# ShawnNew/Detectron2-CenterNet

Measured on AMD Instinct MI355X. Metric: images/sec at 512x512 (infer bs=64), higher is better.
Workload: dtype f16x3; 1 GPU; DLA-34 CenterNet eval forward+decode, 64x3x512x512 uint8 per GPU, 80 classes, K=100, random-init weights (BatchNorm statistics calibrated), DCN offsets ~N(0,1px), 100 detections per image post-processed; per_gpu_batch=64, global_batch=64, parallelism=replicas x1

## Files before the change

### detectron2-centernet_amd/_lib.py

```python
import ctypes as C
import os

_HERE = os.path.dirname(os.path.abspath(__file__))
LIB_PATH = os.path.join(_HERE, "lib", "libctdet_hip.so")

F16, F32, U8, F16X3 = 0, 1, 2, 3
ACT_NONE, ACT_RELU, ACT_SIGMOID_CLAMP = 0, 1, 2
DCN_MASK_LOGIT, DCN_MASK_PROB, DCN_MASK_NONE = 0, 1, 2
CLIP_NONE, CLIP_VALUE, CLIP_NORM = 0, 1, 2
NORM_L1, NORM_L2, NORM_INF = 1, 2, 3


class ConvDesc(C.Structure):
    _fields_ = [(n, C.c_int32) for n in (
        "B", "H", "W", "Cin", "in_stride", "Cout", "Ho", "Wo", "out_stride",
        "R", "S", "stride", "pad", "dil", "Kpad", "Cout_pad",
        "compute_dtype", "out_dtype", "act", "res_stride")] + [("clamp_lo", C.c_float), ("clamp_hi", C.c_float), ("korder", C.c_int32), ("in_dil", C.c_int32)]


_vp, _i32, _i64, _f32, _f64, _sz = C.c_void_p, C.c_int32, C.c_int64, C.c_float, C.c_double, C.c_size_t
SIGNATURES = {
    "ctdet_last_error": (C.c_char_p, []),
    "ctdet_abi_version": (_i32, []),
    "ctdet_conv_cout_tile": (_i32, [_i32]),
    "ctdet_set_label_mode": (_i32, [_i32]),
    "ctdet_last_kernel_label": (C.c_char_p, []),
    "ctdet_conv_pair_supported": (_i32, [C.POINTER(ConvDesc), _vp]),
    "ctdet_head_fused_supported": (_i32, [_i32, _i32, _i32, _i32, _i32, _vp]),
    "ctdet_conv2d_fwd": (_i32, [C.POINTER(ConvDesc), _vp, _vp, _vp, _vp, _vp, _vp, _vp]),
    "ctdet_conv1x1_cat_fwd": (_i32, [C.POINTER(ConvDesc), _vp, _vp, _vp, _i32, _vp, _vp, _vp, _vp, _vp, _vp]),
    "ctdet_dcnv2_fwd": (_i32, [C.POINTER(ConvDesc), _vp, _vp, _i32, _i32, _vp, _vp, _vp, _vp, _vp]),
    "ctdet_dcnv2_offset_supported": (_i32, [C.POINTER(ConvDesc)]),
    "ctdet_dcnv2_cols_supported": (_i32, [C.POINTER(ConvDesc), _vp, _vp]),
    "ctdet_dcnv2_fwd_cols": (_i32, [C.POINTER(ConvDesc), _vp, _vp, _i32, _i32, _vp, _vp, _vp, _vp, _vp, _vp]),
    "ctdet_dcnv2_offset_fwd": (_i32, [C.POINTER(ConvDesc), _vp, _vp, _vp, _vp, _i32, _vp, _vp, _vp, _vp, _vp]),
    "ctdet_preprocess": (_i32, [_vp, _i32, _vp, _i32, _i32, _i32, _i32, _i32, _i32, _i64, _vp, _vp, _i32, _i32, _vp]),
    "ctdet_preprocess_mirror": (_i32, [_vp, _i32, _vp, _i32, _i32, _i32, _i32, _i32, _i32, _i64, _vp, _vp, _i32, _i32, _i32, _vp]),
    "ctdet_head_fused_fwd": (_i32, [_vp, _vp, _vp, _vp, _vp]),
    "ctdet_head_fused_x3_fwd": (_i32, [_vp, _vp, _vp, _vp, _vp, _vp]),
    "ctdet_dla_base_fwd": (_i32, [_vp] * 14),
    "ctdet_dla_base_x3_fwd": (_i32, [_vp] * 14),
    "ctdet_dla_base_mirror_fwd": (_i32, [_vp, _i32] + [_vp] * 13),
    "ctdet_dla_base_x3_mirror_fwd": (_i32, [_vp, _i32] + [_vp] * 13),
    "ctdet_maxpool2x2": (_i32, [_vp, _vp, _i32, _i32, _i32, _i32, _i32, _i32, _i32, _vp]),
    "ctdet_maxpool3x3s2": (_i32, [_vp, _vp, _i32, _i32, _i32, _i32, _i32, _i32, _i32, _vp]),
    "ctdet_maxpool3x3s2_ceil": (_i32, [_vp, _vp, _i32, _i32, _i32, _i32, _i32, _i32, _i32, _vp]),
    "ctdet_global_avgpool": (_i32, [_vp, _i32, _i32, _i32, _i32, _i32, _vp, _vp]),
    "ctdet_ese_scale": (_i32, [_vp, _i32, _vp, _vp, _i32, _vp, _i32, _i32, _i32, _i32, _i32, _vp]),
    "ctdet_pack_weights": (_i32, [_vp, _vp, _i32, _i32, _i32, _i32, _i32, _i32, _i32, _i32, _i32, _vp]),
    "ctdet_pack_weights_batch": (_i32, [_vp, _i32, _i32, _vp]),
    "ctdet_split_weights": (_i32, [_vp, _vp, _i64, _vp]),
    "ctdet_pack_weights_x3": (_i32, [_vp, _vp, _vp] + [_i32] * 10 + [_vp]),
    "ctdet_pack_weights_x3_batch": (_i32, [_vp, _i32, _i32, _vp]),
    "ctdet_dwconvT_add": (_i32, [_vp, _vp, _vp, _vp, _i32, _i32, _i32, _i32, _i32, _i32, _i32, _i32, _i32, _vp]),
    "ctdet_dwconv3x3_fwd": (_i32, [_vp, _i32, _vp, _vp, _i32, _i32, _i32, _i32, _i32, _i32, _i32, _i32, _vp]),
    "ctdet_dwconv3x3_wgrad_workspace_bytes": (_sz, [_i32, _i32, _i32, _i32, _i32]),
    "ctdet_dwconv3x3_wgrad": (_i32, [_vp, _i32, _vp, _i32, _vp, _vp, _f32, _i32, _i32, _i32, _i32, _i32, _i32, _i32, _vp]),
    "ctdet_decode_workspace_bytes": (_sz, [_i32, _i32, _i32, _i32, _i32]),
    "ctdet_decode": (_i32, [_vp, _i32, _vp, _i32, _vp, _i32, _i32, _i32, _i32, _i32, _i32, _f32, _f32, _vp, _vp, _vp, _vp, _vp, _vp]),
    "ctdet_decode_flip": (_i32, [_vp, _i32, _vp, _i32, _vp, _i32, _i32, _i32, _i32, _i32, _i32, _f32, _f32, _vp, _vp, _vp, _vp, _vp, _vp]),
    "ctdet_postprocess": (_i32, [_vp, _vp, _vp, _i32, _i32, _i32, _f32, _vp, _vp, _vp, _vp, _vp, _vp]),
    "ctdet_decode_status": (_i32, [_vp, _i32, _i32, _i32, _i32, _i32, _vp]),
    "ctdet_gaussian_targets": (_i32, [_vp, _vp, _vp, _i32, _i32, _i32, _i32, _i32, _vp, _vp, _vp, _vp, _vp, _vp]),
    "ctdet_gaussian_radius": (_i32, [_vp, _i32, _vp, _vp, _vp]),
    "ctdet_focal_loss_workspace_bytes": (_sz, [_i64]),
    "ctdet_focal_loss": (_i32, [_vp, _vp, _vp, _i32, _i32, _i32, _i32, _f32, _vp, _vp, _vp, _vp, _vp]),
    "ctdet_reg_l1_loss": (_i32, [_vp, _i32, _vp, _vp, _vp, _i32, _i32, _i32, _f32, _vp, _vp, _i32, _vp]),
    "ctdet_chan_workspace_bytes": (_sz, [_i32]),
    "ctdet_bn_train_fwd": (_i32, [_vp, _i32, _vp, _i32, _vp, _i32, _i32, _i32, _vp, _vp, _f32, _f32, _vp, _vp, _vp, _vp,
                                   _vp, _vp, _vp, _i32, _i32, _vp]),
    "ctdet_bn_train_bwd": (_i32, [_vp, _i32, _vp, _i32, _vp, _i32, _vp, _vp, _vp, _i32, _i32, _i32, _vp, _i32, _vp, _i32,
                                   _vp, _vp, _f32, _vp, _i32, _vp]),
    "ctdet_bn_local_stats": (_i32, [_vp, _i32, _i32, _i32, _i32, _i32, _vp, _vp, _i32, _vp]),
    "ctdet_bn_sync_fwd": (_i32, [_vp, _i32, _vp, _i32, _vp, _i32, _i32, _i32, _vp, _i32, _vp, _vp, _f32, _f32, _vp, _vp, _vp,
                                  _vp, _vp, _vp, _i32, _i32, _vp]),
    "ctdet_bn_local_grad_sums": (_i32, [_vp, _i32, _vp, _i32, _vp, _i32, _vp, _vp, _i32, _i32, _i32, _i32, _i32, _vp, _vp, _vp,
                                         _f32, _vp, _i32, _vp]),
    "ctdet_bn_sync_bwd": (_i32, [_vp, _i32, _vp, _i32, _vp, _i32, _vp, _vp, _vp, _vp, _vp, _i32, _i32, _i32, _i32, _vp, _i32,
                                  _vp, _i32, _i32, _vp]),
    "ctdet_conv_wgrad": (_i32, [C.POINTER(ConvDesc), _vp, _vp, _vp, _f32, _vp]),
    "ctdet_conv_wgrad_oihw": (_i32, [C.POINTER(ConvDesc), _vp, _vp, _vp, _f32, _i32, _i32, _i32, _i32, _vp]),
    "ctdet_grad_scatter_oihw": (_i32, [_vp, _vp, _vp, _vp, _vp, _vp, _i32, _vp]),
    "ctdet_depth_to_space2": (_i32, [_vp, _i32, _vp, _i32, _i32, _i32, _i32, _i32, _i32, _i32, _i32, _vp]),
    "ctdet_maxpool3x3s2_bwd": (_i32, [_vp, _i32, _vp, _i32, _vp, _i32, _i32, _i32, _i32, _i32, _i32, _i32, _vp]),
    "ctdet_finite_flag": (_i32, [_vp, _i64, _i32, _i32, _vp, _vp]),
    "ctdet_ese_dot": (_i32, [_vp, _i32, _vp, _i32, _i32, _i32, _i32, _i32, _vp, _vp]),
    "ctdet_ese_bwd": (_i32, [_vp, _i32, _vp, _vp, _vp, _i32, _i32, _i32, _i32, _i32, _vp]),
    "ctdet_maxpool2x2_bwd": (_i32, [_vp, _i32, _vp, _i32, _vp, _i32, _i32, _i32, _i32, _i32, _i32, _vp]),
    "ctdet_dwconvT_bwd": (_i32, [_vp, _i32, _vp, _i32, _vp, _vp, _i32, _vp, _i32, _i32, _i32, _i32, _i32, _i32, _vp]),
    "ctdet_dcn_cols": (_i32, [_vp, _i32, _vp, _i32, _vp, _i32, _i32, _i32, _i32, _i32, _i32, _vp]),
    "ctdet_dcn_col2im_coord": (_i32, [_vp, _vp, _i32, _vp, _i32, _vp, _vp, _i32, _i32, _i32, _i32, _i32, _i32, _i32, _i32, _i32, _vp]),
    "ctdet_dcn_col2im_fused": (_i32, [_vp, _i32, _i32, _vp, _vp, _vp, _i32, _vp, _i32, _vp, _vp, _i32, _i32, _i32, _i32, _i32, _i32, _vp]),
    "ctdet_sgd_momentum": (_i32, [_vp, _vp, _vp, _i64, _vp, _f32, _f32, _i32, _vp]),
    "ctdet_sgd_momentum_runs": (_i32, [_vp, _vp, _vp, C.c_int64, _vp, _vp, _vp, _vp, _i32, _f32, _i32, _vp]),
    "ctdet_grad_chunk_norms": (_i32, [_vp, _i64, _vp, _vp, _i32, _i32, _vp, _vp]),
    "ctdet_grad_clip_coefs": (_i32, [_vp, _vp, _i32, _i32, _i32, _f32, _vp, _vp, _vp]),
    "ctdet_sgd_momentum_runs_clip": (_i32, [_vp, _vp, _vp, _i64, _vp, _vp, _vp, _vp, _i32, _f32, _i32, _i32, _i32, _f32, _vp,
                                             _vp]),
    "ctdet_adam_advance": (_i32, [_vp, _vp, _f64, _f64, _vp]),
    "ctdet_adam_runs": (_i32, [_vp, _vp, _vp, _vp, _vp, _i64, _vp, _vp, _vp, _vp, _i32, _vp, _f64, _f64, _f64, _i32, _i32, _i32,
                               _f32, _vp, _vp]),
    "ctdet_cocoeval_workspace_bytes": (_sz, [_i64, _i64, _i32, _i32, _i32, _i32]),
    "ctdet_cocoeval_iou": (_i32, [_vp, _i32, _vp, _vp, _i32, _vp, _vp]),
    "ctdet_cocoeval_match": (_i32, [_vp, _vp, _vp, _vp, _i64, _vp, _vp, _vp, _vp, _i64, _i32, _i32, _vp, _i32, _vp, _i32, _i32,
                                    _vp, _vp, _vp, _vp, _vp, _vp, _vp]),
    "ctdet_cocoeval_accumulate": (_i32, [_vp, _vp, _vp, _vp, _vp, _vp, _i64, _i32, _i32, _i32, _vp, _i32, _vp, _i32, _i32, _vp,
                                         _vp, _vp, _vp, _vp]),
    "ctdet_set_tuning_flags": (_i32, [C.c_uint32]),
    "ctdet_get_tuning_flags": (C.c_uint32, []),
    "ctdet_comm_unique_id": (_i32, [_vp]),
    "ctdet_comm_init": (_i32, [_vp, _i32, _i32, C.POINTER(C.c_void_p)]),
    "ctdet_allreduce_bucket": (_i32, [_vp, _vp, _i64, _vp]),
    "ctdet_bcast": (_i32, [_vp, _vp, _i64, _i32, _vp]),
    "ctdet_comm_destroy": (_i32, [_vp]),
}

_lib = None


def lib():
    global _lib
    if _lib is None:
        if not os.path.exists(LIB_PATH):
            raise RuntimeError(
                f"{LIB_PATH} is missing: build it with `python -c 'import __graft_entry__ as g; g.build()'` "
                "(or `make -C detectron2-centernet_amd/csrc`). There is no CPU fallback for the HIP path.")
        l = C.CDLL(LIB_PATH)
        for name, (res, args) in SIGNATURES.items():
            fn = getattr(l, name)
            fn.restype = res
            fn.argtypes = args
        _lib = l
        if os.environ.get("CTDET_TUNE_FLAGS"):
            l.ctdet_set_tuning_flags(int(os.environ["CTDET_TUNE_FLAGS"], 0))
    return _lib


def check(rc, what):
    if rc != 0:
        msg = lib().ctdet_last_error()
        raise RuntimeError(f"{what} failed (rc={rc}): {msg.decode() if msg else ''}")


class PackDesc(C.Structure):
    _fields_ = [("w", C.c_void_p), ("packed", C.c_void_p)] + [(n, C.c_int32) for n in (
        "O", "I", "R", "S", "chans_pad", "rows_pad", "Kpad", "korder", "transposed", "blk0")]


class Pack3Desc(C.Structure):
    _fields_ = [("w", C.c_void_p), ("packed", C.c_void_p), ("scale_out", C.c_void_p)] + [(n, C.c_int32) for n in (
        "O", "I", "R", "S", "chans_pad", "rows_pad", "Kpad", "layout", "transposed", "scale_n", "blk0", "pad_")]


class DlaBaseDesc(C.Structure):
    _fields_ = [("B", C.c_int32), ("H", C.c_int32), ("W", C.c_int32), ("Hp", C.c_int32), ("Wp", C.c_int32),
                ("img_dtype", C.c_int32), ("img_batch_stride", C.c_int64), ("mean", C.c_float * 3), ("std", C.c_float * 3),
                ("out_stride", C.c_int32), ("pool_stride", C.c_int32)]


class HeadDesc(C.Structure):
    _fields_ = [("nheads", C.c_int32), ("B", C.c_int32), ("H", C.c_int32), ("W", C.c_int32), ("Cin", C.c_int32),
                ("in_stride", C.c_int32), ("w2", C.c_void_p * 4), ("b2", C.c_void_p * 4), ("y", C.c_void_p * 4),
                ("y_stride", C.c_int32 * 4), ("cout", C.c_int32 * 4), ("act", C.c_int32 * 4),
                ("clamp_lo", C.c_float), ("clamp_hi", C.c_float)]


TUNE_NO_HALO, TUNE_NO_WIN, TUNE_DCN_MIXED, TUNE_NO_WGRAD_WINDOW, TUNE_NO_COL2IM_WINDOW, TUNE_NO_F32_DCN_WINDOW, TUNE_DCN_WINDOW_V1, TUNE_NO_SMALL_GRID_TILES = 1, 2, 4, 8, 16, 32, 64, 128
TUNE_DCN_SPLIT_4W = 256
TUNE_NO_HALO_TAP2 = 512
TUNE_PAIR2_128, TUNE_DCN_SPLIT_8W64, TUNE_TARGETS_MEMSET = 1024, 2048, 4096


class tuning:

    def __init__(self, flags):
        self.flags = flags

    def __enter__(self):
        self.prev = lib().ctdet_get_tuning_flags()
        lib().ctdet_set_tuning_flags(self.prev | self.flags)
        return self

    def __exit__(self, *exc):
        lib().ctdet_set_tuning_flags(self.prev)
        return False
```

### detectron2-centernet_amd/csrc/api.hip

```cpp
#include "conv_common.h"
#include "../../include/ctdet_hip.h"
#include <stdarg.h>
#include <stdio.h>
#include <string.h>
#include <stdlib.h>
#include <atomic>

static thread_local char g_err[512] = "";
void ctdet_set_error(const char* fmt, ...) {
  va_list ap;
  va_start(ap, fmt);
  vsnprintf(g_err, sizeof(g_err), fmt, ap);
  va_end(ap);
}

thread_local int g_label_mode = 0;
static thread_local char g_label[128] = "";
bool ctdet_set_label(const char* fmt, ...) {
  va_list ap;
  va_start(ap, fmt);
  vsnprintf(g_label, sizeof(g_label), fmt, ap);
  va_end(ap);
  return g_label_mode == 2;
}
// ... 193 lines not shown
    if (j < nsrc) {
      CTDET_CHECK(xs[j] && cins[j] > 0 && cins[j] % align == 0 && strides[j] >= cins[j] && strides[j] % align == 0,
                  "conv1x1_cat: bad source %d (cin=%d stride=%d)", j, cins[j], strides[j]);
      cum += cins[j];
      a.xs[j] = xs[j]; a.xs_stride[j] = strides[j];
    } else {
      a.xs[j] = xs[nsrc - 1]; a.xs_stride[j] = strides[nsrc - 1];
    }
    a.xs_cend[j] = cum;
  }
  CTDET_CHECK(cum == d->Cin, "conv1x1_cat: sources sum to %d channels, descriptor says %d", cum, d->Cin);
  a.nsrc = nsrc < 2 ? 2 : nsrc;
  if (nsrc == 1) { a.nsrc = 1; a.in_stride = strides[0]; }
  a.x = xs[0]; a.w = w_packed; a.scale = scale; a.bias = bias; a.res = residual; a.y = y;
  if (d->compute_dtype == CTDET_DT_F16) return launch_conv_f16(a, d->out_dtype, false, (hipStream_t)stream);
  if (d->compute_dtype == CTDET_DT_F32 || d->compute_dtype == CTDET_DT_F16X3) {
    CTDET_CHECK(d->out_dtype == CTDET_DT_F32, "conv1x1_cat(f32 / f16x3): output must be f32");
    return launch_conv_f32(a, false, d->compute_dtype == CTDET_DT_F16X3, (hipStream_t)stream);
  }
  CTDET_CHECK(false, "conv1x1_cat: bad compute dtype %d", d->compute_dtype);
}

int32_t ctdet_dcnv2_fwd(const ctdet_conv_desc* d, const void* x, const float* offset_mask, int32_t om_stride,
                        int32_t mask_is_prob, const void* w_packed, const float* scale, const float* bias, void* y, void* stream) {
  ConvArgs a;
  int rc = fill_args(d, a);
  if (rc) return rc;
  if (a.M == 0) return 0;
  CTDET_CHECK(x && w_packed && y && offset_mask, "dcnv2: null pointer");
  CTDET_CHECK(mask_is_prob >= CTDET_DCN_MASK_LOGIT && mask_is_prob <= CTDET_DCN_MASK_NONE, "dcnv2: mask mode %d", mask_is_prob);
  CTDET_CHECK(om_stride >= (mask_is_prob == CTDET_DCN_MASK_NONE ? 2 : 3) * d->R * d->S, "dcnv2: om_stride=%d < %d*R*S", om_stride,
              mask_is_prob == CTDET_DCN_MASK_NONE ? 2 : 3);
  a.x = x; a.w = w_packed; a.scale = scale; a.bias = bias; a.res = nullptr; a.y = y;
  a.om = offset_mask; a.om_stride = om_stride; a.mask_is_prob = mask_is_prob;
  if (d->compute_dtype == CTDET_DT_F16) return launch_conv_f16(a, d->out_dtype, true, (hipStream_t)stream);
  if (d->compute_dtype == CTDET_DT_F32 || d->compute_dtype == CTDET_DT_F16X3) {
    CTDET_CHECK(d->out_dtype == CTDET_DT_F32, "dcnv2(f32 / f16x3): output must be f32");
    return launch_conv_f32(a, true, d->compute_dtype == CTDET_DT_F16X3, (hipStream_t)stream);
  }
  CTDET_CHECK(false, "dcnv2: bad compute dtype %d", d->compute_dtype);
}

int32_t ctdet_dcnv2_cols_supported(const ctdet_conv_desc* d, const void* x, const void* y) {
  ConvArgs a;
  if (fill_args(d, a) || d->compute_dtype != CTDET_DT_F16X3 || d->out_dtype != CTDET_DT_F32) return 0;
  a.x = x; a.y = const_cast<void*>(y);
  return dcn_split_window_ok(a) ? 1 : 0;
}

int32_t ctdet_dcnv2_fwd_cols(const ctdet_conv_desc* d, const void* x, const float* offset_mask, int32_t om_stride,
                             int32_t mask_is_prob, const void* w_packed, const float* scale, const float* bias, void* y,
                             float* cols_out, void* stream) {
  ConvArgs a;
  int rc = fill_args(d, a);
  if (rc) return rc;
  if (a.M == 0) return 0;
  CTDET_CHECK(x && w_packed && y && offset_mask && cols_out, "dcnv2_fwd_cols: null pointer");
  CTDET_CHECK(mask_is_prob >= CTDET_DCN_MASK_LOGIT && mask_is_prob <= CTDET_DCN_MASK_NONE, "dcnv2: mask mode %d", mask_is_prob);
  CTDET_CHECK(om_stride >= (mask_is_prob == CTDET_DCN_MASK_NONE ? 2 : 3) * d->R * d->S, "dcnv2: om_stride=%d < %d*R*S", om_stride,
              mask_is_prob == CTDET_DCN_MASK_NONE ? 2 : 3);
  CTDET_CHECK(d->compute_dtype == CTDET_DT_F16X3 && d->out_dtype == CTDET_DT_F32 && (((size_t)cols_out) & 15) == 0,
              "dcnv2_fwd_cols: the f16x3 mode's entry point (f32 tensors), 16-byte aligned columns");
  a.x = x; a.w = w_packed; a.scale = scale; a.bias = bias; a.res = nullptr; a.y = y;
  a.om = offset_mask; a.om_stride = om_stride; a.mask_is_prob = mask_is_prob;
  CTDET_CHECK(dcn_split_window_ok(a), "dcnv2_fwd_cols: shape not served by the LDS-window kernel (ask ctdet_dcnv2_cols_supported first)");
  a.cols_out = cols_out;
  return launch_conv_f32(a, true, true, (hipStream_t)stream);
}

int32_t ctdet_dcnv2_offset_supported(const ctdet_conv_desc* d) {
  ConvArgs a;
  if (fill_args(d, a)) return 0;
  a.y = nullptr;
  if (d->compute_dtype == CTDET_DT_F16X3) return (d->out_dtype == CTDET_DT_F32 && dcn_offset_fused_x3_ok(a)) ? 1 : 0;
  if (d->compute_dtype != CTDET_DT_F16) return 0;
  return dcn_offset_fused_ok(a) ? 1 : 0;
}

int32_t ctdet_dcnv2_offset_fwd(const ctdet_conv_desc* d, const void* x, const void* w_off_packed, const float* b_off,
                               float* om_out, int32_t om_out_stride, const void* w_packed, const float* scale,
                               const float* bias, void* y, void* stream) {
  ConvArgs a;
  int rc = fill_args(d, a);
  if (rc) return rc;
  if (a.M == 0) return 0;
  CTDET_CHECK(x && w_off_packed && b_off && w_packed && y, "dcnv2_offset: null pointer");
  if (d->compute_dtype == CTDET_DT_F16X3) {
    CTDET_CHECK(d->out_dtype == CTDET_DT_F32 && !om_out, "dcnv2_offset(f16x3): f32 output, no om_out (inference form)");
    a.x = x; a.w = w_packed; a.scale = scale; a.bias = bias; a.res = nullptr; a.y = y;
    a.w_off = w_off_packed; a.b_off = b_off; a.mask_is_prob = DCN_MASK_LOGIT;
    return launch_dcn_offset_x3(a, (hipStream_t)stream);
  }
  CTDET_CHECK(d->compute_dtype == CTDET_DT_F16, "dcnv2_offset: f16 or f16x3");
  CTDET_CHECK(!om_out || (om_out_stride >= 28 && om_out_stride % 4 == 0 && ((size_t)om_out & 15) == 0),
              "dcnv2_offset: om_out needs a 16-byte aligned row of >= 28 floats (stride %d)", om_out_stride);
  a.x = x; a.w = w_packed; a.scale = scale; a.bias = bias; a.res = nullptr; a.y = y;
  a.w_off = w_off_packed; a.b_off = b_off; a.om_out = om_out; a.om_out_stride = om_out_stride;
  return launch_conv_f16(a, d->out_dtype, true, (hipStream_t)stream);
}

int32_t ctdet_preprocess(const void* img, int32_t img_dtype, void* out, int32_t out_dtype, int32_t B, int32_t H,
                         int32_t W, int32_t Hp, int32_t Wp, int64_t img_batch_stride, const float* mean3,
                         const float* std3, int32_t out_stride, int32_t border, void* stream) {
  CTDET_CHECK(img && out && mean3 && std3, "preprocess: null pointer");
  return launch_preprocess(img, img_dtype, out, out_dtype, B, H, W, Hp, Wp, (long)img_batch_stride, mean3, std3,
                           out_stride, border, -1, (hipStream_t)stream);
}

int32_t ctdet_preprocess_mirror(const void* img, int32_t img_dtype, void* out, int32_t out_dtype, int32_t B, int32_t H,
                                int32_t W, int32_t Hp, int32_t Wp, int64_t img_batch_stride, const float* mean3,
                                const float* std3, int32_t out_stride, int32_t border, int32_t mirror_from, void* stream) {
  CTDET_CHECK(img && out && mean3 && std3, "preprocess: null pointer");
  CTDET_CHECK(mirror_from >= 0 && mirror_from <= B, "preprocess: mirror_from=%d outside [0, B=%d]", mirror_from, B);
  return launch_preprocess(img, img_dtype, out, out_dtype, B, H, W, Hp, Wp, (long)img_batch_stride, mean3, std3,
                           out_stride, border, mirror_from, (hipStream_t)stream);
}

static int head_args(const ctdet_head_desc* d, HeadArgs& a) {
  a.nheads = d->nheads; a.B = d->B; a.H = d->H; a.W = d->W; a.Cin = d->Cin; a.in_stride = d->in_stride;
  a.clamp_lo = d->clamp_lo; a.clamp_hi = d->clamp_hi;
  CTDET_CHECK(d->nheads >= 1 && d->nheads <= 4, "head_fused: nheads=%d out of range", d->nheads);
  for (int h = 0; h < d->nheads; ++h) {
    CTDET_CHECK(d->w2[h] && d->b2[h] && d->y[h], "head_fused: head %d: null pointer", h);
    a.w2[h] = d->w2[h]; a.b2[h] = (const float*)d->b2[h]; a.y[h] = (float*)d->y[h];
    a.y_stride[h] = d->y_stride[h]; a.cout[h] = d->cout[h]; a.act[h] = d->act[h];
  }
  return 0;
}

int32_t ctdet_head_fused_supported(int32_t compute_dtype, int32_t H, int32_t W, int32_t Cin, int32_t in_stride, const void* x) {
  HeadArgs a = {};
  a.x = x; a.H = H; a.W = W; a.Cin = Cin; a.in_stride = in_stride;
  if (compute_dtype != CTDET_DT_F16 && compute_dtype != CTDET_DT_F16X3) return 0;
  return head_fused_x_ok(a, compute_dtype == CTDET_DT_F16X3) ? 1 : 0;
}

int32_t ctdet_head_fused_fwd(const ctdet_head_desc* d, const void* x, const void* w1, const float* b1, void* stream) {
  CTDET_CHECK(d && x && w1 && b1, "head_fused: null pointer");
  HeadArgs a = {};
  a.x = x; a.w1 = w1; a.b1 = b1;
  if (int rc = head_args(d, a)) return rc;
  return launch_head_fused(a, (hipStream_t)stream);
}

int32_t ctdet_head_fused_x3_fwd(const ctdet_head_desc* d, const void* x, const void* w1, const float* s1, const float* b1,
                                void* stream) {
  CTDET_CHECK(d && x && w1 && s1 && b1, "head_fused_x3: null pointer");
  HeadArgs a = {};
  a.x = x; a.w1 = w1; a.s1 = s1; a.b1 = b1;
  if (int rc = head_args(d, a)) return rc;
  return launch_head_fused_x3(a, (hipStream_t)stream);
}

static int32_t dla_base_entry(const ctdet_dla_base_desc* d, int mirror_from, const void* images, const void* w_stem,
                              const float* scale_stem, const float* bias_stem, const void* w_l0, const float* scale_l0,
                              const float* bias_l0, const void* w_l1, const float* scale_l1, const float* bias_l1,
                              void* out, void* pooled, void* stream) {
  CTDET_CHECK(d && images && w_stem && scale_stem && bias_stem && w_l0 && scale_l0 && bias_l0 && w_l1 && scale_l1 && bias_l1 &&
              out, "dla_base: null pointer");
  BaseArgs a = {};
  a.img = images; a.img_dtype = d->img_dtype; a.img_batch_stride = (long)d->img_batch_stride;
  a.B = d->B; a.H = d->H; a.W = d->W; a.Hp = d->Hp; a.Wp = d->Wp;
  for (int i = 0; i < 3; ++i) { a.mean[i] = d->mean[i]; a.stdv[i] = d->std[i]; }
  a.w0 = w_stem; a.s0 = scale_stem; a.b0 = bias_stem;
  a.w1 = w_l0; a.s1 = scale_l0; a.b1 = bias_l0;
  a.w2 = w_l1; a.s2 = scale_l1; a.b2 = bias_l1;
  a.y = out; a.out_stride = d->out_stride;
  a.pool = pooled; a.pool_stride = d->pool_stride;
  a.mirror_from = mirror_from;
  return launch_dla_base(a, (hipStream_t)stream);
}

int32_t ctdet_dla_base_fwd(const ctdet_dla_base_desc* d, const void* images, const void* w_stem, const float* scale_stem,
                           const float* bias_stem, const void* w_l0, const float* scale_l0, const float* bias_l0,
                           const void* w_l1, const float* scale_l1, const float* bias_l1, void* out, void* pooled,
                           void* stream) {
  return dla_base_entry(d, -1, images, w_stem, scale_stem, bias_stem, w_l0, scale_l0, bias_l0, w_l1, scale_l1, bias_l1, out,
                        pooled, stream);
}

int32_t ctdet_dla_base_mirror_fwd(const ctdet_dla_base_desc* d, int32_t mirror_from, const void* images, const void* w_stem,
                                  const float* scale_stem, const float* bias_stem, const void* w_l0, const float* scale_l0,
                                  const float* bias_l0, const void* w_l1, const float* scale_l1, const float* bias_l1,
                                  void* out, void* pooled, void* stream) {
  CTDET_CHECK(d && mirror_from >= 0 && mirror_from <= d->B, "dla_base: mirror_from=%d outside [0, B=%d]", mirror_from,
              d ? d->B : 0);
  return dla_base_entry(d, mirror_from, images, w_stem, scale_stem, bias_stem, w_l0, scale_l0, bias_l0, w_l1, scale_l1,
                        bias_l1, out, pooled, stream);
}

static int32_t dla_base_x3_entry(const ctdet_dla_base_desc* d, int mirror_from, const void* images, const void* w_stem,
                                 const float* scale_stem, const float* bias_stem, const void* w_l0, const float* scale_l0,
                                 const float* bias_l0, const void* w_l1, const float* scale_l1, const float* bias_l1,
                                 float* out, float* pooled, void* stream) {
  CTDET_CHECK(d && images && w_stem && scale_stem && bias_stem && w_l0 && scale_l0 && bias_l0 && w_l1 && scale_l1 && bias_l1 &&
              out, "dla_base(f16x3): null pointer");
  BaseArgs a = {};
  a.img = images; a.img_dtype = d->img_dtype; a.img_batch_stride = (long)d->img_batch_stride;
  a.B = d->B; a.H = d->H; a.W = d->W; a.Hp = d->Hp; a.Wp = d->Wp;
  for (int i = 0; i < 3; ++i) { a.mean[i] = d->mean[i]; a.stdv[i] = d->std[i]; }
  a.w0 = w_stem; a.s0 = scale_stem; a.b0 = bias_stem;
  a.w1 = w_l0; a.s1 = scale_l0; a.b1 = bias_l0;
  a.w2 = w_l1; a.s2 = scale_l1; a.b2 = bias_l1;
  a.y = out; a.out_stride = d->out_stride;
  a.pool = pooled; a.pool_stride = d->pool_stride;
  a.mirror_from = mirror_from;
  return launch_dla_base_x3(a, (hipStream_t)stream);
}

int32_t ctdet_dla_base_x3_fwd(const ctdet_dla_base_desc* d, const void* images, const void* w_stem, const float* scale_stem,
                              const float* bias_stem, const void* w_l0, const float* scale_l0, const float* bias_l0,
                              const void* w_l1, const float* scale_l1, const float* bias_l1, float* out, float* pooled,
                              void* stream) {
  return dla_base_x3_entry(d, -1, images, w_stem, scale_stem, bias_stem, w_l0, scale_l0, bias_l0, w_l1, scale_l1, bias_l1,
                           out, pooled, stream);
}

int32_t ctdet_dla_base_x3_mirror_fwd(const ctdet_dla_base_desc* d, int32_t mirror_from, const void* images,
                                     const void* w_stem, const float* scale_stem, const float* bias_stem, const void* w_l0,
                                     const float* scale_l0, const float* bias_l0, const void* w_l1, const float* scale_l1,
                                     const float* bias_l1, float* out, float* pooled, void* stream) {
  CTDET_CHECK(d && mirror_from >= 0 && mirror_from <= d->B, "dla_base(f16x3): mirror_from=%d outside [0, B=%d]", mirror_from,
              d ? d->B : 0);
  return dla_base_x3_entry(d, mirror_from, images, w_stem, scale_stem, bias_stem, w_l0, scale_l0, bias_l0, w_l1, scale_l1,
                           bias_l1, out, pooled, stream);
}

int32_t ctdet_maxpool2x2(const void* x, void* y, int32_t dtype, int32_t B, int32_t H, int32_t W, int32_t C,
                         int32_t in_stride, int32_t out_stride, void* stream) {
  CTDET_CHECK(x && y, "maxpool2x2: null pointer");
  return launch_maxpool2x2(x, y, dtype, B, H, W, C, in_stride, out_stride, (hipStream_t)stream);
}

int32_t ctdet_maxpool3x3s2(const void* x, void* y, int32_t dtype, int32_t B, int32_t H, int32_t W, int32_t C,
                           int32_t in_stride, int32_t out_stride, void* stream) {
  CTDET_CHECK(x && y, "maxpool3x3s2: null pointer");
  return launch_maxpool3x3s2(x, y, dtype, B, H, W, C, in_stride, out_stride, 0, (hipStream_t)stream);
}

int32_t ctdet_maxpool3x3s2_ceil(const void* x, void* y, int32_t dtype, int32_t B, int32_t H, int32_t W, int32_t C,
                                int32_t in_stride, int32_t out_stride, void* stream) {
  CTDET_CHECK(x && y, "maxpool3x3s2_ceil: null pointer");
  return launch_maxpool3x3s2(x, y, dtype, B, H, W, C, in_stride, out_stride, 1, (hipStream_t)stream);
}

int32_t ctdet_global_avgpool(const void* x, int32_t dtype, int32_t B, int32_t HW, int32_t C, int32_t stride, float* out,
                             void* stream) {
  CTDET_CHECK(x && out, "global_avgpool: null pointer");
  return launch_global_avgpool(x, dtype, B, HW, C, stride, out, (hipStream_t)stream);
}

int32_t ctdet_finite_flag(const float* x, int64_t M, int32_t C, int32_t stride, int32_t* flag, void* stream) {
  CTDET_CHECK(x && flag, "finite_flag: null pointer");
  return launch_finite_flag(x, (long)M, C, stride, (int*)flag, (hipStream_t)stream);
}

int32_t ctdet_ese_scale(const void* x, int32_t x_stride, const float* s, const void* identity, int32_t identity_stride,
                        void* y, int32_t y_stride, int32_t dtype, int32_t B, int32_t HW, int32_t C, void* stream) {
  CTDET_CHECK(x && s && y, "ese_scale: null pointer");
  return launch_ese_scale(x, x_stride, s, identity, identity_stride, y, y_stride, dtype, B, HW, C, (hipStream_t)stream);
}

int32_t ctdet_pack_weights(const float* w, void* packed, int32_t O, int32_t I, int32_t R, int32_t S, int32_t chans_pad,
                           int32_t rows_pad, int32_t Kpad, int32_t korder, int32_t transposed, void* stream) {
  CTDET_CHECK(w && packed, "pack_weights: null pointer");
  return launch_pack_weights(w, packed, O, I, R, S, chans_pad, rows_pad, Kpad, korder, transposed, (hipStream_t)stream);
}

int32_t ctdet_split_weights(const float* w_packed_f32, void* w_split, int64_t n, void* stream) {
  CTDET_CHECK(w_packed_f32 && w_split && n >= 0, "split_weights: bad arguments");
  return launch_split_weights(w_packed_f32, w_split, (long)n, (hipStream_t)stream);
}

int32_t ctdet_pack_weights_batch(const ctdet_pack_desc* table_dev, int32_t n, int32_t total_blocks, void* stream) {
  CTDET_CHECK(n >= 0 && total_blocks >= 0 && (n == 0 || table_dev), "pack_weights_batch: bad arguments");
  static_assert(sizeof(ctdet_pack_desc) == 56, "ctdet_pack_desc layout");
  return launch_pack_weights_batch(table_dev, n, total_blocks, (hipStream_t)stream);
}

int32_t ctdet_pack_weights_x3(const float* w, void* packed, float* scale_out, int32_t O, int32_t I, int32_t R, int32_t S,
                              int32_t chans_pad, int32_t rows_pad, int32_t Kpad, int32_t layout, int32_t transposed,
                              int32_t scale_n, void* stream) {
  return launch_pack_weights_x3(w, packed, scale_out, O, I, R, S, chans_pad, rows_pad, Kpad, layout, transposed, scale_n,
                                (hipStream_t)stream);
}

int32_t ctdet_pack_weights_x3_batch(const ctdet_pack3_desc* table_dev, int32_t n, int32_t total_blocks, void* stream) {
  CTDET_CHECK(n >= 0 && total_blocks >= 0 && (n == 0 || table_dev), "pack_weights_x3_batch: bad arguments");
  static_assert(sizeof(ctdet_pack3_desc) == 72, "ctdet_pack3_desc layout");
  return launch_pack_weights_x3_batch(table_dev, n, total_blocks, (hipStream_t)stream);
}

int32_t ctdet_dwconvT_add(const void* x, const float* w, const void* skip, void* y, int32_t dtype, int32_t B,
                          int32_t H, int32_t W, int32_t C, int32_t f, int32_t in_stride, int32_t skip_stride,
                          int32_t out_stride, void* stream) {
  CTDET_CHECK(x && w && y, "dwconvT: null pointer");
  return launch_dwconvT_add(x, w, skip, y, dtype, B, H, W, C, f, in_stride, skip_stride, out_stride,
                            (hipStream_t)stream);
}

int32_t ctdet_dwconv3x3_fwd(const void* x, int32_t x_stride, const float* w, void* y, int32_t y_stride, int32_t B, int32_t H,
                            int32_t W, int32_t C, int32_t stride, int32_t rot180, int32_t dtype, void* stream) {
  CTDET_CHECK(x && w && y, "dwconv3x3: null pointer");
  CTDET_CHECK(rot180 == 0 || rot180 == 1, "dwconv3x3: rot180 %d", rot180);
  const int strides[2] = {x_stride, y_stride};
  const int rc = dwconv3x3_check(dtype, B, H, W, C, stride, strides, 2);
  if (rc) return rc;
  return launch_dwconv3x3(x, x_stride, w, y, y_stride, B, H, W, C, stride, rot180, dtype, (hipStream_t)stream);
}

size_t ctdet_dwconv3x3_wgrad_workspace_bytes(int32_t B, int32_t H, int32_t W, int32_t C, int32_t dtype) {
  return dwconv3x3_wgrad_workspace_bytes(B, H, W, C, dtype);
}

int32_t ctdet_dwconv3x3_wgrad(const void* x, int32_t x_stride, const void* dy, int32_t dy_stride, float* workspace, float* dw,
                              float scale, int32_t accumulate, int32_t B, int32_t H, int32_t W, int32_t C, int32_t stride,
                              int32_t dtype, void* stream) {
  CTDET_CHECK(x && dy && dw, "dwconv3x3_wgrad: null pointer");
  CTDET_CHECK(accumulate == 0 || accumulate == 1, "dwconv3x3_wgrad: accumulate %d", accumulate);
  const int strides[2] = {x_stride, dy_stride};
  const int rc = dwconv3x3_check(dtype, B, H, W, C, stride, strides, 2);
  if (rc) return rc;
  CTDET_CHECK(stride == 1, "dwconv3x3_wgrad: stride %d: only the stride-1 backward is built", stride);
  CTDET_CHECK(workspace || dwconv3x3_wgrad_workspace_bytes(B, H, W, C, dtype) == 0, "dwconv3x3_wgrad: null workspace");
  CTDET_CHECK(((uintptr_t)dw & 3) == 0 && ((uintptr_t)workspace & 3) == 0, "dwconv3x3_wgrad: misaligned dw / workspace");
  return launch_dwconv3x3_wgrad(x, x_stride, dy, dy_stride, workspace, dw, scale, accumulate, B, H, W, C, dtype,
                                (hipStream_t)stream);
}

size_t ctdet_decode_workspace_bytes(int32_t B, int32_t H, int32_t W, int32_t C, int32_t K) {
  return decode_workspace_bytes(B, H, W, C, K);
}

static int32_t decode_entry(bool flip, const float* heat, int32_t heat_stride, const float* wh, int32_t wh_stride,
                            const float* reg, int32_t reg_stride, int32_t B, int32_t H, int32_t W, int32_t C, int32_t K,
                            float down_ratio, float heat_floor, void* workspace, float* boxes, float* scores,
                            int32_t* classes, int32_t* inds, void* stream) {
  CTDET_CHECK(heat && wh && workspace && boxes && scores && classes, "decode: null pointer");
  CTDET_CHECK(B >= 0 && H > 0 && W > 0, "decode: bad shape B=%d H=%d W=%d", B, H, W);
  CTDET_CHECK(heat_floor >= 0.f && heat_floor < 1.f, "decode: heat_floor %g outside [0, 1)", (double)heat_floor);
  DecArgs a;
  a.heat = heat; a.wh = wh; a.reg = reg; a.heat_stride = heat_stride; a.wh_stride = wh_stride; a.reg_stride = reg_stride;
  a.B = B; a.H = H; a.W = W; a.C = C; a.K = K; a.down_ratio = down_ratio;
  memcpy(&a.floor_bits, &heat_floor, 4);
  a.ws = (uint32_t*)workspace; a.boxes = boxes; a.scores = scores; a.classes = classes; a.inds = inds;
  return launch_decode(a, flip, (hipStream_t)stream);
}

int32_t ctdet_decode(const float* heat, int32_t heat_stride, const float* wh, int32_t wh_stride, const float* reg,
                     int32_t reg_stride, int32_t B, int32_t H, int32_t W, int32_t C, int32_t K, float down_ratio,
                     float heat_floor, void* workspace, float* boxes, float* scores, int32_t* classes, int32_t* inds,
                     void* stream) {
  return decode_entry(false, heat, heat_stride, wh, wh_stride, reg, reg_stride, B, H, W, C, K, down_ratio, heat_floor,
                      workspace, boxes, scores, classes, inds, stream);
}

int32_t ctdet_decode_flip(const float* heat, int32_t heat_stride, const float* wh, int32_t wh_stride, const float* reg,
                          int32_t reg_stride, int32_t B, int32_t H, int32_t W, int32_t C, int32_t K, float down_ratio,
                          float heat_floor, void* workspace, float* boxes, float* scores, int32_t* classes, int32_t* inds,
                          void* stream) {
  return decode_entry(true, heat, heat_stride, wh, wh_stride, reg, reg_stride, B, H, W, C, K, down_ratio, heat_floor,
                      workspace, boxes, scores, classes, inds, stream);
}

int32_t ctdet_postprocess(const float* boxes, const float* scores, const int32_t* classes, int32_t B, int32_t K,
                          int32_t max_det, float score_thresh, const float* img_params, float* out_boxes,
                          float* out_scores, int32_t* out_classes, int32_t* counts, void* stream) {
  CTDET_CHECK(boxes && scores && classes && img_params && out_boxes && out_scores && out_classes && counts,
              "postprocess: null pointer");
  return launch_postprocess(boxes, scores, classes, B, K, max_det, score_thresh, img_params, out_boxes, out_scores,
                            out_classes, counts, (hipStream_t)stream);
}

int32_t ctdet_decode_status(const void* workspace, int32_t B, int32_t H, int32_t W, int32_t C, int32_t K, void* stream) {
  long words = 0;
  int below = 0;
  const int flag = decode_status_words(H, W, C, K, &words, &below);
  for (int b = 0; b < B; ++b) {
    uint32_t st[16];
    hipError_t e = hipMemcpyAsync(st, (const char*)workspace + (size_t)words * 4 * b, sizeof(st), hipMemcpyDeviceToHost,
                                  (hipStream_t)stream);
    if (e == hipSuccess) e = hipStreamSynchronize((hipStream_t)stream);
    CTDET_CHECK(e == hipSuccess, "decode_status: copy failed: %s", hipGetErrorString(e));
    if (st[flag]) {
      ctdet_set_error("decode: image %d overflowed the candidate buffer", b);
      return -75;
    }
    if (st[below]) {
      ctdet_set_error("decode: image %d holds positive heat values below the promised heat_floor", b);
      return -22;
    }
  }
  return 0;
}

int32_t ctdet_gaussian_targets(const float* boxes, const int64_t* classes, const int32_t* counts, int32_t B,
                               int32_t Nmax, int32_t H, int32_t W, int32_t C, float* hm, float* wh, float* reg,
                               int64_t* ind, uint8_t* reg_mask, void* stream) {
  CTDET_CHECK(boxes && classes && counts && hm && wh && reg && ind && reg_mask, "gaussian_targets: null pointer");
  CTDET_CHECK(Nmax >= 1, "gaussian_targets: Nmax must be >= 1");
  return launch_gaussian_targets(boxes, classes, counts, B, Nmax, H, W, C, hm, wh, reg, ind, reg_mask,
                                 (hipStream_t)stream);
}

int32_t ctdet_gaussian_radius(const int32_t* hw_pairs, int32_t n, double* out_radius, int32_t* out_int, void* stream) {
  CTDET_CHECK(hw_pairs, "gaussian_radius: null pointer");
  return launch_gaussian_radius(hw_pairs, n, out_radius, out_int, (hipStream_t)stream);
}

size_t ctdet_focal_loss_workspace_bytes(int64_t numel) { return focal_workspace_bytes((long)numel); }

int32_t ctdet_focal_loss(const float* logits, const float* gt, const float* alpha, int32_t B, int32_t H, int32_t W,
                         int32_t C, float grad_scale, void* workspace, float* loss, float* stats, float* grad,
                         void* stream) {
  CTDET_CHECK(logits && gt && alpha && workspace && loss && stats, "focal_loss: null pointer");
  return launch_focal_loss(logits, gt, alpha, B, H, W, C, grad_scale, workspace, loss, stats, grad, (hipStream_t)stream);
}

int32_t ctdet_reg_l1_loss(const float* pred, int32_t pred_stride, const uint8_t* mask, const int64_t* ind,
                          const float* target, int32_t B, int32_t N, int32_t HW, float grad_scale, float* loss,
                          float* grad, int32_t grad_stride, void* stream) {
  CTDET_CHECK(pred && mask && ind && target && loss, "reg_l1_loss: null pointer");
  return launch_reg_l1(pred, pred_stride, mask, ind, target, B, N, HW, grad_scale, loss, grad, grad_stride,
                       (hipStream_t)stream);
}

size_t ctdet_chan_workspace_bytes(int32_t C) { return chan_reduce_workspace_bytes(C); }

int32_t ctdet_bn_train_fwd(const void* y, int32_t y_stride, const void* res, int32_t res_stride, void* z,
                           int32_t z_stride, int32_t M, int32_t C, const float* gamma, const float* beta, float eps,
                           float momentum, float* running_mean, float* running_var, float* save_mean,
                           float* save_invstd, float* scale, float* shift, void* workspace, int32_t relu, int32_t dtype,
                           void* stream) {
  CTDET_CHECK(y && z && gamma && beta && save_mean && save_invstd && scale && shift && workspace, "bn_train_fwd: null pointer");
  CTDET_CHECK(M > 0, "bn_train_fwd: empty batch");
  if (dtype == CTDET_DT_F32)
    return launch_bn_train_fwd_f32((const float*)y, y_stride, (const float*)res, res_stride, (float*)z, z_stride, M, C, gamma,
                                   beta, eps, momentum, running_mean, running_var, save_mean, save_invstd, scale, shift,
                                   workspace, relu, (hipStream_t)stream);
  return launch_bn_train_fwd((const f16*)y, y_stride, (const f16*)res, res_stride, (f16*)z, z_stride, M, C, gamma, beta,
                             eps, momentum, running_mean, running_var, save_mean, save_invstd, scale, shift, workspace,
                             relu, (hipStream_t)stream);
}

int32_t ctdet_bn_train_bwd(const void* dz, int32_t dz_stride, const void* z, int32_t z_stride, const void* y,
                           int32_t y_stride, const float* mean, const float* invstd, const float* scale, int32_t M,
                           int32_t C, int32_t relu, void* dy, int32_t dy_stride, void* dres, int32_t dres_stride,
                           float* dgamma, float* dbeta, float grad_mult, void* workspace, int32_t dtype, void* stream) {
  CTDET_CHECK(dz && dy && dgamma && dbeta && workspace, "bn_train_bwd: null pointer");
  CTDET_CHECK(!relu || z, "bn_train_bwd: relu backward needs z");
  CTDET_CHECK(!y || (mean && invstd && scale), "bn_train_bwd: statistics missing");
  if (dtype == CTDET_DT_F32)
    return launch_bn_train_bwd_f32((const float*)dz, dz_stride, (const float*)z, z_stride, (const float*)y, y_stride, mean,
                                   invstd, scale, M, C, relu, (float*)dy, dy_stride, (float*)dres, dres_stride, dgamma,
                                   dbeta, grad_mult, workspace, (hipStream_t)stream);
  return launch_bn_train_bwd((const f16*)dz, dz_stride, (const f16*)z, z_stride, (const f16*)y, y_stride, mean, invstd,
                             scale, M, C, relu, (f16*)dy, dy_stride, (f16*)dres, dres_stride, dgamma, dbeta, grad_mult,
                             workspace, (hipStream_t)stream);
}

static const int SYNC_BN_MAX_WORLD = 4096;

int32_t ctdet_bn_local_stats(const void* y, int32_t y_stride, int32_t M, int32_t C, int32_t rank, int32_t world,
                             double* stats, void* workspace, int32_t dtype, void* stream) {
  CTDET_CHECK(M > 0, "bn_local_stats: empty batch on rank %d (SyncBatchNorm needs at least one row on every rank)", rank);
  CTDET_CHECK(y && stats && workspace, "bn_local_stats: null pointer");
  CTDET_CHECK(world >= 1 && world <= SYNC_BN_MAX_WORLD && rank >= 0 && rank < world, "bn_local_stats: rank %d of world %d",
              rank, world);
  return launch_bn_local_stats(y, y_stride, M, C, rank, world, stats, workspace, dtype == CTDET_DT_F32, (hipStream_t)stream);
}

int32_t ctdet_bn_sync_fwd(const void* y, int32_t y_stride, const void* res, int32_t res_stride, void* z, int32_t z_stride,
                          int32_t M, int32_t C, const double* stats, int32_t world, const float* gamma, const float* beta,
                          float eps, float momentum, float* running_mean, float* running_var, float* save_mean,
                          float* save_invstd, float* scale, float* shift, int32_t relu, int32_t dtype, void* stream) {
  CTDET_CHECK(y && z && stats && gamma && beta && save_mean && save_invstd && scale && shift, "bn_sync_fwd: null pointer");
  CTDET_CHECK(!running_mean == !running_var, "bn_sync_fwd: running_mean and running_var go together");
  CTDET_CHECK(M > 0, "bn_sync_fwd: empty batch");
  CTDET_CHECK(world >= 1 && world <= SYNC_BN_MAX_WORLD, "bn_sync_fwd: world %d", world);
  return launch_bn_sync_fwd(y, y_stride, res, res_stride, z, z_stride, M, C, stats, world, gamma, beta, eps, momentum,
                            running_mean, running_var, save_mean, save_invstd, scale, shift, relu, dtype == CTDET_DT_F32,
                            (hipStream_t)stream);
}

int32_t ctdet_bn_local_grad_sums(const void* dz, int32_t dz_stride, const void* z, int32_t z_stride, const void* y,
                                 int32_t y_stride, const float* mean, const float* invstd, int32_t M, int32_t C, int32_t relu,
                                 int32_t rank, int32_t world, double* sums, float* dgamma, float* dbeta, float grad_mult,
                                 void* workspace, int32_t dtype, void* stream) {
  CTDET_CHECK(dz && sums && dgamma && dbeta && workspace, "bn_local_grad_sums: null pointer");
  CTDET_CHECK(!relu || z, "bn_local_grad_sums: relu backward needs z");
  CTDET_CHECK(!y || (mean && invstd), "bn_local_grad_sums: statistics missing");
// ... 220 lines not shown
```

### detectron2-centernet_amd/csrc/common.h

```cpp
#pragma once
#include <hip/hip_runtime.h>
#include <stdint.h>

typedef _Float16 f16;
typedef f16 f16x4 __attribute__((ext_vector_type(4)));
typedef f16 f16x8 __attribute__((ext_vector_type(8)));
typedef f16 f16x16 __attribute__((ext_vector_type(16)));
typedef float f32x4 __attribute__((ext_vector_type(4)));

void ctdet_set_error(const char* fmt, ...);
#define CTDET_CHECK(cond, ...)            \
  do {                                    \
    if (!(cond)) {                        \
      ctdet_set_error(__VA_ARGS__);       \
      return -22;            \
    }                                     \
  } while (0)
#define CTDET_LAUNCH_CHECK()                                          \
  do {                                                                \
    hipError_t e_ = hipGetLastError();                                \
    if (e_ != hipSuccess) {                                           \
      ctdet_set_error("kernel launch failed: %s (%s:%d)",            \
                      hipGetErrorString(e_), __FILE__, __LINE__);     \
      return -5;                                            \
    }                                                                 \
  } while (0)

extern thread_local int g_label_mode;
bool ctdet_set_label(const char* fmt, ...);
#define CTDET_KERNEL(...)                                             \
  do {                                                                \
    if (g_label_mode && ctdet_set_label(__VA_ARGS__)) return 0;       \
  } while (0)
template <typename TOut> inline const char* out_name() { return sizeof(TOut) == 2 ? "f16" : "f32"; }

enum { CTDET_F16 = 0, CTDET_F32 = 1, CTDET_U8 = 2, CTDET_F16X3 = 3 };
enum { CTDET_ACT_NONE = 0, CTDET_ACT_RELU = 1, CTDET_ACT_SIGMOID_CLAMP = 2 };
enum { DCN_MASK_LOGIT = 0, DCN_MASK_PROB = 1, DCN_MASK_NONE = 2 };
enum { SGD_CLIP_NONE = 0, SGD_CLIP_VALUE = 1, SGD_CLIP_NORM = 2 };
enum { GRAD_NORM_L1 = 1, GRAD_NORM_L2 = 2, GRAD_NORM_INF = 3 };
__host__ __device__ inline int dcn_om_channels(int mask_mode) { return mask_mode == DCN_MASK_NONE ? 18 : 27; }

struct ConvArgs {
  const void* x;
  const void* w;
  const float* scale;
  const float* bias;
  const void* res;
  void* y;
  const void* xs[4];
  int xs_stride[4];
  int xs_cend[4];
  int nsrc;
  const float* om;
  int om_stride;
  int mask_is_prob;
  int B, H, W, Cin, in_stride;
  int Cout, Ho, Wo, out_stride, res_stride;
  int R, S, stride, pad, dil;
  int K, Kpad, Cout_pad;
  int M;
  int act;
  float clamp_lo, clamp_hi;
  int korder;
  int in_dil;
  const void* w_off; const float* b_off; float* om_out; int om_out_stride;
  float* cols_out;
};

struct HeadArgs {
  const void* x;
  const void* w1;
  const float* b1;
  const void* w2[4];
  const float* b2[4];
  float* y[4];
  int y_stride[4], cout[4], act[4];
  int nheads, B, H, W, Cin, in_stride;
  float clamp_lo, clamp_hi;
  const float* s1;
};

struct BaseArgs {
  const void* img;
  int img_dtype;
  long img_batch_stride;
  int B, H, W;
  int Hp, Wp;
  float mean[3], stdv[3];
  const void* w0;
  const void* w1;
  const void* w2;
  const float *s0, *b0, *s1, *b1, *s2, *b2;
  void* y;
  int out_stride;
  void* pool;
  int pool_stride;
  int mirror_from;
};
int launch_dla_base(const BaseArgs& a, hipStream_t s);
int launch_dla_base_x3(const BaseArgs& a, hipStream_t s);

struct DecArgs {
  const float* heat; const float* wh; const float* reg;
  int heat_stride, wh_stride, reg_stride;
  int B, H, W, C, K;
  float down_ratio;
  uint32_t floor_bits;
  uint32_t* ws;
  float* boxes; float* scores; int* classes; int* inds;
};

__device__ __forceinline__ float ctdet_sigmoid(float v) { return 1.0f / (1.0f + __expf(-v)); }
__device__ __forceinline__ float ctdet_sigmoid_exact(float v) { return 1.0f / (1.0f + expf(-v)); }

enum {
  CTDET_TUNE_NO_HALO = 1,
  CTDET_TUNE_NO_WIN = 2,
  CTDET_TUNE_DCN_MIXED = 4,
  CTDET_TUNE_NO_WGRAD_WINDOW = 8,
  CTDET_TUNE_NO_COL2IM_WINDOW = 16,
  CTDET_TUNE_NO_F32_DCN_WINDOW = 32,
  CTDET_TUNE_NO_SMALL_GRID_TILES = 128,
  CTDET_TUNE_NO_HALO_TAP2 = 512,
  CTDET_TUNE_DCN_SPLIT_4W = 256,
  CTDET_TUNE_PAIR2_128 = 1024,
  CTDET_TUNE_DCN_SPLIT_8W64 = 2048,
  CTDET_TUNE_TARGETS_MEMSET = 4096,
  CTDET_TUNE_DCN_WINDOW_V1 = 64,
};
unsigned ctdet_tuning_flags();
int ctdet_device_cu_count();

int launch_conv_f16(const ConvArgs& a, int out_dtype, bool deform, hipStream_t s);
int launch_head_fused(const HeadArgs& a, hipStream_t s);
int launch_head_fused_x3(const HeadArgs& a, hipStream_t s);
int launch_conv_f32(const ConvArgs& a, bool deform, bool split, hipStream_t s);
```

### detectron2-centernet_amd/csrc/conv_igemm.hip

```cpp
#include "common.h"
#include <type_traits>
#include <stdlib.h>

#include "conv_common.h"

template <int BP, int BC, int WP, int WC_, typename TOut>
__global__ void __launch_bounds__(256) conv_igemm_dma_kernel(const ConvArgs a) {
  constexpr int TP = BP / WP / 16;
  constexpr int TC = BC / WC_ / 16;
  constexpr int A_LD = BP / 64;
  constexpr int BCL = BC < 64 ? 64 : BC;
  constexpr int B_LD = BCL / 64;
  constexpr int NLOAD = A_LD + B_LD;
  constexpr int STAGE = (BP + BCL) * 64;
  constexpr int NST = 3;
  static_assert(WP * WC_ == 4, "4 waves per workgroup");
  __shared__ __attribute__((aligned(16))) char smem[NST * STAGE];

  const int tid = threadIdx.x, lane = tid & 63;
  const int wave = __builtin_amdgcn_readfirstlane(tid >> 6);
  const int wp = wave / WC_, wc = wave % WC_;
  int m_tile, n_tile;
  if (!tile_of_block((a.M + BP - 1) / BP, a.Cout_pad / BC, m_tile, n_tile)) return;
  const int m0 = m_tile * BP, n0 = n_tile * BC;
// ... 1390 lines not shown
#pragma unroll
    for (int hb = 0; hb < TC / 2; ++hb) {
      const f16x8 wa = *(const f16x8*)(wrow + hb * 32);
#pragma unroll
      for (int p = 0; p < TP; ++p) o[p] = __builtin_amdgcn_mfma_f32_16x16x32_f16(wa, frag[p][hb], o[p], 0, 0, 0);
    }
    const int c0 = ot * 16 + 4 * kg;
    if (c0 < ((cout + 3) & ~3)) {
      const f32x4 bv = *(const f32x4*)(b2 + c0);
#pragma unroll
      for (int p = 0; p < TP; ++p) {
        f32x4 v = o[p] + bv;
        if (act == CTDET_ACT_RELU) {
#pragma unroll
          for (int j = 0; j < 4; ++j) v[j] = fmaxf(v[j], 0.f);
        } else if (act == CTDET_ACT_SIGMOID_CLAMP) {
#pragma unroll
          for (int j = 0; j < 4; ++j) v[j] = fminf(fmaxf(ctdet_sigmoid_exact(v[j]), a.clamp_lo), a.clamp_hi);
        }
        const long m = (long)(b * a.H + ty0 + row0 + p) * a.W + tx0 + l15;
        *(f32x4*)(yh + m * ystride + c0) = v;
      }
    }
  }
}

bool head_fused_x_ok(const HeadArgs& a, bool x3) {
  if (!x3) return a.Cin % 32 == 0 && a.H % 8 == 0 && a.W % 16 == 0 && a.in_stride % 8 == 0;
  return a.Cin % 32 == 0 && ((a.H % 8 == 0 && a.W % 32 == 0) || (a.H % 16 == 0 && a.W % 16 == 0)) && a.in_stride % 4 == 0 &&
         (((size_t)a.x) & 15) == 0;
}

int launch_head_fused(const HeadArgs& a, hipStream_t s) {
  CTDET_CHECK(a.nheads >= 1 && a.nheads <= 4, "head_fused: 1..4 heads");
  CTDET_CHECK(head_fused_x_ok(a, false),
              "head_fused: needs Cin %% 32 == 0 and a map divisible by 8x16 (Cin=%d, %dx%d)", a.Cin, a.H, a.W);
  for (int h = 0; h < a.nheads; ++h)
    CTDET_CHECK(a.cout[h] >= 1 && a.cout[h] <= 256 && a.y_stride[h] % 4 == 0 && a.y_stride[h] >= ((a.cout[h] + 3) & ~3) &&
                    (((size_t)a.y[h]) & 15) == 0,
                "head_fused: head %d: bad output (cout %d, stride %d)", h, a.cout[h], a.y_stride[h]);
  const int nbx = a.B * (a.H / 8) * (a.W / 16);
  dim3 grid(8 * ((nbx + 7) / 8) * a.nheads);
  CTDET_KERNEL("head_fused_kernel<128x256,f16>");
  hipLaunchKernelGGL(head_fused_kernel, grid, dim3(256), 0, s, a);
  CTDET_LAUNCH_CHECK();
  return 0;
}

template <int TW>
__global__ void __launch_bounds__(256, 2) head_fused_x3_kernel(const HeadArgs a) {
  constexpr int HID = 256, BC = 64, WP = 4, NSL = HID / BC;
  constexpr int TH = 256 / TW, EN = TW / 16, TP = 256 / WP / 16, TC = BC / 16, ROWS_W = TH / WP;
  static_assert(TP == 4 && TC == 4, "four 16-pixel tiles x four 16-channel tiles per wave");
  __shared__ __attribute__((aligned(16))) char smem[pair2_smem_bytes<BC>()];
  const int tiles_x = a.W / TW, tiles_y = a.H / TH;
  int m_tile, head;
  if (!tile_of_block(a.B * tiles_y * tiles_x, a.nheads, m_tile, head)) return;
  const int tx0 = (m_tile % tiles_x) * TW;
  const int ty0 = ((m_tile / tiles_x) % tiles_y) * TH;
  const int b = m_tile / (tiles_x * tiles_y);
  ConvArgs c = {};
  c.x = a.x; c.w = a.w1; c.H = a.H; c.W = a.W; c.in_stride = a.in_stride; c.Cin = a.Cin; c.Kpad = a.Cin / 32 * 288;

  const int lane = threadIdx.x & 63, wave = __builtin_amdgcn_readfirstlane(threadIdx.x >> 6);
  const int row0 = wave * ROWS_W, l15 = lane & 15, q = lane >> 4;
  const f16* w2 = (const f16*)a.w2[head];
  const float* b2 = a.b2[head];
  float* yh = a.y[head];
  const int ystride = a.y_stride[head], cout = a.cout[head], act = a.act[head];
  const int rows2 = (cout + 15) & ~15, ntile2 = rows2 >> 4, cw = (cout + 3) & ~3;
  long mpix[TP];
#pragma unroll
  for (int p = 0; p < TP; ++p) mpix[p] = (long)(b * a.H + ty0 + row0 + p / EN) * a.W + tx0 + 16 * (p % EN) + l15;

  for (int sl = 0; sl < NSL; ++sl) {
    if (sl > 0) __syncthreads();
    const int n0 = head * HID + sl * BC;
    f32x4 acc[TP][TC];
    pair2_kloop<BC, WP, 1, TW>(c, smem, b, ty0, tx0, n0, acc);

    f16x8 hf[TP][TC / 2], lf[TP][TC / 2];
#pragma unroll
    for (int hb = 0; hb < TC / 2; ++hb) {
      const int c0 = n0 + hb * 32 + q * 8;
      const f32x4 sa = *(const f32x4*)(a.s1 + c0), sb = *(const f32x4*)(a.s1 + c0 + 4);
      const f32x4 ba = *(const f32x4*)(a.b1 + c0), bb = *(const f32x4*)(a.b1 + c0 + 4);
#pragma unroll
      for (int p = 0; p < TP; ++p) {
        const f32x4 v0 = acc[p][2 * hb] * sa + ba, v1 = acc[p][2 * hb + 1] * sb + bb;
        f16x8 hi, lo;
#pragma unroll
        for (int j = 0; j < 8; ++j) {
          const float h = fmaxf(j < 4 ? v0[j] : v1[j - 4], 0.f);
          hi[j] = (f16)h;
          lo[j] = (f16)(h - (float)hi[j]);
        }
        hf[p][hb] = hi;
        lf[p][hb] = lo;
      }
    }
    for (int ot = 0; ot < ntile2; ++ot) {
      f32x4 o[TP];
#pragma unroll
      for (int p = 0; p < TP; ++p) o[p] = (f32x4){0.f, 0.f, 0.f, 0.f};
      const f16* wrow = w2 + (long)(ot * 16 + l15) * (2 * HID) + sl * BC + q * 8;
#pragma unroll
      for (int hb = 0; hb < TC / 2; ++hb) {
        const f16x8 X = *(const f16x8*)(wrow + hb * 32), Y = *(const f16x8*)(wrow + HID + hb * 32);
#pragma unroll
        for (int p = 0; p < TP; ++p) o[p] = __builtin_amdgcn_mfma_f32_16x16x32_f16(X, hf[p][hb], o[p], 0, 0, 0);
#pragma unroll
        for (int p = 0; p < TP; ++p) o[p] = __builtin_amdgcn_mfma_f32_16x16x32_f16(Y, hf[p][hb], o[p], 0, 0, 0);
#pragma unroll
        for (int p = 0; p < TP; ++p) o[p] = __builtin_amdgcn_mfma_f32_16x16x32_f16(X, lf[p][hb], o[p], 0, 0, 0);
      }
      const int c0 = ot * 16 + 4 * q;
      if (c0 < cw) {
#pragma unroll
        for (int p = 0; p < TP; ++p) {
          float* yp = yh + mpix[p] * ystride + c0;
          f32x4 v = o[p];
          if (sl > 0) v = *(const f32x4*)yp + v;
          if (sl == NSL - 1) {
            v = v * *(const f32x4*)(b2 + rows2 + c0) + *(const f32x4*)(b2 + c0);
            if (act == CTDET_ACT_RELU) {
#pragma unroll
              for (int j = 0; j < 4; ++j) v[j] = fmaxf(v[j], 0.f);
            } else if (act == CTDET_ACT_SIGMOID_CLAMP) {
#pragma unroll
              for (int j = 0; j < 4; ++j) v[j] = fminf(fmaxf(ctdet_sigmoid_exact(v[j]), a.clamp_lo), a.clamp_hi);
            }
          }
          *(f32x4*)yp = v;
        }
      }
    }
  }
}

int launch_head_fused_x3(const HeadArgs& a, hipStream_t s) {
  CTDET_CHECK(a.nheads >= 1 && a.nheads <= 4, "head_fused_x3: 1..4 heads");
  CTDET_CHECK(head_fused_x_ok(a, true) && (((size_t)a.w1 | (size_t)a.s1 | (size_t)a.b1) & 15) == 0,
              "head_fused_x3: needs Cin %% 32 == 0 and a map divisible by 8x32 or 16x16 (Cin=%d, %dx%d)", a.Cin, a.H, a.W);
  for (int h = 0; h < a.nheads; ++h)
    CTDET_CHECK(a.cout[h] >= 1 && a.cout[h] <= 256 && a.y_stride[h] % 4 == 0 && a.y_stride[h] >= ((a.cout[h] + 3) & ~3) &&
                    ((((size_t)a.y[h]) | (size_t)a.w2[h] | (size_t)a.b2[h]) & 15) == 0,
                "head_fused_x3: head %d: bad output (cout %d, stride %d)", h, a.cout[h], a.y_stride[h]);
  const int TW = a.W % 32 == 0 ? 32 : 16;
  const int nbx = a.B * (a.H / (256 / TW)) * (a.W / TW);
  dim3 grid(8 * ((nbx + 7) / 8) * a.nheads);
  CTDET_KERNEL(TW == 32 ? "head_fused_x3_kernel<256x256,f16x3>" : "head_fused_x3_kernel<16x16x256,f16x3>");
  if (TW == 32) hipLaunchKernelGGL(head_fused_x3_kernel<32>, grid, dim3(256), 0, s, a);
  else hipLaunchKernelGGL(head_fused_x3_kernel<16>, grid, dim3(256), 0, s, a);
  CTDET_LAUNCH_CHECK();
  return 0;
}

static bool halo16_ok(const ConvArgs& a) {
  return a.R == 3 && a.S == 3 && a.stride == 1 && a.pad == 1 && a.dil == 1 && a.in_dil == 1 && a.nsrc <= 1 &&
         a.korder == 1 && a.Cin % 32 == 0 && a.Kpad == a.K && a.H % 16 == 0 && a.W % 16 == 0 && a.W % 32 != 0 && a.Ho == a.H &&
         a.Wo == a.W && !(ctdet_tuning_flags() & CTDET_TUNE_NO_HALO);
}

static bool halo_ok(const ConvArgs& a) {
  return a.R == 3 && a.S == 3 && a.stride == 1 && a.pad == 1 && a.dil == 1 && a.in_dil == 1 && a.nsrc <= 1 &&
         a.korder == 1 && a.Cin % 32 == 0 && a.Kpad == a.K && a.H % 8 == 0 && a.W % 32 == 0 && a.Ho == a.H &&
         a.Wo == a.W && !(ctdet_tuning_flags() & CTDET_TUNE_NO_HALO);
}

__device__ __forceinline__ unsigned pk_mul_wlo(unsigned v, unsigned w) {
  unsigned r;
  asm("v_pk_mul_f16 %0, %1, %2 op_sel_hi:[1,0]" : "=v"(r) : "v"(v), "v"(w));
  return r;
}
__device__ __forceinline__ unsigned pk_fma_wlo(unsigned v, unsigned w, unsigned c) {
  unsigned r;
  asm("v_pk_fma_f16 %0, %1, %2, %3 op_sel_hi:[1,0,1]" : "=v"(r) : "v"(v), "v"(w), "v"(c));
  return r;
}
__device__ __forceinline__ unsigned pk_fma_whi(unsigned v, unsigned w, unsigned c) {
  unsigned r;
  asm("v_pk_fma_f16 %0, %1, %2, %3 op_sel:[0,1,0] op_sel_hi:[1,1,1]" : "=v"(r) : "v"(v), "v"(w), "v"(c));
  return r;
}
typedef unsigned u32x4 __attribute__((ext_vector_type(4)));
__device__ __forceinline__ u32x4 dcn_blend(const u32x4& v0, const u32x4& v1, const u32x4& v2, const u32x4& v3,
                                           unsigned w01, unsigned w23) {
  unsigned r0, r1, r2, r3;
  asm("v_pk_mul_f16 %0, %4, %20 op_sel_hi:[1,0]\n\t"
      "v_pk_mul_f16 %1, %5, %20 op_sel_hi:[1,0]\n\t"
      "v_pk_mul_f16 %2, %6, %20 op_sel_hi:[1,0]\n\t"
      "v_pk_mul_f16 %3, %7, %20 op_sel_hi:[1,0]\n\t"
      "v_pk_fma_f16 %0, %8, %20, %0 op_sel:[0,1,0] op_sel_hi:[1,1,1]\n\t"
      "v_pk_fma_f16 %1, %9, %20, %1 op_sel:[0,1,0] op_sel_hi:[1,1,1]\n\t"
      "v_pk_fma_f16 %2, %10, %20, %2 op_sel:[0,1,0] op_sel_hi:[1,1,1]\n\t"
      "v_pk_fma_f16 %3, %11, %20, %3 op_sel:[0,1,0] op_sel_hi:[1,1,1]\n\t"
      "v_pk_fma_f16 %0, %12, %21, %0 op_sel_hi:[1,0,1]\n\t"
      "v_pk_fma_f16 %1, %13, %21, %1 op_sel_hi:[1,0,1]\n\t"
      "v_pk_fma_f16 %2, %14, %21, %2 op_sel_hi:[1,0,1]\n\t"
      "v_pk_fma_f16 %3, %15, %21, %3 op_sel_hi:[1,0,1]\n\t"
      "v_pk_fma_f16 %0, %16, %21, %0 op_sel:[0,1,0] op_sel_hi:[1,1,1]\n\t"
      "v_pk_fma_f16 %1, %17, %21, %1 op_sel:[0,1,0] op_sel_hi:[1,1,1]\n\t"
      "v_pk_fma_f16 %2, %18, %21, %2 op_sel:[0,1,0] op_sel_hi:[1,1,1]\n\t"
      "v_pk_fma_f16 %3, %19, %21, %3 op_sel:[0,1,0] op_sel_hi:[1,1,1]"
      : "=&v"(r0), "=&v"(r1), "=&v"(r2), "=&v"(r3)
      : "v"(v0.x), "v"(v0.y), "v"(v0.z), "v"(v0.w), "v"(v1.x), "v"(v1.y), "v"(v1.z), "v"(v1.w), "v"(v2.x), "v"(v2.y),
        "v"(v2.z), "v"(v2.w), "v"(v3.x), "v"(v3.y), "v"(v3.z), "v"(v3.w), "v"(w01), "v"(w23));
  u32x4 r;
  r.x = r0; r.y = r1; r.z = r2; r.w = r3;
  return r;
}

template <int BC, int NST, bool PARTIAL, typename TOut, bool MIXED = false, bool NM = false>
__global__ void __launch_bounds__(256, 2) dcn_window_kernel(const ConvArgs a) {
  constexpr int TH = 8, TW = 16, BP = 128, MG = 4;
  constexpr int WR = TH + 2 + 2 * MG, WCOLS = TW + 2 + 2 * MG;
  constexpr int NPIECE = WR * WCOLS * 4;
  constexpr int W_LD = (NPIECE + 255) / 256;
  constexpr int WINB = ((NPIECE + 63) / 64) * 1024;
  constexpr int GEOW = 9 * BP * 8, GEOO = 9 * BP * 4;
  constexpr int TP = 2, TC = BC / 16;
  constexpr int B_LD = BC / 64, WST = BC * 64;
  constexpr int PF = NST - 1;
  static_assert(BC % 64 == 0, "BC");
  constexpr int SBB = 2 * BC * 4;
  constexpr bool WPRE = BC == 64;
  static_assert(WINB + GEOW + GEOO + NST * WST + SBB <= 81920, "two workgroups per CU");
  __shared__ __attribute__((aligned(16))) char smem[WINB + GEOW + GEOO + NST * WST + SBB];
  char* const win = smem;
  char* const geow = smem + WINB;
  char* const geoo = smem + WINB + GEOW;
  char* const ring = smem + WINB + GEOW + GEOO;
  float* const sbuf = (float*)(smem + WINB + GEOW + GEOO + NST * WST);

  const int tid = threadIdx.x, lane = tid & 63;
  const int wave = __builtin_amdgcn_readfirstlane(tid >> 6);
  const int tiles_x = (a.W + TW - 1) / TW, tiles_y = (a.H + TH - 1) / TH;
  int m_tile, n_tile;
  if (!tile_of_block(a.B * tiles_y * tiles_x, a.Cout_pad / BC, m_tile, n_tile)) return;
  const int tx0 = (m_tile % tiles_x) * TW;
  const int ty0 = ((m_tile / tiles_x) % tiles_y) * TH;
  const int b = m_tile / (tiles_x * tiles_y);
  const int n0 = n_tile * BC;
  const f16* zero = (const f16*)g_zero_page;
  asm volatile("" : "+v"(zero));
  const f16* ximg = (const f16*)a.x + (long)b * a.H * a.W * a.in_stride;
  const int wy0 = ty0 - 1 - MG, wx0 = tx0 - 1 - MG;
  const int nch = a.Cin / 32, nk = nch * 9;

  const int lrow = tid >> 2, slotw = tid & 3;
  const int gwk = slotw ^ swz(lrow);
  const f16* wptr[B_LD];
#pragma unroll
  for (int j = 0; j < B_LD; ++j) {
    const int L = lrow + 64 * j;
    const int tt = L >> 4, r = L & 15;
    const int cl = cout_of<TC>(tt, r >> 2, r & 3);
    wptr[j] = (const f16*)a.w + (long)(n0 + cl) * a.Kpad + gwk * 8;
  }
  auto issue_w = [&](int kt) {
    const int st = kt % NST;
#pragma unroll
    for (int j = 0; j < B_LD; ++j) dma16(wptr[j] + (long)kt * 32, ring + st * WST + wave * 1024 + j * 4096);
  };
  int wofs[W_LD];
#pragma unroll
  for (int i = 0; i < W_LD; ++i) {
    const int pid = tid + 256 * i;
    const int pw = pid >> 2, sl = pid & 3;
    const int wr = pw / WCOLS, wcn = pw - wr * WCOLS;
    const int y = wy0 + wr, x = wx0 + wcn;
    const bool ok = pid < NPIECE && y >= 0 && y < a.H && x >= 0 && x < a.W;
    wofs[i] = ok ? (y * a.W + x) * a.in_stride + (sl ^ (2 * (wr & 1))) * 8 : -1;
  }
  auto issue_window = [&](int chunk) {
#pragma unroll
    for (int i = 0; i < W_LD; ++i) {
      if (i < W_LD - 1 || (wave * 64 + 256 * i) * 16 < WINB)
        dma16(wofs[i] >= 0 ? ximg + wofs[i] + chunk * 32 : zero, win + (wave * 64 + 256 * i) * 16);
    }
  };
  issue_window(0);
#pragma unroll
  for (int i = 0; i < PF; ++i)
    if (i < nk) issue_w(i);

  if (tid < BC) {
    const int c = n0 + tid;
    sbuf[tid] = (a.scale && c < a.Cout) ? a.scale[c] : 1.f;
    sbuf[BC + tid] = (a.bias && c < a.Cout) ? a.bias[c] : 0.f;
  }
  {
    const int gp = tid & 127, gh = tid >> 7;
    const int py = ty0 + (gp >> 4), pxx = tx0 + (gp & 15);
    const bool pin = !PARTIAL || (py < a.H && pxx < a.W);
    const float* omrow = a.om + ((long)(b * a.H + (pin ? py : 0)) * a.W + (pin ? pxx : 0)) * a.om_stride;
    float oh[5], ow[5], om_[5];
#pragma unroll
    for (int i = 0; i < 5; ++i) {
      const int t = 2 * i + gh;
      const bool on = t < 9 && pin;
      oh[i] = on ? omrow[2 * t] : 0.f; ow[i] = on ? omrow[2 * t + 1] : 0.f; om_[i] = (on && !NM) ? omrow[18 + t] : 0.f;
    }
#pragma unroll
    for (int i = 0; i < 5; ++i) {
      const int t = 2 * i + gh;
// ... 941 lines not shown
```

### detectron2-centernet_amd/csrc/decode.hip

```cpp
#include "common.h"

#define DEC_CAP 2048
#define DEC_NCAND 4096
#define DEC_HIST 4096
#define DEC_LEVELS 6
#define DEC_TILE_SLACK 128
#define DEC_TW 16
#define DEC_LDS_TILE (60 * 1024)
#define DEC_ST_WORDS 16
enum { ST_NCAND = 0, ST_OVERFLOW = 1, ST_BELOW_FLOOR = 2 };

__device__ __forceinline__ int dec_d0(uint32_t bits) {
  const int d = ((int)bits - 0x38000000) >> 15;
  return d < 0 ? 0 : (d > 4095 ? 4095 : d);
}
__device__ __forceinline__ uint64_t dec_key(uint32_t bits, uint32_t canon) {
  return ((uint64_t)bits << 24) | (uint64_t)(0xFFFFFFu - canon);
}

struct DecSel { uint32_t p0; uint64_t care, want; uint32_t above, inbin; bool takeall; };

template <int NT, typename V>
__device__ __forceinline__ DecSel dec_select(V visit, uint32_t* lh, uint32_t need, uint32_t slack) {
  constexpr int NW = NT / 64;
// ... 238 lines not shown
  const uint32_t npk = sh_npk;
  auto visit = [&](auto f) {
    for (uint32_t i = t; i < npk; i += DEC_TNT) {
      const uint32_t lp = ppos[i];
      const uint32_t pos = (uint32_t)((y0 + (int)((lp >> 4) & 7u)) * a.W + x0 + (int)(lp & 15u));
      f(pbits[i], (uint32_t)(c0 + (int)(lp >> 7)) * (uint32_t)HW + pos);
    }
  };
  const DecSel sel = dec_select<DEC_TNT>(visit, lh, (uint32_t)a.K, DEC_TILE_SLACK);
  uint32_t* ws = a.ws + (long)b * ws_words;
  if (t == 0) {
    const uint32_t n = sel.above + sel.inbin;
    sh_slot = 0;
    sh_base = n ? atomicAdd(&ws[ST_NCAND], n) : 0u;
  }
  __syncthreads();
  uint64_t* cand = (uint64_t*)(ws + DEC_ST_WORDS);
  const uint32_t base = sh_base;
  visit([&](uint32_t bits, uint32_t canon) {
    if (!dec_selected(sel, bits, canon)) return;
    const uint32_t slot = base + atomicAdd(&sh_slot, 1u);
    if (slot < (uint32_t)cap) cand[slot] = ((uint64_t)bits << 32) | (uint64_t)(0xFFFFFFFFu - canon);
    else ws[ST_OVERFLOW] = 1;
  });
}

template <bool FLIP>
__global__ void __launch_bounds__(1024) dec_final_kernel(DecArgs a, long ws_words, int cap) {
  __shared__ uint64_t keys[DEC_NCAND];
  __shared__ uint32_t lh[DEC_HIST];
  __shared__ uint32_t sh_n;
  const int b = blockIdx.x;
  uint32_t* ws = a.ws + (long)b * ws_words;
  const uint64_t* cand = (const uint64_t*)(ws + DEC_ST_WORDS);
  uint32_t ncand = ws[ST_NCAND];
  if (ncand > (uint32_t)cap) ncand = (uint32_t)cap;
  const int t = threadIdx.x;
  auto visit = [&](auto f) {
    for (uint32_t i = t; i < ncand; i += 1024) {
      const uint64_t k = cand[i];
      f((uint32_t)(k >> 32), 0xFFFFFFFFu - (uint32_t)k);
    }
  };
  const DecSel sel = dec_select<1024>(visit, lh, (uint32_t)a.K, DEC_CAP);
  if (t == 0) sh_n = 0;
  __syncthreads();
  visit([&](uint32_t bits, uint32_t canon) {
    if (!dec_selected(sel, bits, canon)) return;
    const uint32_t slot = atomicAdd(&sh_n, 1u);
    if (slot < DEC_NCAND) keys[slot] = ((uint64_t)bits << 32) | (uint64_t)(0xFFFFFFFFu - canon);
    else ws[ST_OVERFLOW] = 1;
  });
  __syncthreads();
  uint32_t n = sh_n;
  if (n > DEC_NCAND) n = DEC_NCAND;
  int NS = 256;
  while ((uint32_t)NS < n) NS <<= 1;
  for (int i = t; i < NS; i += 1024) if ((uint32_t)i >= n) keys[i] = 0ull;
  __syncthreads();
  for (int k = 2; k <= NS; k <<= 1) {
    for (int j = k >> 1; j > 0; j >>= 1) {
      for (int i = t; i < NS; i += 1024) {
        const int ixj = i ^ j;
        if (ixj > i) {
          const uint64_t x = keys[i], y = keys[ixj];
          const bool desc = (i & k) == 0;
          if (desc ? (x < y) : (x > y)) { keys[i] = y; keys[ixj] = x; }
        }
      }
      __syncthreads();
    }
  }
  const int HW = a.H * a.W;
  uint32_t* fill = lh;
  uint32_t nfloor = 0;
  if (n < (uint32_t)a.K) {
    __shared__ uint32_t sh_got, wcnt[16];
    const float* hb = a.heat + (long)b * HW * a.heat_stride;
    const float* hb2 = FLIP ? a.heat + (long)(b + a.B) * HW * a.heat_stride : nullptr;
    const uint32_t total = (uint32_t)a.C * (uint32_t)HW, need = (uint32_t)a.K - n;
    const int lane = t & 63, wv = t >> 6;
    auto probe = [&](uint32_t c, float& v) -> bool {
      const int cls = (int)(c / (uint32_t)HW), pix = (int)(c % (uint32_t)HW);
      const int x = pix % a.W, y = pix / a.W;
      if constexpr (FLIP) v = dec_heat_flip(hb, hb2, a.W, a.heat_stride, pix, cls);
      else v = hb[(long)pix * a.heat_stride + cls];
      if (!(v > 0.f)) return false;
      bool peak = true;
      for (int dy = -1; dy <= 1; ++dy)
        for (int dx = -1; dx <= 1; ++dx) {
          const int yy = y + dy, xx = x + dx;
          if (yy < 0 || yy >= a.H || xx < 0 || xx >= a.W) continue;
          if constexpr (FLIP) peak &= dec_heat_flip(hb, hb2, a.W, a.heat_stride, yy * a.W + xx, cls) <= v;
          else peak &= hb[(long)(yy * a.W + xx) * a.heat_stride + cls] <= v;
        }
      return peak;
    };
    if (t == 0) sh_got = 0;
    __syncthreads();
    if (a.floor_bits) {
      for (uint32_t base = 0; base < total; base += 1024) {
        const uint32_t c = base + (uint32_t)t;
        bool on = false;
        if (c < total) {
          const int cls = (int)(c / (uint32_t)HW), pix = (int)(c % (uint32_t)HW);
          float v = hb[(long)pix * a.heat_stride + cls];
          if constexpr (FLIP) v = dec_heat_flip(hb, hb2, a.W, a.heat_stride, pix, cls);
          if (__float_as_uint(v) == a.floor_bits) on = probe(c, v);
        }
        const unsigned long long m = __ballot(on);
        if (lane == 0) wcnt[wv] = (uint32_t)__popcll(m);
        __syncthreads();
        uint32_t before = sh_got, all = 0;
        for (int w = 0; w < 16; ++w) { const uint32_t q = wcnt[w]; all += q; if (w < wv) before += q; }
        if (on) {
          const uint32_t pos = before + (uint32_t)__popcll(m & ((1ull << lane) - 1ull));
          if (pos < need) fill[2048 + pos] = c;
        }
        __syncthreads();
        if (t == 0) sh_got += all;
        __syncthreads();
        if (sh_got >= need) break;
      }
    }
    const uint32_t got_f = sh_got < need ? sh_got : need;
    nfloor = got_f;
    if (got_f < need) {
      const uint32_t span = 2u * (uint32_t)a.K < total ? 2u * (uint32_t)a.K : total;
      for (uint32_t c = t; c < span; c += 1024) { float v; fill[c] = probe(c, v) ? 1u : 0u; }
      __syncthreads();
      if (t == 0) {
        uint32_t got = got_f;
        for (uint32_t c = 0; c < span && got < need; ++c)
          if (!fill[c]) fill[2048 + got++] = c;
        for (; got < need; ++got) fill[2048 + got] = 0;
      }
      __syncthreads();
    }
  }
  for (int k = t; k < a.K; k += 1024) {
    const uint64_t key = k < NS ? keys[k] : 0ull;
    float score = 0.f; int cls = 0, ind = 0;
    if ((uint32_t)k < n) {
      score = __uint_as_float((uint32_t)(key >> 32));
      const uint32_t canon = 0xFFFFFFFFu - (uint32_t)key;
      cls = (int)(canon / HW);
      ind = (int)(canon % HW);
    } else {
      const uint32_t canon = fill[2048 + k - n];
      cls = (int)(canon / HW);
      ind = (int)(canon % HW);
      if ((uint32_t)k - n < nfloor) score = __uint_as_float(a.floor_bits);
    }
    const int x = ind % a.W, y = ind / a.W;
    const long pix = (long)b * HW + ind;
    float xs = (float)x, ys = (float)y;
    if (a.reg) { xs = xs + a.reg[pix * a.reg_stride]; ys = ys + a.reg[pix * a.reg_stride + 1]; }
    else { xs += 0.5f; ys += 0.5f; }
    const float w0 = a.wh[pix * a.wh_stride], h0 = a.wh[pix * a.wh_stride + 1];
    float wm = w0, hm = h0;
    if constexpr (FLIP) {
      const long mpix = (long)(b + a.B) * HW + (ind - x) + (a.W - 1 - x);
      wm = (w0 + a.wh[mpix * a.wh_stride]) * 0.5f;
      hm = (h0 + a.wh[mpix * a.wh_stride + 1]) * 0.5f;
    }
    const float w = wm, h = hm;
    const long o = (long)b * a.K + k;
    a.boxes[o * 4 + 0] = (xs - w / 2) * a.down_ratio;
    a.boxes[o * 4 + 1] = (ys - h / 2) * a.down_ratio;
    a.boxes[o * 4 + 2] = (xs + w / 2) * a.down_ratio;
    a.boxes[o * 4 + 3] = (ys + h / 2) * a.down_ratio;
    a.scores[o] = score;
    a.classes[o] = cls;
    if (a.inds) a.inds[o] = ind;
  }
}

__global__ void __launch_bounds__(64) dec_postprocess_kernel(const float* __restrict__ boxes,
                                                            const float* __restrict__ scores,
                                                            const int* __restrict__ classes, int K, int max_det,
                                                            float thresh, const float* __restrict__ img_params,
                                                            float* __restrict__ out_boxes, float* __restrict__ out_scores,
                                                            int* __restrict__ out_classes, int* __restrict__ counts) {
  const int b = blockIdx.x, lane = threadIdx.x;
  const float sx = img_params[b * 4 + 0], sy = img_params[b * 4 + 1];
  const float ow = img_params[b * 4 + 2], oh = img_params[b * 4 + 3];
  int base = 0;
  for (int k0 = 0; k0 < K; k0 += 64) {
    const int k = k0 + lane;
    bool keep = false;
    float x1 = 0, y1 = 0, x2 = 0, y2 = 0, sc = 0;
    int cl = 0;
    if (k < K && k < max_det) {
      const long o = (long)b * K + k;
      sc = scores[o];
      cl = classes[o];
      x1 = fminf(fmaxf(boxes[o * 4 + 0] * sx, 0.f), ow);
      y1 = fminf(fmaxf(boxes[o * 4 + 1] * sy, 0.f), oh);
      x2 = fminf(fmaxf(boxes[o * 4 + 2] * sx, 0.f), ow);
      y2 = fminf(fmaxf(boxes[o * 4 + 3] * sy, 0.f), oh);
      keep = sc > thresh && (x2 - x1) > 0.f && (y2 - y1) > 0.f;
    }
    const unsigned long long m = __ballot(keep);
    if (keep) {
      const int pos = base + __popcll(m & ((1ull << lane) - 1ull));
      const long o = (long)b * K + pos;
      out_boxes[o * 4 + 0] = x1; out_boxes[o * 4 + 1] = y1; out_boxes[o * 4 + 2] = x2; out_boxes[o * 4 + 3] = y2;
      out_scores[o] = sc;
      out_classes[o] = cl;
    }
    base += __popcll(m);
  }
  if (lane == 0) counts[b] = base;
}

int launch_postprocess(const float* boxes, const float* scores, const int* classes, int B, int K, int max_det,
                       float thresh, const float* img_params, float* out_boxes, float* out_scores, int* out_classes,
                       int* counts, hipStream_t s) {
  if (B == 0) return 0;
  hipLaunchKernelGGL(dec_postprocess_kernel, dim3(B), dim3(64), 0, s, boxes, scores, classes, K, max_det, thresh,
                     img_params, out_boxes, out_scores, out_classes, counts);
  CTDET_LAUNCH_CHECK();
  return 0;
}

static long dec_cap(int H, int W, int C, int K) {
  const DecGeom g = dec_geom(H, W, C);
  return (long)g.tiles_x * g.tiles_y * g.cchunks * (K - 1 + DEC_TILE_SLACK);
}
static long dec_ws_words(int H, int W, int C, int K) { return DEC_ST_WORDS + 2 * dec_cap(H, W, C, K); }

size_t decode_workspace_bytes(int B, int H, int W, int C, int K) {
  return (size_t)B * dec_ws_words(H, W, C, K) * sizeof(uint32_t);
}
int decode_status_words(int H, int W, int C, int K, long* ws_words, int* below_word) {
  *ws_words = dec_ws_words(H, W, C, K);
  *below_word = ST_BELOW_FLOOR;
  return ST_OVERFLOW;
}

int launch_decode(const DecArgs& a, bool flip, hipStream_t s) {
  CTDET_CHECK(a.C >= 1 && a.heat_stride >= a.C, "decode: C=%d / heat_stride=%d invalid", a.C, a.heat_stride);
  CTDET_CHECK(a.K >= 1 && a.K <= 1024 && a.K - 1 + DEC_CAP <= DEC_NCAND, "decode: K=%d out of range", a.K);
  CTDET_CHECK((long)a.C * a.H * a.W < (1L << 24), "decode: C*H*W too large for the 24-bit index field");
  CTDET_CHECK(((uintptr_t)a.heat & 15) == 0, "decode: heat must be 16-byte aligned");
  if (a.B == 0) return 0;
  const DecGeom g = dec_geom(a.H, a.W, a.C);
  const long words = dec_ws_words(a.H, a.W, a.C, a.K);
  const long cap = dec_cap(a.H, a.W, a.C, a.K);
  CTDET_CHECK(cap < (1L << 31), "decode: candidate list too large");
  const size_t tile_b = (size_t)(g.TH + 2) * (DEC_TW + 2) * g.CW * 4, list_b = (size_t)g.TH * DEC_TW * g.CW * 6;
  const size_t lds = DEC_HIST * 4 + (tile_b > list_b ? tile_b : list_b);
  CTDET_CHECK((DEC_TW + 2) * (g.CW / 4) <= DEC_TNT && g.CW <= 112, "decode: tile geometry");
  hipLaunchKernelGGL(dec_init_kernel, dim3(a.B), dim3(256), 0, s, a, words);
  const dim3 grid(g.tiles_x * g.tiles_y * g.cchunks, a.B);
#define DEC_TILE(TH_, FLIP_)                                                                                          \
  hipLaunchKernelGGL((dec_tile_kernel<TH_, FLIP_>), grid, dim3(DEC_TNT), lds, s, a, g.CW, g.tiles_x, g.tiles_y, words, \
                     (int)cap)
#define DEC_RUN(FLIP_)                                                                                       \
  do {                                                                                                       \
    switch (g.TH) {                                                                                          \
      case 8: DEC_TILE(8, FLIP_); break;                                                                     \
      case 4: DEC_TILE(4, FLIP_); break;                                                                     \
      case 2: DEC_TILE(2, FLIP_); break;                                                                     \
      default: DEC_TILE(1, FLIP_); break;                                                                    \
    }                                                                                                        \
    hipLaunchKernelGGL((dec_final_kernel<FLIP_>), dim3(a.B), dim3(1024), 0, s, a, words, (int)cap);          \
  } while (0)
  if (flip) DEC_RUN(true);
  else DEC_RUN(false);
#undef DEC_RUN
#undef DEC_TILE
  CTDET_LAUNCH_CHECK();
  return 0;
}
```

### detectron2-centernet_amd/modeling/meta_arch/centernet.py

```python
import numpy as np
import torch
from torch import nn

from ... import ops
from ...data.catalog import DatasetCatalog, MetadataCatalog
from ...layers import hipnn
from ...ops import ACT_NONE, ACT_RELU, ACT_SIGMOID_CLAMP, F16, F16X3, F32
from ...structures import Boxes, ImageList, Instances
from ..backbone import build_backbone
from .build import META_ARCH_REGISTRY

__all__ = ["CenterNet", "ctdet_decode"]


def fill_fc_weights(layers):
    for m in layers.modules():
        if isinstance(m, nn.Conv2d) and m.bias is not None:
            nn.init.constant_(m.bias, 0)


def ctdet_decode(heat, wh, reg=None, down_ratio=1, cat_spec_wh=False, K=100):
    if cat_spec_wh:
        raise NotImplementedError("cat_spec_wh is not used by any CenterNet config of the reference")
    if not heat.is_cuda:
        raise NotImplementedError("ctdet_decode runs on the HIP device only")
    h = heat.permute(0, 2, 3, 1).float().contiguous()
    w = wh.permute(0, 2, 3, 1).float().contiguous()
    r = reg.permute(0, 2, 3, 1).float().contiguous() if reg is not None else None
    boxes, scores, classes, _ = ops.decode(h, w, r, K, down_ratio)
    if heat.shape[0] == 1:
        return boxes[0], scores[0], classes[0]
    return boxes, scores, classes


MAX_ENGINES = 16
SIGMOID_CLAMP = (ops.SIGMOID_CLAMP_FLOOR, 1.0 - ops.SIGMOID_CLAMP_FLOOR)


def _engine_key(fused_base, B, H, W, Hp, Wp, img_dtype, flip=False):
    key = (B, Hp, Wp, img_dtype) if fused_base else (B, H, W, Hp, Wp, img_dtype)
    return key + ("flip",) if flip else key


class _EvalEngine:

    def __init__(self, model, B, H, W, Hp, Wp, img_dtype, use_graph=True, flip=False):
        import weakref
        self._model = weakref.ref(model)
        dev = model.device
        self.B, self.img_dtype, self.flip = B, img_dtype, bool(flip)
        NB = 2 * B if flip else B
        self._mirror = "both" if flip else False
        self.img_params = torch.zeros(B, 4, dtype=torch.float32, device=dev)
        self.fused_base = model.backbone_type == "dla34" and model.backbone.images_fusable(model._ctx, Hp, Wp)
        self.key = _engine_key(self.fused_base, B, H, W, Hp, Wp, img_dtype, flip)
        self.images = torch.zeros(B, 3, H, W, dtype=img_dtype, device=dev)
        self.border = int(getattr(model.backbone, "stem_border", 3))
        xch = 4 if (model._ctx.dtype == torch.float32 and model.backbone_type == "dla34") else 8
        self.xpad = None if self.fused_base else torch.zeros(NB, Hp + 2 * self.border, Wp + 2 * self.border, xch,
                                                             dtype=model._ctx.dtype, device=dev)
        self.l1 = torch.empty(NB, Hp // 2, Wp // 2, 32, dtype=model._ctx.dtype, device=dev) if self.fused_base else None
        self.l1p = torch.empty(NB, Hp // 4, Wp // 4, 32, dtype=model._ctx.dtype, device=dev) if self.fused_base else None
        self.graph = None
        self.Hp, self.Wp = Hp, Wp
        if self.fused_base:
            self._base(self.images)
        self._run()
        torch.cuda.synchronize()
        if use_graph:
            import gc
            gc.collect()
            gc_was_on = gc.isenabled()
            gc.disable()
            try:
                g = torch.cuda.CUDAGraph(keep_graph=True)
                with torch.cuda.graph(g):
                    self._run()
                from ...engine import graph_nodes
                self.graph_nodes = graph_nodes.inspect(g, "eval step") or {}
                g.instantiate()
            finally:
                if gc_was_on:
                    gc.enable()
            self.graph = g

    @property
    def model(self):
        m = self._model()
        if m is None:
            raise RuntimeError("the model of this eval engine no longer exists")
        return m

    def staging(self, H, W):
        if tuple(self.images.shape[2:]) != (H, W):
            assert self.fused_base, "this engine's graph reads a fixed-size image buffer"
            self.images = torch.zeros(self.B, 3, H, W, dtype=self.img_dtype, device=self.images.device)
        return self.images

    def _base(self, images):
        m = self.model
        m.backbone.base.base_level1(images, m._mean_host, m._std_host, self.Hp, self.Wp, out=self.l1, pooled=self.l1p,
                                    x3=m._ctx.compute == ops.F16X3, mirror=self._mirror)

    def _run(self):
        m = self.model
        if self.fused_base:
            self.out = m._network_outputs(None, apply_sigmoid=True, level1=(self.l1, self.l1p))
        else:
            x = ops.preprocess(self.images, m._mean_host, m._std_host, self.Hp, self.Wp, out=self.xpad, border=self.border,
                               mirror=self._mirror)
            self.out = m._network_outputs(x, apply_sigmoid=True, prepadded=self.border > 0)
        hm, wh, reg = self.out
        self.dec = ops.decode(hm, wh, reg, m.topk_candidates, m.backbone.down_ratio, heat_floor=ops.SIGMOID_CLAMP_FLOOR,
                              flip=self.flip)
        self.finite = ops.finite_flag(wh, reg).bool()

    def _post(self):
        m = self.model
        boxes, scores, classes, _ = self.dec
        max_det = min(m.max_detections_per_image, m.topk_candidates)
        boxes, scores, classes, counts = ops.postprocess(boxes, scores, classes, max_det, m.score_threshold, self.img_params)
        return boxes, scores, classes, torch.where(self.finite, counts, torch.full_like(counts, -1))

    def __call__(self, images=None):
        if self.fused_base:
            self._base(self.images if images is None else images)
        elif images is not None:
            self.images.copy_(images, non_blocking=True)
        if self.graph is not None:
            self.graph.replay()
        else:
            self._run()
        return self._post()


@META_ARCH_REGISTRY.register()
class CenterNet(nn.Module):
    def __init__(self, cfg):
        super().__init__()
        head_conv                     = cfg.MODEL.CENTERNET.HEAD_CONV
        final_kernel                  = cfg.MODEL.CENTERNET.FINAL_KERNEL
        backbone_type                 = cfg.MODEL.BACKBONE.NAME
        self.heads                    = dict(cfg.MODEL.CENTERNET.TASK)
        self.hm_weight                = cfg.MODEL.CENTERNET.HM_WEIGHT
        self.wh_weight                = cfg.MODEL.CENTERNET.WH_WEIGHT
        self.off_weight               = cfg.MODEL.CENTERNET.OFF_WEIGHT
        self.focal_loss_alpha         = list(cfg.MODEL.CENTERNET.FOCAL_LOSS_ALPHA)
        self.score_threshold          = cfg.MODEL.CENTERNET.SCORE_THRESH_TEST
        self.topk_candidates          = cfg.MODEL.CENTERNET.TOPK_CANDIDATES_TEST
        self.max_detections_per_image = cfg.TEST.DETECTIONS_PER_IMAGE
        precision                     = cfg.MODEL.CENTERNET.get("HIP_PRECISION", "f16")
        assert precision in ("f16", "f32", "f16x3"), precision
        self._ctx = hipnn.Ctx({"f16": F16, "f32": F32, "f16x3": F16X3}[precision])

        given_dataset = cfg.DATASETS.TRAIN[0]
        DatasetCatalog.get(given_dataset)
        self.meta = MetadataCatalog.get(given_dataset)
        self.num_classes = len(self.meta.thing_classes)
        self.heads["HM"] = self.num_classes
        self.register_buffer("pixel_mean", torch.Tensor(cfg.MODEL.PIXEL_MEAN).view(-1, 1, 1))
        self.register_buffer("pixel_std", torch.Tensor(cfg.MODEL.PIXEL_STD).view(-1, 1, 1))
        self._mean_host = [float(v) for v in cfg.MODEL.PIXEL_MEAN]
        self._std_host = [float(v) for v in cfg.MODEL.PIXEL_STD]

        self.backbone_type = backbone_type.split("_")[1]
        self.backbone = build_backbone(cfg)
        if self.backbone_type in ("resnet", "vovnet"):
            self.backbone.down_ratio = 4
            self.size_divisibility = 16
            self.deconv_feature = "res4" if self.backbone_type == "resnet" else "stage4"
            self.deconv_layers = self._make_deconv_layer(self.backbone._out_feature_channels[self.deconv_feature], 2,
                                                         [256, 256], [4, 4])
            cin, final_kernel = 256, 1
        elif self.backbone_type == "dla34":
            self.size_divisibility = self.backbone.size_divisibility
            cin = self.backbone.channels[self.backbone.first_level]
        else:
            raise NotImplementedError(f"backbone '{backbone_type}': DLA-34, ResNet and VoVNet are built (SURVEY.md 8(a), 8(f))")
        self.head_conv = head_conv
        for head in self.heads:
            classes = self.heads[head]
            if head_conv > 0:
                fc = nn.Sequential(
                    nn.Conv2d(cin, head_conv, kernel_size=3, padding=1, bias=True),
                    nn.ReLU(inplace=True),
                    nn.Conv2d(head_conv, classes, kernel_size=final_kernel, stride=1, padding=final_kernel // 2,
                              bias=True))
                if "hm" in head.lower():
                    fc[-1].bias.data.fill_(-2.19)
                else:
                    fill_fc_weights(fc)
            else:
                fc = nn.Conv2d(cin, classes, kernel_size=final_kernel, stride=1, padding=final_kernel // 2, bias=True)
                if "hm" in head.lower():
                    fc.bias.data.fill_(-2.19)
                else:
                    fill_fc_weights(fc)
            self.__setattr__(head.lower(), fc)
        if self.backbone_type == "resnet":
            self.init_weights()
        self._engines = {}
        self.use_hip_graph = True

    @staticmethod
    def _make_deconv_layer(inplanes, num_layers, num_filters, num_kernels):
        assert num_layers == len(num_filters) == len(num_kernels)
        layers = []
        for i in range(num_layers):
            planes = num_filters[i]
            layers.append(nn.ConvTranspose2d(inplanes, planes, kernel_size=num_kernels[i], stride=2, padding=1,
                                             output_padding=0, bias=False))
            layers.append(nn.BatchNorm2d(planes, momentum=0.1))
            layers.append(nn.ReLU(inplace=True))
            inplanes = planes
        return nn.Sequential(*layers)

    def init_weights(self):
        for m in self.deconv_layers.modules():
            if isinstance(m, nn.ConvTranspose2d):
                nn.init.normal_(m.weight, std=0.001)
            elif isinstance(m, nn.BatchNorm2d):
                nn.init.constant_(m.weight, 1)
                nn.init.constant_(m.bias, 0)
        for head in self.heads:
            for m in getattr(self, head.lower()).modules():
                if isinstance(m, nn.Conv2d) and m.weight.shape[0] == self.heads[head]:
                    if "hm" in head.lower():
                        nn.init.constant_(m.bias, -2.19)
                    else:
                        nn.init.normal_(m.weight, std=0.001)
                        nn.init.constant_(m.bias, 0)

    @property
    def device(self):
        return self.pixel_mean.device

    def load_state_dict(self, *args, **kwargs):
        self._engines = {}
        return super().load_state_dict(*args, **kwargs)

    def train(self, mode=True):
        if mode != self.training:
            self._engines = {}
        return super().train(mode)

    def _engine(self, B, H, W, Hp, Wp, img_dtype, flip=False):
        fused = self.backbone_type == "dla34" and self.backbone.images_fusable(self._ctx, Hp, Wp)
        key = _engine_key(fused, B, H, W, Hp, Wp, img_dtype, flip)
        eng = self._engines.get(key)
        if eng is not None:
            self._engines[key] = self._engines.pop(key)
            return eng
        while len(self._engines) >= MAX_ENGINES:
            old = self._engines.pop(next(iter(self._engines)))
            del old
        eng = self._engines[key] = _EvalEngine(self, B, H, W, Hp, Wp, img_dtype, self.use_hip_graph and not ops.RANGE_CHECK,
                                               flip=flip)
        return eng

    def _head_outputs(self, y, apply_sigmoid):
        ctx = self._ctx
        names = [h.lower() for h in self.heads]
        out = {}
        fused = (self.head_conv == ops.PackedHeads.HID and ctx.compute in (F16, F16X3) and ops.HEADS_FUSED
                 and ops.heads_fused_ok(y, ctx.compute) and len(names) <= 4
                 and all(getattr(self, n)[2].kernel_size == (1, 1) for n in names))
        if fused:
            fcs = [getattr(self, n) for n in names]
            acts = [ACT_SIGMOID_CLAMP if (apply_sigmoid and n == "hm") else ACT_NONE for n in names]
            cache = self.__dict__.setdefault("_ctdet_packed", {})
            ver = tuple((t.data_ptr(), t._version) for fc in fcs for t in (fc[0].weight, fc[0].bias, fc[2].weight, fc[2].bias))
            key = ("heads_fused", ctx.compute, tuple(acts))
            hit = cache.get(key)
            if hit is None or hit[0] != ver:
                ph = ops.PackedHeads([fc[0].weight for fc in fcs], [fc[0].bias for fc in fcs],
                                     [fc[2].weight for fc in fcs], [fc[2].bias for fc in fcs], acts, compute=ctx.compute)
                hit = cache[key] = (ver, ph)
            outs = ops.heads_fused(y, hit[1], clamp=SIGMOID_CLAMP)
            return dict(zip(names, outs))
        if self.head_conv > 0:
            convs = [getattr(self, n)[0] for n in names]
            w = torch.cat([c.weight for c in convs], 0)
            b = torch.cat([c.bias for c in convs], 0)
            p = self._packed_cat("heads3x3", w, b, convs, 1)
            hid = ops.conv2d(y, p, act=ACT_RELU)
            c0 = 0
            for n in names:
                fc = getattr(self, n)
                hs = hid[..., c0:c0 + self.head_conv]
                c0 += self.head_conv
                act = ACT_SIGMOID_CLAMP if (apply_sigmoid and n == "hm") else ACT_NONE
                out[n] = hipnn.conv_module(hs, fc[2], None, act, ctx=ctx, out_dtype=torch.float32,
                                           clamp=SIGMOID_CLAMP)
        else:
            for n in names:
                act = ACT_SIGMOID_CLAMP if (apply_sigmoid and n == "hm") else ACT_NONE
                out[n] = hipnn.conv_module(y, getattr(self, n), None, act, ctx=ctx, out_dtype=torch.float32,
                                           clamp=SIGMOID_CLAMP)
        return out

    def _packed_cat(self, key, w, b, convs, pad):
        cache = self.__dict__.setdefault("_ctdet_packed", {})
        ver = tuple((c.weight.data_ptr(), c.weight._version, c.bias._version) for c in convs)
        hit = cache.get((key, self._ctx.compute))
        if hit is not None and hit[0] == ver:
            return hit[1]
        p = ops.PackedConv(w, None, b, stride=1, pad=pad, compute=self._ctx.compute)
        cache[(key, self._ctx.compute)] = (ver, p)
        return p

    def _deconv_forward(self, y):
        mods = list(self.deconv_layers)
        for i in range(0, len(mods), 3):
            up, bn = mods[i], mods[i + 1]
            cache = up.__dict__.setdefault("_ctdet_packed", {})
            ver = hipnn._versions(up.weight, bn.weight, bn.bias, bn.running_mean, bn.running_var)
            slot = cache.get(self._ctx.compute)
            if slot is None or slot[0] != ver:
                slot = cache[self._ctx.compute] = (ver, {})
            scale, bias = hipnn.fold_bn(bn)
            y = ops.conv_transpose2d(y, up.weight, scale, bias, up.stride[0], up.padding[0], self._ctx.compute,
                                     act=ACT_RELU, cache=slot[1])
            if y.shape[3] != up.out_channels:
                y = y[..., :up.out_channels]
        return y

    def _network_outputs(self, x_nhwc, apply_sigmoid, prepadded=False, level1=None):
        if self.backbone_type in ("resnet", "vovnet"):
            y = self._deconv_forward(self.backbone.hip_forward(x_nhwc, self._ctx, prepadded)[self.deconv_feature])
        else:
            y = self.backbone.hip_forward(x_nhwc, self._ctx, prepadded, level1=level1)[-1]
        z = self._head_outputs(y, apply_sigmoid)
        hm = z["hm"]
        assert hm.shape[3] == self.num_classes or hm.shape[3] == ops.round_up(self.num_classes, 4)
        return hm[..., :self.num_classes] if hm.shape[3] != self.num_classes else hm, z["wh"][..., :2], z["reg"][..., :2]

    def forward(self, batched_inputs):
        if self.training:
            return self._forward_train(batched_inputs)
        return self._forward_eval(batched_inputs)

    def _forward_eval(self, batched_inputs, flip=False):
        dev = self.device
        if dev.type != "cuda":
            raise NotImplementedError("the CenterNet HIP path has no CPU implementation (MODEL.DEVICE must be cuda)")
        imgs = [x["image"] for x in batched_inputs]
        sizes = [tuple(im.shape[-2:]) for im in imgs]
        B = len(imgs)
        same = all(s == sizes[0] for s in sizes) and all(im.dtype == imgs[0].dtype for im in imgs)
        Hp, Wp = ImageList.padded_size(sizes, self.size_divisibility)
        if not same:
            return self._forward_eval_ragged(batched_inputs, imgs, sizes, Hp, Wp, flip)
        H, W = sizes[0]
        img_dtype = torch.uint8 if imgs[0].dtype == torch.uint8 else torch.float32
        eng = self._engine(B, H, W, Hp, Wp, img_dtype, flip)
        stage = eng.staging(H, W)
        for b, im in enumerate(imgs):
            stage[b].copy_(im if im.dtype == img_dtype else im.to(img_dtype), non_blocking=True)
        return self._finish_eval(eng, batched_inputs, sizes)

    def forward_async(self, batched_inputs, flip=False):
        assert not self.training
        imgs = [x["image"] for x in batched_inputs]
        sizes = [tuple(im.shape[-2:]) for im in imgs]
        if not (all(s == sizes[0] for s in sizes) and all(im.dtype == imgs[0].dtype for im in imgs)):
            return _Done(self._forward_eval(batched_inputs, flip))
        Hp, Wp = ImageList.padded_size(sizes, self.size_divisibility)
        H, W = sizes[0]
        img_dtype = torch.uint8 if imgs[0].dtype == torch.uint8 else torch.float32
        eng = self._engine(len(imgs), H, W, Hp, Wp, img_dtype, flip)
        stage = eng.staging(H, W)
        for b, im in enumerate(imgs):
            stage[b].copy_(im if im.dtype == img_dtype else im.to(img_dtype), non_blocking=True)
        return self._launch_eval(eng, batched_inputs, sizes)

    def infer_batch_tensor(self, images, out_sizes=None, flip=False):
        return self.infer_batch_tensor_async(images, out_sizes, flip).result()

    def infer_batch_tensor_async(self, images, out_sizes=None, flip=False):
        B, _, H, W = images.shape
        Hp, Wp = ImageList.padded_size([(H, W)], self.size_divisibility)
        img_dtype = torch.uint8 if images.dtype == torch.uint8 else torch.float32
        eng = self._engine(B, H, W, Hp, Wp, img_dtype, flip)
        if images.dtype != img_dtype or not images.is_contiguous():
            images = images.to(img_dtype).contiguous()
        inputs = [{} if out_sizes is None else {"height": out_sizes[b][0], "width": out_sizes[b][1]} for b in range(B)]
        return self._launch_eval(eng, inputs, [(H, W)] * B, images=images)

    def _finish_eval(self, eng, batched_inputs, sizes):
        return self._launch_eval(eng, batched_inputs, sizes).result()

    def _launch_eval(self, eng, batched_inputs, sizes, images=None):
        out_sizes = tuple((inp.get("height", size[0]), inp.get("width", size[1])) for inp, size in zip(batched_inputs, sizes))
        pkey = (out_sizes, tuple(sizes))
        if getattr(eng, "_params_key", None) != pkey:
            params = torch.tensor([[ow / size[1], oh / size[0], ow, oh] for (oh, ow), size in zip(out_sizes, sizes)],
                                  dtype=torch.float32)
            eng.img_params.copy_(params, non_blocking=False)
            eng._params_key = pkey
        boxes, scores, classes, counts = eng(images)
        return _EvalHandle(boxes, scores, classes, counts, out_sizes)

    def _forward_eval_ragged(self, batched_inputs, imgs, sizes, Hp, Wp, flip=False):
        dev, B = self.device, len(imgs)
        x = torch.zeros(2 * B if flip else B, Hp, Wp, 8, dtype=self._ctx.dtype, device=dev)
        for b, im in enumerate(imgs):
            im = im.to(dev)
            im = (im if im.dtype == torch.uint8 else im.float()).unsqueeze(0).contiguous()
            ops.preprocess(im, self._mean_host, self._std_host, Hp, Wp, out=x[b:b + 1], partial=True)
            if flip:
                ops.preprocess(im, self._mean_host, self._std_host, Hp, Wp, out=x[B + b:B + b + 1], partial=True, mirror=True)
        hm, wh, reg = self._network_outputs(x, apply_sigmoid=True)
        boxes, scores, classes, _ = ops.decode(hm, wh, reg, self.topk_candidates, self.backbone.down_ratio,
                                               heat_floor=ops.SIGMOID_CLAMP_FLOOR, flip=flip)
        params = torch.empty(B, 4, dtype=torch.float32)
        out_sizes = []
        for b, (inp, size) in enumerate(zip(batched_inputs, sizes)):
            oh, ow = inp.get("height", size[0]), inp.get("width", size[1])
            out_sizes.append((oh, ow))
            params[b, 0], params[b, 1], params[b, 2], params[b, 3] = ow / size[1], oh / size[0], ow, oh
        max_det = min(self.max_detections_per_image, self.topk_candidates)
        boxes, scores, classes, counts = ops.postprocess(boxes, scores, classes, max_det, self.score_threshold,
                                                         params.to(dev))
        counts = counts.tolist()
        results = []
        for b in range(B):
            r = Instances(out_sizes[b])
            r.pred_boxes = Boxes(boxes[b, :counts[b]])
            r.scores = scores[b, :counts[b]]
            r.pred_classes = classes[b, :counts[b]]
            results.append({"instances": r})
        return results

    def preprocess_image(self, batched_inputs, flip=False):
        dev = self.device
        imgs = [x["image"].to(dev) for x in batched_inputs]
        sizes = [tuple(im.shape[-2:]) for im in imgs]
        B = len(imgs)
        assert not (flip and self.training), "the flip test is an inference-time augmentation"
        Hp, Wp = ImageList.padded_size(sizes, self.size_divisibility)
        x = torch.zeros(2 * B if flip else B, Hp, Wp, 8, dtype=self._ctx.dtype, device=dev)
        for b, im in enumerate(imgs):
            im = (im if im.dtype == torch.uint8 else im.float()).unsqueeze(0).contiguous()
            ops.preprocess(im, self._mean_host, self._std_host, Hp, Wp, out=x[b:b + 1], partial=True)
            if flip:
                ops.preprocess(im, self._mean_host, self._std_host, Hp, Wp, out=x[B + b:B + b + 1], partial=True, mirror=True)
        images = ImageList(x[..., :3].permute(0, 3, 1, 2), sizes)
        images.nhwc = x
        if not self.training:
            return images, []
        targets = self.generate_targets([x["instances"] for x in batched_inputs], Hp // self.backbone.down_ratio,
                                        Wp // self.backbone.down_ratio)
        return images, targets

    def generate_targets(self, instances, out_h, out_w):
        dev = self.device
        B = len(instances)
        nmax = max(1, max(len(i) for i in instances))
        boxes = torch.zeros(B, nmax, 4, dtype=torch.float32)
        classes = torch.zeros(B, nmax, dtype=torch.int64)
        counts = torch.zeros(B, dtype=torch.int32)
        for b, inst in enumerate(instances):
            n = len(inst)
            counts[b] = n
            if n:
                boxes[b, :n] = inst.gt_boxes.tensor.detach().float().cpu()
                classes[b, :n] = inst.gt_classes.detach().cpu()
        return ops.gaussian_targets(boxes.to(dev), classes.to(dev), counts.to(dev), out_h, out_w, self.num_classes)

    def _alpha_tensor(self):
        a = list(self.focal_loss_alpha)
        C = self.num_classes
        if len(a) == 1:
            a = a * C
        elif len(a) != C:
            a = a + [1] * (C - len(a))
        key = (tuple(a), str(self.device))
        hit = self.__dict__.get("_alpha_cache")
        if hit is None or hit[0] != key:
            hit = self.__dict__["_alpha_cache"] = (key, torch.tensor(a, dtype=torch.float32, device=self.device))
        return hit[1]

    def losses(self, outputs, targets):
        hm, wh, reg = outputs
        hm_loss, _, _ = ops.focal_loss(hm.contiguous(), targets["hm"], self._alpha_tensor(), want_grad=False)
        wh_loss, _ = ops.reg_l1_loss(wh, targets["reg_mask"], targets["ind"], targets["wh"], want_grad=False)
        off_loss, _ = ops.reg_l1_loss(reg, targets["reg_mask"], targets["ind"], targets["reg"], want_grad=False)
        return {"hm_loss": hm_loss[0] * self.hm_weight, "wh_loss": wh_loss[0] * self.wh_weight,
# ... 73 lines not shown
```

### detectron2-centernet_amd/ops.py

```python
import ctypes as C
import os
import math

import torch

from . import _lib
from ._lib import (ACT_NONE, ACT_RELU, ACT_SIGMOID_CLAMP, DCN_MASK_LOGIT, DCN_MASK_NONE, DCN_MASK_PROB, F16, F16X3, F32, U8,
                   ConvDesc, HeadDesc)

_TORCH_DT = {F16: torch.float16, F32: torch.float32}

PROFILE_ON = False
PROFILE = []
PROFILE_REP = 5


class _Prof:
    def __init__(self, p, M, deform, out_dt, nsrc=1, flops=None):
        self.on = PROFILE_ON
        if self.on:
            _lib.lib().ctdet_set_label_mode(1)
            self.flops = flops if flops is not None else 2.0 * M * p.Cout * p.R * p.S * p.Cin_real
            osz = 2 if out_dt == F16 else 4
            if p is not None:
# ... 629 lines not shown
    return out


class PackedDlaBase:

    def __init__(self, w_stem, sb_stem, w_l0, sb_l0, w_l1, sb_l1):
        assert tuple(w_stem.shape) == (16, 3, 7, 7) and tuple(w_l0.shape) == (16, 16, 3, 3) and tuple(w_l1.shape) == (32, 16, 3, 3)
        dev = w_stem.device
        w4 = torch.zeros(16, 7, 8, 4, dtype=torch.float32, device=dev)
        w4[:, :, :7, :3] = w_stem.detach().float().permute(0, 2, 3, 1)
        self.w0 = w4.reshape(16, 224).to(torch.float16).contiguous()
        self.p1 = PackedConv(w_l0, sb_l0[0], sb_l0[1], stride=1, pad=1, compute=F16)
        self.p2 = PackedConv(w_l1, sb_l1[0], sb_l1[1], stride=2, pad=1, compute=F16)
        assert self.p1.korder == 0 and self.p1.Kpad == 160 and self.p2.korder == 0 and self.p2.Kpad == 160
        self.s0 = sb_stem[0].detach().float().contiguous()
        self.b0 = sb_stem[1].detach().float().contiguous()


class PackedDlaBaseX3:
    x3 = True

    def __init__(self, w_stem, sb_stem, w_l0, sb_l0, w_l1, sb_l1):
        assert tuple(w_stem.shape) == (16, 3, 7, 7) and tuple(w_l0.shape) == (16, 16, 3, 3) and tuple(w_l1.shape) == (32, 16, 3, 3)
        w4 = torch.zeros(16, 7, 8, 4, dtype=torch.float32, device=w_stem.device)
        w4[:, :, :7, :3] = w_stem.detach().float().permute(0, 2, 3, 1)
        self.p0 = PackedConv(w4.reshape(16, 224, 1, 1), sb_stem[0], sb_stem[1], compute=F16X3)
        self.p1 = PackedConv(w_l0.detach().float().contiguous(), sb_l0[0], sb_l0[1], stride=1, pad=1, compute=F16X3)
        self.p2 = PackedConv(w_l1.detach().float().contiguous(), sb_l1[0], sb_l1[1], stride=2, pad=1, compute=F16X3)
        for p, kpad, rows in ((self.p0, 224, 16), (self.p1, 144, 16), (self.p2, 144, 32)):
            assert p.korder == 0 and p.Kpad == kpad and p.w.shape[0] >= rows and p.w.shape[1] == kpad, (p.korder, p.Kpad, p.w.shape)
            assert p.scale.numel() >= rows and p.bias.numel() >= rows


BASE_FUSED = os.environ.get("CTDET_NO_FUSED_BASE", "0") != "1"


def dla_base_fused_ok(Hp, Wp):
    return BASE_FUSED and Hp % 16 == 0 and Wp % 32 == 0


def dla_base_fused(images, mean, std, Hp, Wp, p, out=None, pooled=None, mirror=False):
    _require_cuda(images, out, pooled)
    B, Cc, H, W = images.shape
    assert Cc == 3 and images.stride(3) == 1 and images.stride(2) == W and images.stride(1) == H * W
    B, mfrom = _mirror_from(mirror, B)
    x3 = getattr(p, "x3", False)
    odt = torch.float32 if x3 else torch.float16
    if out is None:
        out = torch.empty(B, Hp // 2, Wp // 2, 32, dtype=odt, device=images.device)
    assert out.dtype == odt and tuple(out.shape[:3]) == (B, Hp // 2, Wp // 2) and out.shape[3] >= 32
    d = _lib.DlaBaseDesc()
    d.B, d.H, d.W, d.Hp, d.Wp, d.img_dtype = B, H, W, Hp, Wp, dt_of(images)
    d.img_batch_stride = images.stride(0)
    for i in range(3):
        d.mean[i], d.std[i] = float(mean[i]), float(std[i])
    d.out_stride = _nhwc_stride(out)
    if pooled is not None:
        assert pooled.dtype == odt and tuple(pooled.shape[:3]) == (B, Hp // 4, Wp // 4) and pooled.shape[3] >= 32
        d.pool_stride = _nhwc_stride(pooled)
    px = B * Hp * Wp
    prof = _Prof(None, px, False, F16X3 if x3 else F16,
                 flops=2.0 * (px * 16 * 147 + px * 16 * 144 + (px // 4) * 32 * 144))
    L = _lib.lib()
    if x3:
        operands = (_ptr(images), _ptr(p.p0.w), _ptr(p.p0.scale), _ptr(p.p0.bias), _ptr(p.p1.w), _ptr(p.p1.scale),
                    _ptr(p.p1.bias), _ptr(p.p2.w), _ptr(p.p2.scale), _ptr(p.p2.bias), _ptr(out), _ptr(pooled), _stream())
        fn = L.ctdet_dla_base_x3_fwd if mfrom is None else L.ctdet_dla_base_x3_mirror_fwd
    else:
        operands = (_ptr(images), _ptr(p.w0), _ptr(p.s0), _ptr(p.b0), _ptr(p.p1.w), _ptr(p.p1.scale), _ptr(p.p1.bias),
                    _ptr(p.p2.w), _ptr(p.p2.scale), _ptr(p.p2.bias), _ptr(out), _ptr(pooled), _stream())
        fn = L.ctdet_dla_base_fwd if mfrom is None else L.ctdet_dla_base_mirror_fwd
    for _ in range(prof.reps()):
        rc = fn(C.byref(d), *operands) if mfrom is None else fn(C.byref(d), mfrom, *operands)
    _lib.check(rc, "ctdet_dla_base_fwd")
    if prof.on:
        prof.bytes = images.numel() * images.element_size() + (px // 4) * 32 * out.element_size() * (1.25 if pooled is not None else 1.0)
        prof.info = f"M={px} 3->16->16->32 fused"
    prof.done()
    return out


class PackedHeads:

    HID = 256

    def __init__(self, first_weights, first_biases, final_weights, final_biases, acts, compute=F16):
        n = len(first_weights)
        assert 1 <= n <= 4 and all(w.shape[0] == self.HID and tuple(w.shape[2:]) == (3, 3) for w in first_weights)
        assert all(tuple(w.shape[1:]) == (self.HID, 1, 1) for w in final_weights)
        assert compute in (F16, F16X3)
        dev = first_weights[0].device
        self.n, self.Cin, self.acts, self.compute = n, first_weights[0].shape[1], list(acts), compute
        w1 = torch.cat([w.detach().float() for w in first_weights], 0).contiguous()
        b1 = torch.cat([b.detach().float() for b in first_biases]).contiguous()
        self.couts = [w.shape[0] for w in final_weights]
        self.w2, self.b2 = [], []
        if compute == F16X3:
            assert self.Cin % 32 == 0, "f16x3 fused heads: Cin % 32 == 0"
            self.p1 = PackedConv(w1, None, b1, stride=1, pad=1, compute=F16X3)
            self.w1, self.s1 = self.p1._x3_operand(3)
            self.b1 = self.p1.bias
            for w, b in zip(final_weights, final_biases):
                c = w.shape[0]
                rows = round_up(c, 16)
                wp = torch.zeros(rows, self.HID, dtype=torch.float32, device=dev)
                wp[:c] = w.detach().reshape(c, self.HID).float()
                amax = wp.abs().amax(dim=1)
                e = torch.floor(torch.log2(amax.clamp_min(1e-30)))
                pw = torch.where(amax > 0, torch.exp2(10.0 - e), torch.ones_like(amax))
                ws = wp * pw[:, None]
                hi = ws.to(torch.float16)
                lo = (ws - hi.float()).to(torch.float16)
                self.w2.append(torch.stack([hi, lo], 1).contiguous())
                bp = torch.zeros(2, rows, dtype=torch.float32, device=dev)
                bp[0, :c] = b.detach().float()
                bp[1] = 1.0 / pw
                self.b2.append(bp)
            return
        self.p1 = PackedConv(w1, None, None, stride=1, pad=1, compute=F16)
        assert self.p1.korder == 1 and self.p1.Kpad == 9 * self.Cin
        self.b1 = b1
        for w, b in zip(final_weights, final_biases):
            c = w.shape[0]
            wp = torch.zeros(round_up(c, 16), self.HID, dtype=torch.float16, device=dev)
            wp[:c] = w.detach().reshape(c, self.HID).half()
            bp = torch.zeros(round_up(c, 16), dtype=torch.float32, device=dev)
            bp[:c] = b.detach().float()
            self.w2.append(wp)
            self.b2.append(bp)


def heads_fused_ok(x, compute):
    if compute not in (F16, F16X3) or x.dtype != _TORCH_DT[F16 if compute == F16 else F32] or (compute == F16X3 and RANGE_CHECK):
        return False
    _, H, W, Cin = x.shape
    return bool(_lib.lib().ctdet_head_fused_supported(compute, H, W, Cin, _nhwc_stride(x), _ptr(x)))


def heads_fused(x, ph, clamp=(0.0, 1.0), outs=None):
    _require_cuda(x)
    x3 = ph.compute == F16X3
    assert x.dtype == (torch.float32 if x3 else torch.float16) and x.shape[3] == ph.Cin
    B, H, W, _ = x.shape
    if outs is None:
        outs = [torch.empty(B, H, W, round_up(c, 4), dtype=torch.float32, device=x.device) for c in ph.couts]
    d = HeadDesc()
    d.nheads, d.B, d.H, d.W, d.Cin, d.in_stride = ph.n, B, H, W, ph.Cin, _nhwc_stride(x)
    for h in range(ph.n):
        d.w2[h], d.b2[h], d.y[h] = ph.w2[h].data_ptr(), ph.b2[h].data_ptr(), outs[h].data_ptr()
        d.y_stride[h], d.cout[h], d.act[h] = _nhwc_stride(outs[h]), ph.couts[h], ph.acts[h]
    d.clamp_lo, d.clamp_hi = clamp
    M = B * H * W
    prof = _Prof(None, M, False, F32, flops=sum(2.0 * M * PackedHeads.HID * (9 * ph.Cin + c) for c in ph.couts))
    for _ in range(prof.reps()):
        if x3:
            rc = _lib.lib().ctdet_head_fused_x3_fwd(C.byref(d), _ptr(x), _ptr(ph.w1), _ptr(ph.s1), _ptr(ph.b1), _stream())
        else:
            rc = _lib.lib().ctdet_head_fused_fwd(C.byref(d), _ptr(x), _ptr(ph.p1.w), _ptr(ph.b1), _stream())
    _lib.check(rc, "ctdet_head_fused_x3_fwd" if x3 else "ctdet_head_fused_fwd")
    prof.done()
    return outs


def maxpool3x3s2(x, out=None):
    _require_cuda(x, out)
    B, H, W, Cc = x.shape
    if out is None:
        out = torch.empty(B, (H - 1) // 2 + 1, (W - 1) // 2 + 1, Cc, dtype=x.dtype, device=x.device)
    rc = _lib.lib().ctdet_maxpool3x3s2(_ptr(x), _ptr(out), dt_of(x), B, H, W, Cc, _nhwc_stride(x), _nhwc_stride(out),
                                       _stream())
    _lib.check(rc, "ctdet_maxpool3x3s2")
    return out


def maxpool3x3s2_ceil(x, out=None):
    _require_cuda(x, out)
    B, H, W, Cc = x.shape
    Ho, Wo = -(-(H - 3) // 2) + 1, -(-(W - 3) // 2) + 1
    if (Ho - 1) * 2 >= H:
        Ho -= 1
    if (Wo - 1) * 2 >= W:
        Wo -= 1
    if out is None:
        out = torch.empty(B, Ho, Wo, Cc, dtype=x.dtype, device=x.device)
    assert tuple(out.shape[:3]) == (B, Ho, Wo)
    rc = _lib.lib().ctdet_maxpool3x3s2_ceil(_ptr(x), _ptr(out), dt_of(x), B, H, W, Cc, _nhwc_stride(x), _nhwc_stride(out),
                                            _stream())
    _lib.check(rc, "ctdet_maxpool3x3s2_ceil")
    return out


def finite_flag(*tensors):
    _require_cuda(*tensors)
    flag = torch.ones(1, dtype=torch.int32, device=tensors[0].device)
    for t in tensors:
        assert t.dtype == torch.float32 and t.dim() == 4 and t.stride(3) == 1
        B, H, W, Cc = t.shape
        _lib.check(_lib.lib().ctdet_finite_flag(_ptr(t), B * H * W, Cc, _nhwc_stride(t), _ptr(flag), _stream()), "ctdet_finite_flag")
    return flag


def global_avgpool(x):
    _require_cuda(x)
    B, H, W, Cc = x.shape
    out = torch.empty(B, Cc, dtype=torch.float32, device=x.device)
    rc = _lib.lib().ctdet_global_avgpool(_ptr(x), dt_of(x), B, H * W, Cc, _nhwc_stride(x), _ptr(out), _stream())
    _lib.check(rc, "ctdet_global_avgpool")
    return out


def ese_scale(x, s, identity=None, out=None):
    _require_cuda(x, s, identity, out)
    B, H, W, Cc = x.shape
    s = s.contiguous()
    assert s.dtype == torch.float32 and tuple(s.shape) == (B, Cc)
    if out is None:
        out = torch.empty(B, H, W, Cc, dtype=x.dtype, device=x.device)
    if identity is not None:
        assert identity.dtype == x.dtype and tuple(identity.shape) == tuple(x.shape)
    rc = _lib.lib().ctdet_ese_scale(_ptr(x), _nhwc_stride(x), _ptr(s), _ptr(identity),
                                    _nhwc_stride(identity) if identity is not None else 0, _ptr(out), _nhwc_stride(out),
                                    dt_of(x), B, H * W, Cc, _stream())
    _lib.check(rc, "ctdet_ese_scale")
    return out


def conv_transpose2d(x, weight, scale, bias, stride, padding, compute, act=ACT_NONE, cache=None):
    _require_cuda(x, weight)
    Cin, Cout, k, k2 = weight.shape
    assert k == k2 and x.shape[3] == Cin
    p = cache.get("p") if cache is not None else None
    if p is None:
        wc = weight.detach().flip(2, 3).permute(1, 0, 2, 3).contiguous()
        p = PackedConv(wc, scale, bias, stride=1, pad=k - 1 - padding, compute=compute, tap_major=True)
        if cache is not None:
            cache["p"] = p
    B, H, W, _ = x.shape
    Ho, Wo = (H - 1) * stride - 2 * padding + k, (W - 1) * stride - 2 * padding + k
    out = torch.empty(B, Ho, Wo, p.Cout_eff, dtype=x.dtype, device=x.device)
    p.in_dil = stride
    return conv2d(x, p, out=out, act=act)


def maxpool2x2(x, out=None):
    _require_cuda(x, out)
    B, H, W, Cc = x.shape
    if out is None:
        out = torch.empty(B, H // 2, W // 2, Cc, dtype=x.dtype, device=x.device)
    rc = _lib.lib().ctdet_maxpool2x2(_ptr(x), _ptr(out), dt_of(x), B, H, W, Cc, _nhwc_stride(x), _nhwc_stride(out),
                                     _stream())
    _lib.check(rc, "ctdet_maxpool2x2")
    return out


def _dw_weight(weight, Cc, f, fresh=False):
    if fresh:
        return weight.detach().reshape(Cc, 2 * f, 2 * f).to(torch.float32).permute(1, 2, 0).contiguous()
    hit = getattr(weight, "_ctdet_dw", None)
    if hit is None or hit[0] != (weight.data_ptr(), weight._version):
        packed = weight.detach().reshape(Cc, 2 * f, 2 * f).to(torch.float32).permute(1, 2, 0).contiguous()
        hit = ((weight.data_ptr(), weight._version), packed)
        try:
            weight._ctdet_dw = hit
        except AttributeError:
            pass
    return hit[1]


def dwconvT_add(x, weight, f, skip=None, out=None, fresh_weight=False, prepared=None):
    _require_cuda(x, weight, skip, out)
    B, H, W, Cc = x.shape
    w = prepared if prepared is not None else _dw_weight(weight, Cc, f, fresh_weight)
    if out is None:
        out = torch.empty(B, H * f, W * f, Cc, dtype=x.dtype, device=x.device)
    rc = _lib.lib().ctdet_dwconvT_add(_ptr(x), _ptr(w), _ptr(skip), _ptr(out), dt_of(x), B, H, W, Cc, f,
                                      _nhwc_stride(x), _nhwc_stride(skip) if skip is not None else 0,
                                      _nhwc_stride(out), _stream())
    _lib.check(rc, "ctdet_dwconvT_add")
    return out


def dw3_weight(weight, fresh=False):
    Cc = weight.shape[0]
    assert tuple(weight.shape) == (Cc, 1, 3, 3), f"depthwise 3x3 weight expected, got {tuple(weight.shape)}"
    if fresh:
        return weight.detach().reshape(Cc, 9).to(torch.float32).t().contiguous()
    hit = getattr(weight, "_ctdet_dw3", None)
    if hit is None or hit[0] != (weight.data_ptr(), weight._version):
        hit = ((weight.data_ptr(), weight._version), weight.detach().reshape(Cc, 9).to(torch.float32).t().contiguous())
        try:
            weight._ctdet_dw3 = hit
        except AttributeError:
            pass
    return hit[1]


def dwconv3x3(x, weight, stride, out=None, rot180=False, prepared=None):
    _require_cuda(x, weight, out)
    B, H, W, Cc = x.shape
    w = prepared if prepared is not None else dw3_weight(weight)
    assert w.shape == (9, Cc) and w.dtype == torch.float32 and w.is_contiguous()
    Ho, Wo = (H - 1) // stride + 1, (W - 1) // stride + 1
    if out is None:
        out = torch.empty(B, Ho, Wo, Cc, dtype=x.dtype, device=x.device)
    assert tuple(out.shape) == (B, Ho, Wo, Cc) and out.dtype == x.dtype
    with prof_region(f"dwconv3x3<s{stride}>", flops=2.0 * 9 * B * Ho * Wo * Cc,
                     nbytes=float(x.element_size() * (B * H * W + B * Ho * Wo) * Cc), info=f"{H}x{W} C={Cc}"):
        rc = _lib.lib().ctdet_dwconv3x3_fwd(_ptr(x), _nhwc_stride(x), _ptr(w), _ptr(out), _nhwc_stride(out), B, H, W, Cc,
                                            stride, int(rot180), dt_of(x), _stream())
    _lib.check(rc, "ctdet_dwconv3x3_fwd")
    return out


class DecodeWorkspace:

    def __init__(self, B, H, W, Cc, K, device):
        n = _lib.lib().ctdet_decode_workspace_bytes(B, H, W, Cc, K)
        self.key = (B, H, W, Cc, K)
        self.buf = torch.empty(n // 4, dtype=torch.int32, device=device)


SIGMOID_CLAMP_FLOOR = 1e-4


def decode(heat, wh, reg, K, down_ratio, workspace=None, check_status=False, heat_floor=0.0, flip=False):
    _require_cuda(heat, wh, reg)
    assert heat.dtype == torch.float32
    B, H, W, Cc = heat.shape
    if flip:
        assert B % 2 == 0 and wh.shape[0] == B and (reg is None or reg.shape[0] == B), "flip decode: 2B images, plain half first"
        assert heat.stride(0) == H * W * heat.stride(2) and wh.stride(0) == H * W * wh.stride(2), "flip decode: dense batches"
        B //= 2
    if workspace is None or workspace.key != (B, H, W, Cc, K):
        workspace = DecodeWorkspace(B, H, W, Cc, K, heat.device)
    dev = heat.device
    boxes = torch.empty(B, K, 4, dtype=torch.float32, device=dev)
    scores = torch.empty(B, K, dtype=torch.float32, device=dev)
    classes = torch.empty(B, K, dtype=torch.int32, device=dev)
    inds = torch.empty(B, K, dtype=torch.int32, device=dev)
    with prof_region("decode", nbytes=float(B * H * W * Cc * 4), info=f"{B}x{H}x{W}x{Cc} K={K}"):
        fn = _lib.lib().ctdet_decode_flip if flip else _lib.lib().ctdet_decode
        rc = fn(_ptr(heat), _nhwc_stride(heat), _ptr(wh), _nhwc_stride(wh), _ptr(reg),
                _nhwc_stride(reg) if reg is not None else 0, B, H, W, Cc, K, float(down_ratio),
                float(heat_floor), _ptr(workspace.buf), _ptr(boxes), _ptr(scores), _ptr(classes), _ptr(inds), _stream())
    _lib.check(rc, "ctdet_decode")
    if check_status:
        _lib.check(_lib.lib().ctdet_decode_status(_ptr(workspace.buf), B, H, W, Cc, K, _stream()), "ctdet_decode_status")
    return boxes, scores, classes, inds


def postprocess(boxes, scores, classes, max_det, score_thresh, img_params):
    _require_cuda(boxes, scores, classes, img_params)
    B, K = scores.shape
    ob, os_, oc = torch.empty_like(boxes), torch.empty_like(scores), torch.empty_like(classes)
    counts = torch.empty(B, dtype=torch.int32, device=boxes.device)
    rc = _lib.lib().ctdet_postprocess(_ptr(boxes), _ptr(scores), _ptr(classes), B, K, int(max_det), float(score_thresh),
                                      _ptr(img_params), _ptr(ob), _ptr(os_), _ptr(oc), _ptr(counts), _stream())
    _lib.check(rc, "ctdet_postprocess")
    return ob, os_, oc, counts


def gaussian_targets(boxes, classes, counts, H, W, num_classes, hm=None):
    _require_cuda(boxes, classes, counts)
    B, Nmax, _ = boxes.shape
    dev = boxes.device
    assert boxes.dtype == torch.float32 and classes.dtype == torch.int64 and counts.dtype == torch.int32
    boxes, classes = boxes.contiguous(), classes.contiguous()
    if hm is None:
        hm = torch.empty(B, H, W, num_classes, dtype=torch.float32, device=dev)
    wh = torch.empty(B, 128, 2, dtype=torch.float32, device=dev)
    reg = torch.empty(B, 128, 2, dtype=torch.float32, device=dev)
    ind = torch.empty(B, 128, dtype=torch.int64, device=dev)
    reg_mask = torch.empty(B, 128, dtype=torch.uint8, device=dev)
    rc = _lib.lib().ctdet_gaussian_targets(_ptr(boxes), _ptr(classes), _ptr(counts), B, Nmax, H, W, num_classes,
                                           _ptr(hm), _ptr(wh), _ptr(reg), _ptr(ind), _ptr(reg_mask), _stream())
    _lib.check(rc, "ctdet_gaussian_targets")
    return {"hm": hm, "wh": wh, "reg": reg, "ind": ind, "reg_mask": reg_mask}


def gaussian_radius(hw_pairs):
    _require_cuda(hw_pairs)
    n = hw_pairs.shape[0]
    r = torch.empty(n, dtype=torch.float64, device=hw_pairs.device)
    ri = torch.empty(n, dtype=torch.int32, device=hw_pairs.device)
    rc = _lib.lib().ctdet_gaussian_radius(_ptr(hw_pairs.contiguous()), n, _ptr(r), _ptr(ri), _stream())
    _lib.check(rc, "ctdet_gaussian_radius")
    return r, ri


def focal_loss(logits, gt, alpha, want_grad=True, grad_scale=1.0):
    _require_cuda(logits, gt, alpha)
    assert logits.is_contiguous() and gt.is_contiguous() and logits.shape == gt.shape
    B, H, W, Cc = logits.shape
    dev = logits.device
    ws = torch.empty(_lib.lib().ctdet_focal_loss_workspace_bytes(logits.numel()) // 4, dtype=torch.float32, device=dev)
    loss = torch.empty(1, dtype=torch.float32, device=dev)
    stats = torch.empty(4, dtype=torch.float32, device=dev)
    grad = torch.empty_like(logits) if want_grad else None
    rc = _lib.lib().ctdet_focal_loss(_ptr(logits), _ptr(gt), _ptr(alpha), B, H, W, Cc, float(grad_scale), _ptr(ws),
                                     _ptr(loss), _ptr(stats), _ptr(grad), _stream())
    _lib.check(rc, "ctdet_focal_loss")
    return loss, stats, grad


def reg_l1_loss(pred, mask, ind, target, want_grad=True, grad_scale=1.0, grad=None):
    _require_cuda(pred, mask, ind, target)
    B, H, W, _ = pred.shape
    N = mask.shape[1]
    dev = pred.device
    loss = torch.empty(1, dtype=torch.float32, device=dev)
    if want_grad and grad is None:
        grad = torch.zeros(B, H, W, 2, dtype=torch.float32, device=dev)
    rc = _lib.lib().ctdet_reg_l1_loss(_ptr(pred), _nhwc_stride(pred), _ptr(mask.contiguous()), _ptr(ind.contiguous()),
                                      _ptr(target.contiguous()), B, N, H * W, float(grad_scale), _ptr(loss),
                                      _ptr(grad) if want_grad else C.c_void_p(0),
                                      _nhwc_stride(grad) if want_grad else 0, _stream())
    _lib.check(rc, "ctdet_reg_l1_loss")
    return loss, grad


def sgd_momentum_(param, grad, buf, lr_dev, momentum, weight_decay, first_step):
    _require_cuda(param, grad, buf, lr_dev)
    assert param.is_contiguous() and grad.is_contiguous() and buf.is_contiguous()
    rc = _lib.lib().ctdet_sgd_momentum(_ptr(param), _ptr(grad), _ptr(buf), param.numel(), _ptr(lr_dev),
                                       float(momentum), float(weight_decay), int(bool(first_step)), _stream())
    _lib.check(rc, "ctdet_sgd_momentum")


def sgd_momentum_runs_(param, grad, buf, run_end, run_lr_index, run_wd, lr_table, momentum, first_step):
    _require_cuda(param, grad, buf, run_end, run_lr_index, run_wd, lr_table)
    assert param.is_contiguous() and grad.is_contiguous() and buf.is_contiguous()
    assert run_end.dtype == torch.int64 and run_lr_index.dtype == torch.int32
    rc = _lib.lib().ctdet_sgd_momentum_runs(_ptr(param), _ptr(grad), _ptr(buf), param.numel(), _ptr(run_end),
                                            _ptr(run_lr_index), _ptr(run_wd), _ptr(lr_table), run_end.numel(),
                                            float(momentum), int(bool(first_step)), _stream())
    _lib.check(rc, "ctdet_sgd_momentum_runs")


def grad_chunk_norms_(grad, chunk_start, chunk_len, norm_type, partials):
    _require_cuda(grad, chunk_start, chunk_len, partials)
    assert grad.is_contiguous() and grad.dtype == torch.float32 and partials.dtype == torch.float32
    assert chunk_start.dtype == torch.int64 and chunk_len.dtype == torch.int32
    assert chunk_start.numel() == chunk_len.numel() == partials.numel()
    rc = _lib.lib().ctdet_grad_chunk_norms(_ptr(grad), grad.numel(), _ptr(chunk_start), _ptr(chunk_len), chunk_start.numel(),
                                           int(norm_type), _ptr(partials), _stream())
    _lib.check(rc, "ctdet_grad_chunk_norms")


def grad_clip_coefs_(partials, param_chunk_end, norm_type, clip_value, norms, coefs):
    _require_cuda(partials, param_chunk_end, norms, coefs)
    assert param_chunk_end.dtype == torch.int32 and norms.dtype == coefs.dtype == torch.float32
    assert param_chunk_end.numel() == norms.numel() == coefs.numel()
    rc = _lib.lib().ctdet_grad_clip_coefs(_ptr(partials), _ptr(param_chunk_end), param_chunk_end.numel(), partials.numel(),
                                          int(norm_type), float(clip_value), _ptr(norms), _ptr(coefs), _stream())
    _lib.check(rc, "ctdet_grad_clip_coefs")


def sgd_momentum_runs_clip_(param, grad, buf, run_end, run_lr_index, run_wd, lr_table, momentum, first_step, nesterov=False,
                            clip_type=_lib.CLIP_NONE, clip_value=0.0, coefs=None):
    _require_cuda(param, grad, buf, run_end, run_lr_index, run_wd, lr_table)
    assert param.is_contiguous() and grad.is_contiguous() and buf.is_contiguous()
    assert run_end.dtype == torch.int64 and run_lr_index.dtype == torch.int32
    if clip_type == _lib.CLIP_NORM:
        _require_cuda(coefs)
        assert coefs.dtype == torch.float32 and coefs.numel() == run_end.numel()
    else:
        coefs = None
    rc = _lib.lib().ctdet_sgd_momentum_runs_clip(_ptr(param), _ptr(grad), _ptr(buf), param.numel(), _ptr(run_end),
                                                 _ptr(run_lr_index), _ptr(run_wd), _ptr(lr_table), run_end.numel(),
                                                 float(momentum), int(bool(first_step)), int(bool(nesterov)), int(clip_type),
                                                 float(clip_value), _ptr(coefs), _stream())
    _lib.check(rc, "ctdet_sgd_momentum_runs_clip")


def adam_advance_(step_count, bias, beta1, beta2):
    _require_cuda(step_count, bias)
    assert step_count.dtype == torch.int64 and step_count.numel() == 1
    assert bias.dtype == torch.float32 and bias.numel() == 2 and bias.is_contiguous()
    rc = _lib.lib().ctdet_adam_advance(_ptr(step_count), _ptr(bias), float(beta1), float(beta2), _stream())
    _lib.check(rc, "ctdet_adam_advance")


def adam_runs_(param, grad, exp_avg, exp_avg_sq, max_exp_avg_sq, run_end, run_lr_index, run_wd, lr_table, bias, beta1, beta2,
               eps, decoupled=False, amsgrad=False, clip_type=_lib.CLIP_NONE, clip_value=0.0, coefs=None):
    _require_cuda(param, grad, exp_avg, exp_avg_sq, run_end, run_lr_index, run_wd, lr_table, bias)
    state = [param, grad, exp_avg, exp_avg_sq]
    if amsgrad:
        _require_cuda(max_exp_avg_sq)
        state.append(max_exp_avg_sq)
    else:
        max_exp_avg_sq = None
    assert all(t.is_contiguous() and t.dtype == torch.float32 and t.numel() == param.numel() for t in state)
    assert run_end.dtype == torch.int64 and run_lr_index.dtype == torch.int32
    assert bias.dtype == torch.float32 and bias.numel() == 2
    if clip_type == _lib.CLIP_NORM:
# ... 10 lines not shown
```

### include/ctdet_hip.h

```cpp
#ifndef CTDET_HIP_H
#define CTDET_HIP_H
#include <stddef.h>
#include <stdint.h>
#ifdef __cplusplus
extern "C" {
#endif

enum ctdet_dtype { CTDET_DT_F16 = 0, CTDET_DT_F32 = 1, CTDET_DT_U8 = 2, CTDET_DT_F16X3 = 3 };
enum ctdet_act { CTDET_AC_NONE = 0, CTDET_AC_RELU = 1, CTDET_AC_SIGMOID_CLAMP = 2 };

typedef struct ctdet_conv_desc {
  int32_t B, H, W, Cin, in_stride;
  int32_t Cout, Ho, Wo, out_stride;
  int32_t R, S, stride, pad, dil;
  int32_t Kpad, Cout_pad;
  int32_t compute_dtype, out_dtype;
  int32_t act;
  int32_t res_stride;
  float clamp_lo, clamp_hi;
  int32_t korder;
  int32_t in_dil;
} ctdet_conv_desc;

const char* ctdet_last_error(void);
int32_t ctdet_abi_version(void);
enum ctdet_tuning {
  CTDET_TUNING_NO_HALO = 1, CTDET_TUNING_NO_WIN = 2, CTDET_TUNING_DCN_MIXED = 4, CTDET_TUNING_NO_WGRAD_WINDOW = 8,
  CTDET_TUNING_NO_COL2IM_WINDOW = 16, CTDET_TUNING_NO_F32_DCN_WINDOW = 32,
  CTDET_TUNING_DCN_WINDOW_V1 = 64, CTDET_TUNING_NO_SMALL_GRID_TILES = 128
};
int32_t ctdet_set_tuning_flags(uint32_t flags);
uint32_t ctdet_get_tuning_flags(void);
int32_t ctdet_conv_cout_tile(int32_t cout);

int32_t     ctdet_set_label_mode(int32_t mode);
const char* ctdet_last_kernel_label(void);

int32_t ctdet_conv_pair_supported(const ctdet_conv_desc* d, const void* x);

int32_t ctdet_split_weights(const float* w_packed_f32, void* w_split, int64_t n, void* stream);

int32_t ctdet_conv2d_fwd(const ctdet_conv_desc* d, const void* x, const void* w_packed, const float* scale,
                         const float* bias, const void* residual, void* y, void* stream);

int32_t ctdet_conv1x1_cat_fwd(const ctdet_conv_desc* d, const void* const* xs, const int32_t* cins,
                              const int32_t* strides, int32_t nsrc, const void* w_packed, const float* scale,
                              const float* bias, const void* residual, void* y, void* stream);

enum ctdet_dcn_mask { CTDET_DCN_MASK_LOGIT = 0, CTDET_DCN_MASK_PROB = 1, CTDET_DCN_MASK_NONE = 2 };

int32_t ctdet_dcnv2_fwd(const ctdet_conv_desc* d, const void* x, const float* offset_mask, int32_t om_stride,
                        int32_t mask_is_prob, const void* w_packed, const float* scale, const float* bias, void* y, void* stream);

int32_t ctdet_dcnv2_cols_supported(const ctdet_conv_desc* d, const void* x, const void* y);
int32_t ctdet_dcnv2_fwd_cols(const ctdet_conv_desc* d, const void* x, const float* offset_mask, int32_t om_stride,
                             int32_t mask_is_prob, const void* w_packed, const float* scale, const float* bias, void* y,
                             float* cols_out, void* stream);

int32_t ctdet_dcnv2_offset_supported(const ctdet_conv_desc* d);
int32_t ctdet_dcnv2_offset_fwd(const ctdet_conv_desc* d, const void* x, const void* w_off_packed, const float* b_off,
                               float* om_out, int32_t om_out_stride, const void* w_packed, const float* scale,
                               const float* bias, void* y, void* stream);

int32_t ctdet_preprocess(const void* img, int32_t img_dtype, void* out, int32_t out_dtype, int32_t B, int32_t H,
                         int32_t W, int32_t Hp, int32_t Wp, int64_t img_batch_stride, const float* mean3,
                         const float* std3, int32_t out_stride, int32_t border, void* stream);
int32_t ctdet_preprocess_mirror(const void* img, int32_t img_dtype, void* out, int32_t out_dtype, int32_t B, int32_t H,
                                int32_t W, int32_t Hp, int32_t Wp, int64_t img_batch_stride, const float* mean3,
                                const float* std3, int32_t out_stride, int32_t border, int32_t mirror_from, void* stream);

typedef struct ctdet_head_desc {
  int32_t nheads, B, H, W, Cin, in_stride;
  const void* w2[4];
  const void* b2[4];
  void* y[4];
  int32_t y_stride[4], cout[4], act[4];
  float clamp_lo, clamp_hi;
} ctdet_head_desc;
int32_t ctdet_head_fused_fwd(const ctdet_head_desc* d, const void* x, const void* w1, const float* b1, void* stream);
int32_t ctdet_head_fused_x3_fwd(const ctdet_head_desc* d, const void* x, const void* w1, const float* s1, const float* b1,
                                void* stream);
int32_t ctdet_head_fused_supported(int32_t compute_dtype, int32_t H, int32_t W, int32_t Cin, int32_t in_stride, const void* x);

typedef struct ctdet_dla_base_desc {
  int32_t B, H, W, Hp, Wp, img_dtype;
  int64_t img_batch_stride;
  float mean[3], std[3];
  int32_t out_stride;
  int32_t pool_stride;
} ctdet_dla_base_desc;
int32_t ctdet_dla_base_fwd(const ctdet_dla_base_desc* d, const void* images, const void* w_stem, const float* scale_stem,
                           const float* bias_stem, const void* w_l0, const float* scale_l0, const float* bias_l0,
                           const void* w_l1, const float* scale_l1, const float* bias_l1, void* out, void* pooled,
                           void* stream);
int32_t ctdet_dla_base_x3_fwd(const ctdet_dla_base_desc* d, const void* images, const void* w_stem, const float* scale_stem,
                              const float* bias_stem, const void* w_l0, const float* scale_l0, const float* bias_l0,
                              const void* w_l1, const float* scale_l1, const float* bias_l1, float* out, float* pooled,
                              void* stream);
int32_t ctdet_dla_base_mirror_fwd(const ctdet_dla_base_desc* d, int32_t mirror_from, const void* images, const void* w_stem,
                                  const float* scale_stem, const float* bias_stem, const void* w_l0, const float* scale_l0,
                                  const float* bias_l0, const void* w_l1, const float* scale_l1, const float* bias_l1,
                                  void* out, void* pooled, void* stream);
int32_t ctdet_dla_base_x3_mirror_fwd(const ctdet_dla_base_desc* d, int32_t mirror_from, const void* images,
                                     const void* w_stem, const float* scale_stem, const float* bias_stem, const void* w_l0,
                                     const float* scale_l0, const float* bias_l0, const void* w_l1, const float* scale_l1,
                                     const float* bias_l1, float* out, float* pooled, void* stream);

int32_t ctdet_maxpool2x2(const void* x, void* y, int32_t dtype, int32_t B, int32_t H, int32_t W, int32_t C,
                         int32_t in_stride, int32_t out_stride, void* stream);

int32_t ctdet_maxpool3x3s2(const void* x, void* y, int32_t dtype, int32_t B, int32_t H, int32_t W, int32_t C,
                           int32_t in_stride, int32_t out_stride, void* stream);
int32_t ctdet_maxpool3x3s2_ceil(const void* x, void* y, int32_t dtype, int32_t B, int32_t H, int32_t W, int32_t C,
                                int32_t in_stride, int32_t out_stride, void* stream);
int32_t ctdet_global_avgpool(const void* x, int32_t dtype, int32_t B, int32_t HW, int32_t C, int32_t stride, float* out,
                             void* stream);
int32_t ctdet_finite_flag(const float* x, int64_t M, int32_t C, int32_t stride, int32_t* flag, void* stream);
int32_t ctdet_ese_scale(const void* x, int32_t x_stride, const float* s, const void* identity, int32_t identity_stride,
                        void* y, int32_t y_stride, int32_t dtype, int32_t B, int32_t HW, int32_t C, void* stream);

int32_t ctdet_pack_weights(const float* w, void* packed, int32_t O, int32_t I, int32_t R, int32_t S, int32_t chans_pad,
                           int32_t rows_pad, int32_t Kpad, int32_t korder, int32_t transposed, void* stream);
typedef struct ctdet_pack_desc {
  const float* w; void* packed;
  int32_t O, I, R, S, chans_pad, rows_pad, Kpad, korder, transposed, blk0;
} ctdet_pack_desc;
int32_t ctdet_pack_weights_batch(const ctdet_pack_desc* table_dev, int32_t n, int32_t total_blocks, void* stream);

int32_t ctdet_pack_weights_x3(const float* w, void* packed, float* scale_out, int32_t O, int32_t I, int32_t R, int32_t S,
                              int32_t chans_pad, int32_t rows_pad, int32_t Kpad, int32_t layout, int32_t transposed,
                              int32_t scale_n, void* stream);
typedef struct ctdet_pack3_desc {
  const float* w; void* packed; float* scale_out;
  int32_t O, I, R, S, chans_pad, rows_pad, Kpad, layout, transposed, scale_n, blk0, pad_;
} ctdet_pack3_desc;
int32_t ctdet_pack_weights_x3_batch(const ctdet_pack3_desc* table_dev, int32_t n, int32_t total_blocks, void* stream);

int32_t ctdet_dwconvT_add(const void* x, const float* w, const void* skip, void* y, int32_t dtype, int32_t B,
                          int32_t H, int32_t W, int32_t C, int32_t f, int32_t in_stride, int32_t skip_stride,
                          int32_t out_stride, void* stream);

size_t ctdet_decode_workspace_bytes(int32_t B, int32_t H, int32_t W, int32_t C, int32_t K);
int32_t ctdet_decode(const float* heat, int32_t heat_stride, const float* wh, int32_t wh_stride, const float* reg,
                     int32_t reg_stride, int32_t B, int32_t H, int32_t W, int32_t C, int32_t K, float down_ratio,
                     float heat_floor, void* workspace, float* boxes, float* scores, int32_t* classes, int32_t* inds,
                     void* stream);
int32_t ctdet_decode_flip(const float* heat, int32_t heat_stride, const float* wh, int32_t wh_stride, const float* reg,
                          int32_t reg_stride, int32_t B, int32_t H, int32_t W, int32_t C, int32_t K, float down_ratio,
                          float heat_floor, void* workspace, float* boxes, float* scores, int32_t* classes, int32_t* inds,
                          void* stream);
int32_t ctdet_postprocess(const float* boxes, const float* scores, const int32_t* classes, int32_t B, int32_t K,
                          int32_t max_det, float score_thresh, const float* img_params, float* out_boxes,
                          float* out_scores, int32_t* out_classes, int32_t* counts, void* stream);
int32_t ctdet_decode_status(const void* workspace, int32_t B, int32_t H, int32_t W, int32_t C, int32_t K, void* stream);

int32_t ctdet_gaussian_targets(const float* boxes, const int64_t* classes, const int32_t* counts, int32_t B,
                               int32_t Nmax, int32_t H, int32_t W, int32_t C, float* hm, float* wh, float* reg,
                               int64_t* ind, uint8_t* reg_mask, void* stream);
int32_t ctdet_gaussian_radius(const int32_t* hw_pairs, int32_t n, double* out_radius, int32_t* out_int, void* stream);

size_t ctdet_focal_loss_workspace_bytes(int64_t numel);
int32_t ctdet_focal_loss(const float* logits, const float* gt, const float* alpha, int32_t B, int32_t H, int32_t W,
                         int32_t C, float grad_scale, void* workspace, float* loss, float* stats, float* grad,
                         void* stream);

int32_t ctdet_reg_l1_loss(const float* pred, int32_t pred_stride, const uint8_t* mask, const int64_t* ind,
                          const float* target, int32_t B, int32_t N, int32_t HW, float grad_scale, float* loss,
                          float* grad, int32_t grad_stride, void* stream);

int32_t ctdet_sgd_momentum(float* param, const float* grad, float* momentum_buf, int64_t n, const float* lr_dev,
                           float momentum, float weight_decay, int32_t first_step, void* stream);

int32_t ctdet_sgd_momentum_runs(float* param, const float* grad, float* momentum_buf, int64_t n, const int64_t* run_end,
                                const int32_t* run_lr_index, const float* run_weight_decay, const float* lr_table,
                                int32_t nruns, float momentum, int32_t first_step, void* stream);

enum ctdet_sgd_clip { CTDET_CLIP_NONE = 0, CTDET_CLIP_VALUE = 1, CTDET_CLIP_NORM = 2 };
enum ctdet_grad_norm { CTDET_NORM_L1 = 1, CTDET_NORM_L2 = 2, CTDET_NORM_INF = 3 };

int32_t ctdet_grad_chunk_norms(const float* grad, int64_t n, const int64_t* chunk_start, const int32_t* chunk_len,
                               int32_t nchunks, int32_t norm_type, float* partials, void* stream);

int32_t ctdet_grad_clip_coefs(const float* partials, const int32_t* param_chunk_end, int32_t nparams, int32_t nchunks,
                              int32_t norm_type, float clip_value, float* norms, float* coefs, void* stream);

int32_t ctdet_sgd_momentum_runs_clip(float* param, const float* grad, float* momentum_buf, int64_t n, const int64_t* run_end,
                                     const int32_t* run_lr_index, const float* run_weight_decay, const float* lr_table,
                                     int32_t nruns, float momentum, int32_t first_step, int32_t nesterov, int32_t clip_type,
                                     float clip_value, const float* coefs, void* stream);

int32_t ctdet_adam_advance(int64_t* step_dev, float* bias_dev, double beta1, double beta2, void* stream);

int32_t ctdet_adam_runs(float* param, const float* grad, float* exp_avg, float* exp_avg_sq, float* max_exp_avg_sq, int64_t n,
                        const int64_t* run_end, const int32_t* run_lr_index, const float* run_weight_decay,
                        const float* lr_table, int32_t nruns, const float* bias_dev, double beta1, double beta2, double eps,
                        int32_t decoupled, int32_t amsgrad, int32_t clip_type, float clip_value, const float* coefs,
                        void* stream);


size_t ctdet_chan_workspace_bytes(int32_t C);
int32_t ctdet_bn_train_fwd(const void* y, int32_t y_stride, const void* res, int32_t res_stride, void* z,
                           int32_t z_stride, int32_t M, int32_t C, const float* gamma, const float* beta, float eps,
                           float momentum, float* running_mean, float* running_var, float* save_mean,
                           float* save_invstd, float* scale, float* shift, void* workspace, int32_t relu, int32_t dtype,
                           void* stream);
int32_t ctdet_bn_train_bwd(const void* dz, int32_t dz_stride, const void* z, int32_t z_stride, const void* y,
                           int32_t y_stride, const float* mean, const float* invstd, const float* scale, int32_t M,
                           int32_t C, int32_t relu, void* dy, int32_t dy_stride, void* dres, int32_t dres_stride,
                           float* dgamma, float* dbeta, float grad_mult, void* workspace, int32_t dtype, void* stream);
int32_t ctdet_bn_local_stats(const void* y, int32_t y_stride, int32_t M, int32_t C, int32_t rank, int32_t world,
                             double* stats, void* workspace, int32_t dtype, void* stream);
int32_t ctdet_bn_sync_fwd(const void* y, int32_t y_stride, const void* res, int32_t res_stride, void* z, int32_t z_stride,
                          int32_t M, int32_t C, const double* stats, int32_t world, const float* gamma, const float* beta,
                          float eps, float momentum, float* running_mean, float* running_var, float* save_mean,
                          float* save_invstd, float* scale, float* shift, int32_t relu, int32_t dtype, void* stream);
int32_t ctdet_bn_local_grad_sums(const void* dz, int32_t dz_stride, const void* z, int32_t z_stride, const void* y,
                                 int32_t y_stride, const float* mean, const float* invstd, int32_t M, int32_t C, int32_t relu,
                                 int32_t rank, int32_t world, double* sums, float* dgamma, float* dbeta, float grad_mult,
                                 void* workspace, int32_t dtype, void* stream);
int32_t ctdet_bn_sync_bwd(const void* dz, int32_t dz_stride, const void* z, int32_t z_stride, const void* y, int32_t y_stride,
                          const float* mean, const float* invstd, const float* scale, const double* stats,
                          const double* sums, int32_t world, int32_t M, int32_t C, int32_t relu, void* dy, int32_t dy_stride,
                          void* dres, int32_t dres_stride, int32_t dtype, void* stream);
int32_t ctdet_conv_wgrad(const ctdet_conv_desc* d, const void* x, const void* dy, float* dw, float scale, void* stream);
int32_t ctdet_conv_wgrad_oihw(const ctdet_conv_desc* d, const void* x, const void* dy, float* dw, float scale, int32_t taps,
                              int32_t cin_k, int32_t cin_real, int32_t cout_real, void* stream);
int32_t ctdet_grad_scatter_oihw(const void* const* src, void* const* dst, const int32_t* cout, const int32_t* cin_real,
                                const int32_t* cin_k, const int32_t* taps, int32_t n, void* stream);
int32_t ctdet_depth_to_space2(const void* src, int32_t src_stride, void* dst, int32_t dst_stride, int32_t B, int32_t H,
                              int32_t W, int32_t C, int32_t Hs, int32_t Ws, int32_t dtype, void* stream);
int32_t ctdet_maxpool3x3s2_bwd(const void* x, int32_t x_stride, const void* dz, int32_t dz_stride, void* dx, int32_t dx_stride,
                               int32_t dtype, int32_t B, int32_t H, int32_t W, int32_t C, int32_t ceil_nopad, void* stream);
int32_t ctdet_ese_dot(const void* dy, int32_t dy_stride, const void* x, int32_t x_stride, int32_t dtype, int32_t B, int32_t HW,
                      int32_t C, float* out, void* stream);
// ... 48 lines not shown
```

Baseline: 3943 images/s.

## Evaluate wh/reg heads only at top-K peak locations after heatmap decode

The hm head now runs densely on its own. Decode runs first without wh/reg, then a new sparse MFMA kernel evaluates the 3x3 conv, the 256-wide hidden layer and the 1x1 wh/reg heads only at the K selected peaks, with flip averaging, and writes the boxes directly. This removes the dense wh/reg head evaluation over every output pixel, a large share of head FLOPs and bandwidth. The dense outputs remain available lazily through a property, at the cost of a new kernel path and extra launch ordering.

```diff
diff --git a/detectron2-centernet_amd/_lib.py b/detectron2-centernet_amd/_lib.py
--- a/detectron2-centernet_amd/_lib.py
+++ b/detectron2-centernet_amd/_lib.py
@@ -38,6 +38,7 @@
     "ctdet_preprocess_mirror": (_i32, [_vp, _i32, _vp, _i32, _i32, _i32, _i32, _i32, _i32, _i64, _vp, _vp, _i32, _i32, _i32, _vp]),
     "ctdet_head_fused_fwd": (_i32, [_vp, _vp, _vp, _vp, _vp]),
     "ctdet_head_fused_x3_fwd": (_i32, [_vp, _vp, _vp, _vp, _vp, _vp]),
+    "ctdet_head_sparse_x3_fwd": (_i32, [_vp, _vp, _vp, _vp, _vp, _vp, _i32, _f32, _i32, _vp, _vp, _vp]),
     "ctdet_dla_base_fwd": (_i32, [_vp] * 14),
     "ctdet_dla_base_x3_fwd": (_i32, [_vp] * 14),
     "ctdet_dla_base_mirror_fwd": (_i32, [_vp, _i32] + [_vp] * 13),
diff --git a/detectron2-centernet_amd/csrc/api.hip b/detectron2-centernet_amd/csrc/api.hip
--- a/detectron2-centernet_amd/csrc/api.hip
+++ b/detectron2-centernet_amd/csrc/api.hip
@@ -369,6 +369,18 @@
   return launch_head_fused_x3(a, (hipStream_t)stream);
 }
 
+int32_t ctdet_head_sparse_x3_fwd(const ctdet_head_desc* d, const void* x, const void* w1, const float* s1, const float* b1,
+                                 const int32_t* inds, int32_t K, float down_ratio, int32_t flip, float* whreg, float* boxes,
+                                 void* stream) {
+  CTDET_CHECK(d && x && w1 && s1 && b1 && inds && whreg && boxes, "head_sparse_x3: null pointer");
+  CTDET_CHECK(d->nheads == 2 && d->w2[0] && d->w2[1] && d->b2[0] && d->b2[1], "head_sparse_x3: a two-head (wh, reg) pack");
+  HeadArgs a = {};
+  a.x = x; a.w1 = w1; a.s1 = s1; a.b1 = b1;
+  a.nheads = 2; a.B = d->B; a.H = d->H; a.W = d->W; a.Cin = d->Cin; a.in_stride = d->in_stride;
+  for (int h = 0; h < 2; ++h) { a.w2[h] = d->w2[h]; a.b2[h] = (const float*)d->b2[h]; a.cout[h] = d->cout[h]; }
+  return launch_head_sparse_x3(a, inds, whreg, boxes, K, down_ratio, flip != 0, (hipStream_t)stream);
+}
+
 static int32_t dla_base_entry(const ctdet_dla_base_desc* d, int mirror_from, const void* images, const void* w_stem,
                               const float* scale_stem, const float* bias_stem, const void* w_l0, const float* scale_l0,
                               const float* bias_l0, const void* w_l1, const float* scale_l1, const float* bias_l1,
@@ -553,7 +565,8 @@
                             const float* reg, int32_t reg_stride, int32_t B, int32_t H, int32_t W, int32_t C, int32_t K,
                             float down_ratio, float heat_floor, void* workspace, float* boxes, float* scores,
                             int32_t* classes, int32_t* inds, void* stream) {
-  CTDET_CHECK(heat && wh && workspace && boxes && scores && classes, "decode: null pointer");
+  CTDET_CHECK(heat && workspace && scores && classes, "decode: null pointer");
+  CTDET_CHECK(wh ? boxes != nullptr : (inds != nullptr && !reg), "decode: %s", wh ? "null boxes" : "without wh: inds required, reg must be null");
   CTDET_CHECK(B >= 0 && H > 0 && W > 0, "decode: bad shape B=%d H=%d W=%d", B, H, W);
   CTDET_CHECK(heat_floor >= 0.f && heat_floor < 1.f, "decode: heat_floor %g outside [0, 1)", (double)heat_floor);
   DecArgs a;
diff --git a/detectron2-centernet_amd/csrc/common.h b/detectron2-centernet_amd/csrc/common.h
--- a/detectron2-centernet_amd/csrc/common.h
+++ b/detectron2-centernet_amd/csrc/common.h
@@ -135,4 +135,6 @@
 int launch_conv_f16(const ConvArgs& a, int out_dtype, bool deform, hipStream_t s);
 int launch_head_fused(const HeadArgs& a, hipStream_t s);
 int launch_head_fused_x3(const HeadArgs& a, hipStream_t s);
+int launch_head_sparse_x3(const HeadArgs& a, const int* inds, float* whreg, float* boxes, int K, float down_ratio, bool flip,
+                          hipStream_t s);
 int launch_conv_f32(const ConvArgs& a, bool deform, bool split, hipStream_t s);
diff --git a/detectron2-centernet_amd/csrc/conv_igemm.hip b/detectron2-centernet_amd/csrc/conv_igemm.hip
--- a/detectron2-centernet_amd/csrc/conv_igemm.hip
+++ b/detectron2-centernet_amd/csrc/conv_igemm.hip
@@ -1566,6 +1566,214 @@
   CTDET_KERNEL(TW == 32 ? "head_fused_x3_kernel<256x256,f16x3>" : "head_fused_x3_kernel<16x16x256,f16x3>");
   if (TW == 32) hipLaunchKernelGGL(head_fused_x3_kernel<32>, grid, dim3(256), 0, s, a);
   else hipLaunchKernelGGL(head_fused_x3_kernel<16>, grid, dim3(256), 0, s, a);
+  CTDET_LAUNCH_CHECK();
+  return 0;
+}
+
+struct HeadSparseArgs {
+  const float* x;
+  const void* w1;
+  const float *s1, *b1;
+  const void* w2[2];
+  const float* b2[2];
+  const int* inds;
+  float* whreg;
+  float* boxes;
+  int B, K, H, W, in_stride;
+  float down_ratio;
+};
+
+template <bool FLIP>
+__global__ void __launch_bounds__(256, 2) head_sparse_x3_kernel(const HeadSparseArgs a) {
+  constexpr int CIN = 64, HID = 256, NSTEP = CIN / 32 * 9, KROW = CIN / 32 * 288;
+  constexpr int PPW = FLIP ? 16 : 32;
+  constexpr int FRAG = NSTEP * 1024;
+  __shared__ __attribute__((aligned(16))) char sH[2 * FRAG];
+  __shared__ __attribute__((aligned(16))) char sL[2 * FRAG];
+  __shared__ int s_ind[32];
+  __shared__ float s_part[4][2][32][2];
+  const int tid = threadIdx.x, lane = tid & 63, wave = __builtin_amdgcn_readfirstlane(tid >> 6);
+  const int l15 = lane & 15, q = lane >> 4;
+  const int P = a.B * a.K, HW = a.H * a.W;
+  const int p0 = blockIdx.x * PPW;
+
+  if (tid < 32) {
+    const int p = p0 + (FLIP ? (tid & 15) : tid);
+    int ind = -1;
+    if (p < P) ind = min(max(a.inds[p], 0), HW - 1);
+    s_ind[tid] = ind;
+  }
+  __syncthreads();
+
+  for (int it = tid; it < 32 * 9 * 16; it += 256) {
+    const int kg = it & 3, c = (it >> 2) & 3, T = (it >> 4) % 9, e = (it >> 4) / 9;
+    const int ind = s_ind[e];
+    f32x4 v = (f32x4){0.f, 0.f, 0.f, 0.f};
+    if (ind >= 0) {
+      const int p = p0 + (FLIP ? (e & 15) : e);
+      int b = p / a.K, px = ind % a.W;
+      const int py = ind / a.W;
+      if (FLIP && e >= 16) { b += a.B; px = a.W - 1 - px; }
+      const int yy = py + T / 3 - 1, xx = px + T % 3 - 1;
+      if (yy >= 0 && yy < a.H && xx >= 0 && xx < a.W)
+        v = *(const f32x4*)(a.x + ((long)b * HW + (long)yy * a.W + xx) * a.in_stride + c * 16 + kg * 4);
+    }
+    const f16x4 hi = __builtin_convertvector(v, f16x4);
+    f32x4 r;
+#pragma unroll
+    for (int j = 0; j < 4; ++j) r[j] = v[j] - (float)hi[j];
+    const f16x4 lo = __builtin_convertvector(r, f16x4);
+    const int ab = c & 1;
+    const int S = T == 8 ? 4 : (ab ? 5 : 0) + (T >> 1), op = T == 8 ? ab : (T & 1);
+    const int off = (((e >> 4) * NSTEP + (c >> 1) * 9 + S) * 16 + (e & 15)) * 64 + kg * 16 + op * 8;
+    *(f16x4*)(sH + off) = hi;
+    *(f16x4*)(sL + off) = lo;
+  }
+  __syncthreads();
+
+  const char* fragH = sH + l15 * 64 + q * 16;
+  const char* fragL = sL + l15 * 64 + q * 16;
+  bool late[2];
+#pragma unroll
+  for (int t = 0; t < 2; ++t) {
+    const int y = max(s_ind[t * 16 + l15], 0) / a.W;
+    late[t] = a.W % 32 == 0 ? (y & 1) != 0 : (y & 3) >= 2;
+  }
+#pragma unroll 1
+  for (int h = 0; h < 2; ++h) {
+    const int cbase = h * HID + wave * 64;
+    const char* wrow = (const char*)a.w1 + ((long)(cbase + 8 * (l15 >> 2) + (l15 & 3)) * KROW) * 4 + q * 16;
+    f32x4 acc[2][2][2], acb[2][2][2];
+#pragma unroll
+    for (int i = 0; i < 8; ++i) acc[i >> 2][(i >> 1) & 1][i & 1] = acb[i >> 2][(i >> 1) & 1][i & 1] = (f32x4){0.f, 0.f, 0.f, 0.f};
+#pragma unroll 6
+    for (int st = 0; st < NSTEP; ++st) {
+      f16x8 H[2], L[2];
+#pragma unroll
+      for (int t = 0; t < 2; ++t) {
+        H[t] = *(const f16x8*)(fragH + t * FRAG + st * 1024);
+        L[t] = *(const f16x8*)(fragL + t * FRAG + st * 1024);
+      }
+#pragma unroll
+      for (int hb = 0; hb < 2; ++hb)
+#pragma unroll
+        for (int half = 0; half < 2; ++half) {
+          const char* wp = wrow + ((long)(hb * 32 + half * 4) * KROW) * 4 + st * 128;
+          const f16x8 X = *(const f16x8*)wp, Y = *(const f16x8*)(wp + 64);
+#pragma unroll
+          for (int t = 0; t < 2; ++t) {
+            acc[hb][half][t] = __builtin_amdgcn_mfma_f32_16x16x32_f16(X, H[t], acc[hb][half][t], 0, 0, 0);
+            acb[hb][half][t] = __builtin_amdgcn_mfma_f32_16x16x32_f16(X, L[t], acb[hb][half][t], 0, 0, 0);
+          }
+#pragma unroll
+          for (int t = 0; t < 2; ++t) {
+            acc[hb][half][t] = __builtin_amdgcn_mfma_f32_16x16x32_f16(Y, H[t], acc[hb][half][t], 0, 0, 0);
+            acb[hb][half][t] = __builtin_amdgcn_mfma_f32_16x16x32_f16(X, H[t], acb[hb][half][t], 0, 0, 0);
+          }
+#pragma unroll
+          for (int t = 0; t < 2; ++t) {
+            acc[hb][half][t] = __builtin_amdgcn_mfma_f32_16x16x32_f16(X, L[t], acc[hb][half][t], 0, 0, 0);
+            acb[hb][half][t] = __builtin_amdgcn_mfma_f32_16x16x32_f16(Y, H[t], acb[hb][half][t], 0, 0, 0);
+          }
+        }
+    }
+#pragma unroll
+    for (int i = 0; i < 8; ++i)
+      if (late[i & 1]) acc[i >> 2][(i >> 1) & 1][i & 1] = acb[i >> 2][(i >> 1) & 1][i & 1];
+    const f16* w2 = (const f16*)a.w2[h];
+    f32x4 o[2] = {(f32x4){0.f, 0.f, 0.f, 0.f}, (f32x4){0.f, 0.f, 0.f, 0.f}};
+#pragma unroll
+    for (int hb = 0; hb < 2; ++hb) {
+      const int c0 = cbase + hb * 32 + q * 8;
+      const f32x4 sa = *(const f32x4*)(a.s1 + c0), sb = *(const f32x4*)(a.s1 + c0 + 4);
+      const f32x4 ba = *(const f32x4*)(a.b1 + c0), bb = *(const f32x4*)(a.b1 + c0 + 4);
+      const f16* w2row = w2 + (long)l15 * (2 * HID) + wave * 64 + hb * 32 + q * 8;
+      const f16x8 X = *(const f16x8*)w2row, Y = *(const f16x8*)(w2row + HID);
+      f16x8 hf[2], lf[2];
+#pragma unroll
+      for (int t = 0; t < 2; ++t) {
+        const f32x4 v0 = acc[hb][0][t] * sa + ba, v1 = acc[hb][1][t] * sb + bb;
+#pragma unroll
+        for (int j = 0; j < 8; ++j) {
+          const float hv = fmaxf(j < 4 ? v0[j] : v1[j - 4], 0.f);
+          hf[t][j] = (f16)hv;
+          lf[t][j] = (f16)(hv - (float)hf[t][j]);
+        }
+      }
+#pragma unroll
+      for (int t = 0; t < 2; ++t) o[t] = __builtin_amdgcn_mfma_f32_16x16x32_f16(X, hf[t], o[t], 0, 0, 0);
+#pragma unroll
+      for (int t = 0; t < 2; ++t) o[t] = __builtin_amdgcn_mfma_f32_16x16x32_f16(Y, hf[t], o[t], 0, 0, 0);
+#pragma unroll
+      for (int t = 0; t < 2; ++t) o[t] = __builtin_amdgcn_mfma_f32_16x16x32_f16(X, lf[t], o[t], 0, 0, 0);
+    }
+    if (q == 0) {
+#pragma unroll
+      for (int t = 0; t < 2; ++t) {
+        s_part[wave][h][t * 16 + l15][0] = o[t][0];
+        s_part[wave][h][t * 16 + l15][1] = o[t][1];
+      }
+    }
+  }
+  __syncthreads();
+
+  if (tid < PPW && p0 + tid < P) {
+    const int ind = s_ind[tid];
+    float val[2][2][2];
+#pragma unroll
+    for (int t = 0; t < (FLIP ? 2 : 1); ++t)
+#pragma unroll
+      for (int h = 0; h < 2; ++h)
+#pragma unroll
+        for (int j = 0; j < 2; ++j) {
+          const int e = FLIP ? t * 16 + tid : tid;
+          float v = s_part[0][h][e][j];
+          v = v + s_part[1][h][e][j];
+          v = v + s_part[2][h][e][j];
+          v = v + s_part[3][h][e][j];
+          val[t][h][j] = v * a.b2[h][16 + j] + a.b2[h][j];
+        }
+    const int x = ind % a.W, y = ind / a.W;
+    float xs = (float)x, ys = (float)y;
+    xs = xs + val[0][1][0]; ys = ys + val[0][1][1];
+    const float w0 = val[0][0][0], h0 = val[0][0][1];
+    float wm = w0, hm = h0;
+    if constexpr (FLIP) {
+      wm = (w0 + val[1][0][0]) * 0.5f;
+      hm = (h0 + val[1][0][1]) * 0.5f;
+    }
+    const float w = wm, h = hm;
+    const long o = p0 + tid;
+    *(f32x4*)(a.whreg + o * 4) = (f32x4){w, h, val[0][1][0], val[0][1][1]};
+    f32x4 box;
+    box[0] = (xs - w / 2) * a.down_ratio;
+    box[1] = (ys - h / 2) * a.down_ratio;
+    box[2] = (xs + w / 2) * a.down_ratio;
+    box[3] = (ys + h / 2) * a.down_ratio;
+    *(f32x4*)(a.boxes + o * 4) = box;
+  }
+}
+
+int launch_head_sparse_x3(const HeadArgs& h, const int* inds, float* whreg, float* boxes, int K, float down_ratio, bool flip,
+                          hipStream_t s) {
+  CTDET_CHECK(h.nheads == 2 && h.cout[0] == 2 && h.cout[1] == 2, "head_sparse_x3: a pack of the wh and reg heads (2 + 2 outputs)");
+  CTDET_CHECK(h.Cin == 64 && h.in_stride % 4 == 0 && h.in_stride >= 64 && (((size_t)h.x) & 15) == 0,
+              "head_sparse_x3: needs a 64-channel f32 map, 16-byte aligned (Cin=%d, stride %d)", h.Cin, h.in_stride);
+  CTDET_CHECK(((((size_t)h.w1) | (size_t)h.s1 | (size_t)h.b1 | (size_t)h.w2[0] | (size_t)h.w2[1] | (size_t)h.b2[0] |
+                (size_t)h.b2[1] | (size_t)whreg | (size_t)boxes) & 15) == 0, "head_sparse_x3: misaligned operand");
+  CTDET_CHECK(h.B >= 0 && K >= 1 && h.H >= 1 && h.W >= 1 && (long)h.B * K < (1L << 28) &&
+                  (long)h.B * (flip ? 2 : 1) * h.H * h.W * h.in_stride < (1L << 40),
+              "head_sparse_x3: bad shape B=%d K=%d %dx%d", h.B, K, h.H, h.W);
+  if (h.B == 0) return 0;
+  HeadSparseArgs a = {};
+  a.x = (const float*)h.x; a.w1 = h.w1; a.s1 = h.s1; a.b1 = h.b1;
+  for (int i = 0; i < 2; ++i) { a.w2[i] = h.w2[i]; a.b2[i] = h.b2[i]; }
+  a.inds = inds; a.whreg = whreg; a.boxes = boxes;
+  a.B = h.B; a.K = K; a.H = h.H; a.W = h.W; a.in_stride = h.in_stride; a.down_ratio = down_ratio;
+  const int P = h.B * K, ppw = flip ? 16 : 32;
+  CTDET_KERNEL(flip ? "head_sparse_x3_kernel<16 peaks x 2,f16x3,flip>" : "head_sparse_x3_kernel<32 peaks,f16x3>");
+  if (flip) hipLaunchKernelGGL(head_sparse_x3_kernel<true>, dim3((P + ppw - 1) / ppw), dim3(256), 0, s, a);
+  else hipLaunchKernelGGL(head_sparse_x3_kernel<false>, dim3((P + ppw - 1) / ppw), dim3(256), 0, s, a);
   CTDET_LAUNCH_CHECK();
   return 0;
 }
diff --git a/detectron2-centernet_amd/csrc/decode.hip b/detectron2-centernet_amd/csrc/decode.hip
--- a/detectron2-centernet_amd/csrc/decode.hip
+++ b/detectron2-centernet_amd/csrc/decode.hip
@@ -414,24 +414,26 @@
       ind = (int)(canon % HW);
       if ((uint32_t)k - n < nfloor) score = __uint_as_float(a.floor_bits);
     }
-    const int x = ind % a.W, y = ind / a.W;
-    const long pix = (long)b * HW + ind;
-    float xs = (float)x, ys = (float)y;
-    if (a.reg) { xs = xs + a.reg[pix * a.reg_stride]; ys = ys + a.reg[pix * a.reg_stride + 1]; }
-    else { xs += 0.5f; ys += 0.5f; }
-    const float w0 = a.wh[pix * a.wh_stride], h0 = a.wh[pix * a.wh_stride + 1];
-    float wm = w0, hm = h0;
-    if constexpr (FLIP) {
-      const long mpix = (long)(b + a.B) * HW + (ind - x) + (a.W - 1 - x);
-      wm = (w0 + a.wh[mpix * a.wh_stride]) * 0.5f;
-      hm = (h0 + a.wh[mpix * a.wh_stride + 1]) * 0.5f;
-    }
-    const float w = wm, h = hm;
     const long o = (long)b * a.K + k;
-    a.boxes[o * 4 + 0] = (xs - w / 2) * a.down_ratio;
-    a.boxes[o * 4 + 1] = (ys - h / 2) * a.down_ratio;
-    a.boxes[o * 4 + 2] = (xs + w / 2) * a.down_ratio;
-    a.boxes[o * 4 + 3] = (ys + h / 2) * a.down_ratio;
+    if (a.wh) {
+      const int x = ind % a.W, y = ind / a.W;
+      const long pix = (long)b * HW + ind;
+      float xs = (float)x, ys = (float)y;
+      if (a.reg) { xs = xs + a.reg[pix * a.reg_stride]; ys = ys + a.reg[pix * a.reg_stride + 1]; }
+      else { xs += 0.5f; ys += 0.5f; }
+      const float w0 = a.wh[pix * a.wh_stride], h0 = a.wh[pix * a.wh_stride + 1];
+      float wm = w0, hm = h0;
+      if constexpr (FLIP) {
+        const long mpix = (long)(b + a.B) * HW + (ind - x) + (a.W - 1 - x);
+        wm = (w0 + a.wh[mpix * a.wh_stride]) * 0.5f;
+        hm = (h0 + a.wh[mpix * a.wh_stride + 1]) * 0.5f;
+      }
+      const float w = wm, h = hm;
+      a.boxes[o * 4 + 0] = (xs - w / 2) * a.down_ratio;
+      a.boxes[o * 4 + 1] = (ys - h / 2) * a.down_ratio;
+      a.boxes[o * 4 + 2] = (xs + w / 2) * a.down_ratio;
+      a.boxes[o * 4 + 3] = (ys + h / 2) * a.down_ratio;
+    }
     a.scores[o] = score;
     a.classes[o] = cls;
     if (a.inds) a.inds[o] = ind;
diff --git a/detectron2-centernet_amd/modeling/meta_arch/centernet.py b/detectron2-centernet_amd/modeling/meta_arch/centernet.py
--- a/detectron2-centernet_amd/modeling/meta_arch/centernet.py
+++ b/detectron2-centernet_amd/modeling/meta_arch/centernet.py
@@ -102,15 +102,39 @@
         m.backbone.base.base_level1(images, m._mean_host, m._std_host, self.Hp, self.Wp, out=self.l1, pooled=self.l1p,
                                     x3=m._ctx.compute == ops.F16X3, mirror=self._mirror)
 
+    @property
+    def out(self):
+        if self._out is None:
+            m = self.model
+            z = ops.heads_fused(self._y, m._packed_heads(["wh", "reg"], True), clamp=SIGMOID_CLAMP)
+            self._out = (self._hm, z[0][..., :2], z[1][..., :2])
+        return self._out
+
+    def _run_sparse(self, y):
+        m = self.model
+        K, dr = m.topk_candidates, m.backbone.down_ratio
+        self._y, self._out = y, None
+        self._hm = m._hm_view(m._head_outputs(y, True, only=("hm",))["hm"])
+        _, scores, classes, inds = ops.decode(self._hm, None, None, K, dr, heat_floor=ops.SIGMOID_CLAMP_FLOOR, flip=self.flip)
+        self.whreg, boxes = ops.heads_sparse(y, m._packed_heads(["wh", "reg"], True), inds, dr, flip=self.flip)
+        self.dec = (boxes, scores, classes, inds)
+        self.finite = ops.finite_flag(self.whreg.view(self.B, K, 1, 4), y).bool()
+
     def _run(self):
         m = self.model
         if self.fused_base:
-            self.out = m._network_outputs(None, apply_sigmoid=True, level1=(self.l1, self.l1p))
+            x, prepadded, level1 = None, False, (self.l1, self.l1p)
         else:
             x = ops.preprocess(self.images, m._mean_host, m._std_host, self.Hp, self.Wp, out=self.xpad, border=self.border,
                                mirror=self._mirror)
-            self.out = m._network_outputs(x, apply_sigmoid=True, prepadded=self.border > 0)
-        hm, wh, reg = self.out
+            prepadded, level1 = self.border > 0, None
+        y = m._features(x, prepadded, level1)
+        self.sparse = m._sparse_heads_ok(y)
+        if self.sparse:
+            return self._run_sparse(y)
+        z = m._head_outputs(y, True)
+        self._out = (m._hm_view(z["hm"]), z["wh"][..., :2], z["reg"][..., :2])
+        hm, wh, reg = self._out
         self.dec = ops.decode(hm, wh, reg, m.topk_candidates, m.backbone.down_ratio, heat_floor=ops.SIGMOID_CLAMP_FLOOR,
                               flip=self.flip)
         self.finite = ops.finite_flag(wh, reg).bool()
@@ -127,6 +151,8 @@
             self._base(self.images if images is None else images)
         elif images is not None:
             self.images.copy_(images, non_blocking=True)
+        if self.sparse:
+            self._out = None
         if self.graph is not None:
             self.graph.replay()
         else:
@@ -258,25 +284,42 @@
                                                flip=flip)
         return eng
 
-    def _head_outputs(self, y, apply_sigmoid):
+    def _heads_fusable(self, y):
+        ctx, names = self._ctx, [h.lower() for h in self.heads]
+        return (self.head_conv == ops.PackedHeads.HID and ctx.compute in (F16, F16X3) and ops.HEADS_FUSED
+                and ops.heads_fused_ok(y, ctx.compute) and len(names) <= 4
+                and all(getattr(self, n)[2].kernel_size == (1, 1) for n in names))
+
+    def _packed_heads(self, names, apply_sigmoid):
+        ctx = self._ctx
+        fcs = [getattr(self, n) for n in names]
+        acts = [ACT_SIGMOID_CLAMP if (apply_sigmoid and n == "hm") else ACT_NONE for n in names]
+        cache = self.__dict__.setdefault("_ctdet_packed", {})
+        ver = tuple((t.data_ptr(), t._version) for fc in fcs for t in (fc[0].weight, fc[0].bias, fc[2].weight, fc[2].bias))
+        key = ("heads_fused", ctx.compute, tuple(names), tuple(acts))
+        hit = cache.get(key)
+        if hit is None or hit[0] != ver:
+            ph = ops.PackedHeads([fc[0].weight for fc in fcs], [fc[0].bias for fc in fcs],
+                                 [fc[2].weight for fc in fcs], [fc[2].bias for fc in fcs], acts, compute=ctx.compute)
+            hit = cache[key] = (ver, ph)
+        return hit[1]
+
+    def _sparse_heads_ok(self, y):
+        names = sorted(h.lower() for h in self.heads)
+        return (ops.HEADS_SPARSE and self._ctx.compute == F16X3 and names == ["hm", "reg", "wh"] and self._heads_fusable(y)
+                and y.shape[3] == 64 and self.wh[2].out_channels == 2 and self.reg[2].out_channels == 2
+                and self.topk_candidates < y.shape[1] * y.shape[2])
+
+    def _head_outputs(self, y, apply_sigmoid, only=None):
         ctx = self._ctx
         names = [h.lower() for h in self.heads]
         out = {}
-        fused = (self.head_conv == ops.PackedHeads.HID and ctx.compute in (F16, F16X3) and ops.HEADS_FUSED
-                 and ops.heads_fused_ok(y, ctx.compute) and len(names) <= 4
-                 and all(getattr(self, n)[2].kernel_size == (1, 1) for n in names))
+        fused = self._heads_fusable(y)
+        assert only is None or fused
         if fused:
-            fcs = [getattr(self, n) for n in names]
-            acts = [ACT_SIGMOID_CLAMP if (apply_sigmoid and n == "hm") else ACT_NONE for n in names]
-            cache = self.__dict__.setdefault("_ctdet_packed", {})
-            ver = tuple((t.data_ptr(), t._version) for fc in fcs for t in (fc[0].weight, fc[0].bias, fc[2].weight, fc[2].bias))
-            key = ("heads_fused", ctx.compute, tuple(acts))
-            hit = cache.get(key)
-            if hit is None or hit[0] != ver:
-                ph = ops.PackedHeads([fc[0].weight for fc in fcs], [fc[0].bias for fc in fcs],
-                                     [fc[2].weight for fc in fcs], [fc[2].bias for fc in fcs], acts, compute=ctx.compute)
-                hit = cache[key] = (ver, ph)
-            outs = ops.heads_fused(y, hit[1], clamp=SIGMOID_CLAMP)
+            if only is not None:
+                names = [n for n in names if n in only]
+            outs = ops.heads_fused(y, self._packed_heads(names, apply_sigmoid), clamp=SIGMOID_CLAMP)
             return dict(zip(names, outs))
         if self.head_conv > 0:
             convs = [getattr(self, n)[0] for n in names]
@@ -325,15 +368,18 @@
                 y = y[..., :up.out_channels]
         return y
 
+    def _features(self, x_nhwc, prepadded=False, level1=None):
+        if self.backbone_type in ("resnet", "vovnet"):
+            return self._deconv_forward(self.backbone.hip_forward(x_nhwc, self._ctx, prepadded)[self.deconv_feature])
+        return self.backbone.hip_forward(x_nhwc, self._ctx, prepadded, level1=level1)[-1]
+
+    def _hm_view(self, hm):
+        assert hm.shape[3] == self.num_classes or hm.shape[3] == ops.round_up(self.num_classes, 4)
+        return hm[..., :self.num_classes] if hm.shape[3] != self.num_classes else hm
+
     def _network_outputs(self, x_nhwc, apply_sigmoid, prepadded=False, level1=None):
-        if self.backbone_type in ("resnet", "vovnet"):
-            y = self._deconv_forward(self.backbone.hip_forward(x_nhwc, self._ctx, prepadded)[self.deconv_feature])
-        else:
-            y = self.backbone.hip_forward(x_nhwc, self._ctx, prepadded, level1=level1)[-1]
-        z = self._head_outputs(y, apply_sigmoid)
-        hm = z["hm"]
-        assert hm.shape[3] == self.num_classes or hm.shape[3] == ops.round_up(self.num_classes, 4)
-        return hm[..., :self.num_classes] if hm.shape[3] != self.num_classes else hm, z["wh"][..., :2], z["reg"][..., :2]
+        z = self._head_outputs(self._features(x_nhwc, prepadded, level1), apply_sigmoid)
+        return self._hm_view(z["hm"]), z["wh"][..., :2], z["reg"][..., :2]
 
     def forward(self, batched_inputs):
         if self.training:
diff --git a/detectron2-centernet_amd/ops.py b/detectron2-centernet_amd/ops.py
--- a/detectron2-centernet_amd/ops.py
+++ b/detectron2-centernet_amd/ops.py
@@ -805,6 +805,9 @@
     d.clamp_lo, d.clamp_hi = clamp
     M = B * H * W
     prof = _Prof(None, M, False, F32, flops=sum(2.0 * M * PackedHeads.HID * (9 * ph.Cin + c) for c in ph.couts))
+    if prof.on:
+        prof.bytes = float(M * 4 * (ph.Cin + sum(round_up(c, 4) for c in ph.couts))) if x3 else prof.bytes
+        prof.info = f"M={M} {ph.Cin}->{PackedHeads.HID}->{','.join(str(c) for c in ph.couts)}"
     for _ in range(prof.reps()):
         if x3:
             rc = _lib.lib().ctdet_head_fused_x3_fwd(C.byref(d), _ptr(x), _ptr(ph.w1), _ptr(ph.s1), _ptr(ph.b1), _stream())
@@ -813,6 +816,36 @@
     _lib.check(rc, "ctdet_head_fused_x3_fwd" if x3 else "ctdet_head_fused_fwd")
     prof.done()
     return outs
+
+
+HEADS_SPARSE = os.environ.get("CTDET_NO_SPARSE_HEADS", "0") != "1"
+
+
+def heads_sparse(y, ph, inds, down_ratio, flip=False):
+    _require_cuda(y, inds)
+    assert ph.compute == F16X3 and ph.n == 2 and ph.couts == [2, 2], "heads_sparse: a pack of the wh and reg heads"
+    assert y.dtype == torch.float32 and y.shape[3] == ph.Cin and inds.dtype == torch.int32 and inds.is_contiguous()
+    assert ph.w1.shape[0] >= 2 * PackedHeads.HID and ph.w1.shape[1] == ph.Cin // 32 * 288 and ph.Cin == 64
+    NB, H, W, _ = y.shape
+    B, K = inds.shape
+    assert NB == (2 * B if flip else B) and y.stride(0) == H * W * y.stride(2) and y.stride(1) == W * y.stride(2)
+    whreg = torch.empty(B, K, 4, dtype=torch.float32, device=y.device)
+    boxes = torch.empty(B, K, 4, dtype=torch.float32, device=y.device)
+    d = HeadDesc()
+    d.nheads, d.B, d.H, d.W, d.Cin, d.in_stride = 2, B, H, W, ph.Cin, _nhwc_stride(y)
+    for h in range(2):
+        d.w2[h], d.b2[h], d.cout[h] = ph.w2[h].data_ptr(), ph.b2[h].data_ptr(), ph.couts[h]
+    M = (2 if flip else 1) * B * K
+    prof = _Prof(None, M, False, F32, flops=2.0 * M * PackedHeads.HID * (9 * ph.Cin + 2) * 2)
+    if prof.on:
+        prof.bytes = float(M * 9 * ph.Cin * 4 + ph.w1.numel() * 4)
+        prof.info = f"peaks={M} {ph.Cin}->{PackedHeads.HID}->2,2 at inds" + (" flip" if flip else "")
+    for _ in range(prof.reps()):
+        rc = _lib.lib().ctdet_head_sparse_x3_fwd(C.byref(d), _ptr(y), _ptr(ph.w1), _ptr(ph.s1), _ptr(ph.b1), _ptr(inds), K,
+                                                 float(down_ratio), int(bool(flip)), _ptr(whreg), _ptr(boxes), _stream())
+    _lib.check(rc, "ctdet_head_sparse_x3_fwd")
+    prof.done()
+    return whreg, boxes
 
 
 def maxpool3x3s2(x, out=None):
@@ -849,7 +882,8 @@
     for t in tensors:
         assert t.dtype == torch.float32 and t.dim() == 4 and t.stride(3) == 1
         B, H, W, Cc = t.shape
-        _lib.check(_lib.lib().ctdet_finite_flag(_ptr(t), B * H * W, Cc, _nhwc_stride(t), _ptr(flag), _stream()), "ctdet_finite_flag")
+        with prof_region("finite_flag", nbytes=float(t.numel() * 4), info="x".join(str(n) for n in t.shape)):
+            _lib.check(_lib.lib().ctdet_finite_flag(_ptr(t), B * H * W, Cc, _nhwc_stride(t), _ptr(flag), _stream()), "ctdet_finite_flag")
     return flag
 
 
@@ -980,9 +1014,12 @@
     _require_cuda(heat, wh, reg)
     assert heat.dtype == torch.float32
     B, H, W, Cc = heat.shape
+    assert wh is not None or reg is None, "decode: reg without wh"
     if flip:
-        assert B % 2 == 0 and wh.shape[0] == B and (reg is None or reg.shape[0] == B), "flip decode: 2B images, plain half first"
-        assert heat.stride(0) == H * W * heat.stride(2) and wh.stride(0) == H * W * wh.stride(2), "flip decode: dense batches"
+        assert B % 2 == 0 and (wh is None or wh.shape[0] == B) and (reg is None or reg.shape[0] == B), \
+            "flip decode: 2B images, plain half first"
+        assert heat.stride(0) == H * W * heat.stride(2) and (wh is None or wh.stride(0) == H * W * wh.stride(2)), \
+            "flip decode: dense batches"
         B //= 2
     if workspace is None or workspace.key != (B, H, W, Cc, K):
         workspace = DecodeWorkspace(B, H, W, Cc, K, heat.device)
@@ -993,7 +1030,7 @@
     inds = torch.empty(B, K, dtype=torch.int32, device=dev)
     with prof_region("decode", nbytes=float(B * H * W * Cc * 4), info=f"{B}x{H}x{W}x{Cc} K={K}"):
         fn = _lib.lib().ctdet_decode_flip if flip else _lib.lib().ctdet_decode
-        rc = fn(_ptr(heat), _nhwc_stride(heat), _ptr(wh), _nhwc_stride(wh), _ptr(reg),
+        rc = fn(_ptr(heat), _nhwc_stride(heat), _ptr(wh), _nhwc_stride(wh) if wh is not None else 0, _ptr(reg),
                 _nhwc_stride(reg) if reg is not None else 0, B, H, W, Cc, K, float(down_ratio),
                 float(heat_floor), _ptr(workspace.buf), _ptr(boxes), _ptr(scores), _ptr(classes), _ptr(inds), _stream())
     _lib.check(rc, "ctdet_decode")
diff --git a/include/ctdet_hip.h b/include/ctdet_hip.h
--- a/include/ctdet_hip.h
+++ b/include/ctdet_hip.h
@@ -80,6 +80,9 @@
 int32_t ctdet_head_fused_fwd(const ctdet_head_desc* d, const void* x, const void* w1, const float* b1, void* stream);
 int32_t ctdet_head_fused_x3_fwd(const ctdet_head_desc* d, const void* x, const void* w1, const float* s1, const float* b1,
                                 void* stream);
+int32_t ctdet_head_sparse_x3_fwd(const ctdet_head_desc* d, const void* x, const void* w1, const float* s1, const float* b1,
+                                 const int32_t* inds, int32_t K, float down_ratio, int32_t flip, float* whreg, float* boxes,
+                                 void* stream);
 int32_t ctdet_head_fused_supported(int32_t compute_dtype, int32_t H, int32_t W, int32_t Cin, int32_t in_stride, const void* x);
 
 typedef struct ctdet_dla_base_desc {
```

Measured after the change: 4298 images/s (median of 6 runs). 9.0% higher.
